# bezirganyan/m2-mixer

Measured on AMD Instinct MI355X. Metric: training samples/sec AV-MNIST M2-Mixer-B bf16, higher is better.
Workload: dtype bf16

## Files before the change

include/m2mixer.h:

```cpp
#ifndef M2MIXER_H
#define M2MIXER_H

#include <stdint.h>

#ifdef __cplusplus
extern "C" {
#endif

#define M2M_ABI_VERSION 18
#define M2M_MAX_BLOCKS 8
#define M2M_ROWS_PER_WG 16

#define M2M_SPLIT_GPART 1472

#define M2M_PREC_BF16 0
#define M2M_PREC_F32 1

typedef struct m2m_block {
    const float* ln1_w;
    const float* ln1_b;
    const float* tok_w1;
    const float* tok_b1;
    const float* tok_w2;
    const float* tok_b2;
    const float* ln2_w;
    const float* ln2_b;
    const float* ch_w1;
    const float* ch_b1;
    const float* ch_w2;
    const float* ch_b2;
    void* w1n;
    void* w2c;
    void* w2tn;
    void* w1tc;
    float* ch_b1p;
    float* g_ln1_w; float* g_ln1_b; float* g_tok_w1; float* g_tok_b1; float* g_tok_w2; float* g_tok_b2;
    float* g_ln2_w; float* g_ln2_b; float* g_ch_w1; float* g_ch_b1; float* g_ch_w2; float* g_ch_b2;
    float* x_in;
    float* x_mid;
    void* at_chn;
    void* dyt_chn;
    void* h_chn;
    void* dh_chn;
} m2m_block;

typedef struct m2m_tower {
    int32_t prec;
    int32_t D, N, T, C;
    int32_t Cp;
    int32_t nblocks;
    int32_t has_final_ln;
    float p_drop;
    uint32_t site_base;
    const float* lnf_w;
    const float* lnf_b;
    float* g_lnf_w;
    float* g_lnf_b;
    float* x_final;
    float* ws_a;
    float* ws_b;
    m2m_block blk[M2M_MAX_BLOCKS];
    float* slabs;
    int32_t nsplit;
    int32_t wgrad_flags;
    float* xres;
    float* gpart;
    void* a_nat[M2M_MAX_BLOCKS];
    void* dy_nat[M2M_MAX_BLOCKS];
    float* wslot[M2M_MAX_BLOCKS];
    void* dx0_chn;
} m2m_tower;
#define M2M_WGRAD_OVERWRITE 1
#define M2M_WGRAD_GROUP_SLOTS 4
#define M2M_WGRAD_REDUCES_SMALL 2

typedef struct m2m_embed {
    int32_t prec;
    int32_t Cin, H, W, ph, pw;
    int32_t D;
    int32_t K;
    int32_t Kp;
    const float* w;
    const float* b;
    void* wn;
    float* g_w;
    float* g_b;
    int32_t wgrad_flags;
    int32_t reserved;
} m2m_embed;

int m2m_abi_version(void);
const char* m2m_last_error(void);
int64_t m2m_packed_bytes(int prec, int64_t I, int64_t K);

int m2m_pack(int prec, int mode, int order_k_major, const float* src, int64_t stride_i, int64_t stride_k,
             int64_t I, int64_t K, void* dst, void* stream);
int m2m_pack_tower(const m2m_tower* t, void* stream);
int m2m_pack_embed(const m2m_embed* e, void* stream);
int m2m_pack_all(const m2m_tower* const* towers, int ntowers, const m2m_embed* const* embeds, int nembeds, void* stream);
int m2m_pack_skips_w1tc(const m2m_tower* t);

int m2m_embed_forward(const m2m_embed* e, const float* input, int B, float* x0, void* stream);
typedef struct m2m_step_head {
    float* adam_state; uint32_t* drop_counter; float* losses; int32_t nlosses;
} m2m_step_head;
int m2m_embeds_forward(const m2m_embed* const* embeds, const float* const* inputs, float* const* x0s, const int* nsplits,
                       const int64_t* part_strides, int nembeds, int B, const m2m_step_head* head, void* stream);
int m2m_embed_fwd_splits(const m2m_embed* e);
int m2m_embed_forward_head(const m2m_embed* e, const float* input, int B, float* x0, const m2m_step_head* head, void* stream);

int m2m_tower_forward(const m2m_tower* t, const float* x0, int64_t x0_sample_stride, int B,
                      float* out, int64_t out_sample_stride, float* pooled,
                      int training, uint32_t seed, uint32_t step, const uint32_t* step_dev, void* stream);

int m2m_towers_can_group(const m2m_tower* a, const m2m_tower* b, int B);
typedef struct m2m_tower_io {
    const float* x0; int64_t x0_sample_stride;
    float* out; int64_t out_sample_stride;
    float* pooled;
    int32_t x0_parts;
    int64_t x0_part_stride;
} m2m_tower_io;
int m2m_towers_forward(const m2m_tower* const* towers, const m2m_tower_io* io, int ntowers, int B, int training,
                       uint32_t seed, uint32_t step, const uint32_t* step_dev, void* stream);
int m2m_towers_forward_embeds_ok(const m2m_tower* const* towers, int ntowers, const m2m_embed* const* embeds, int B);
int m2m_towers_forward_embeds(const m2m_tower* const* towers, const m2m_tower_io* io, int ntowers,
                              const m2m_embed* const* embeds, const float* const* inputs, const m2m_step_head* head,
                              int B, int training, uint32_t seed, uint32_t step, const uint32_t* step_dev, void* stream);

int m2m_tower_backward(const m2m_tower* t, int B, const float* d_out, int64_t d_out_sample_stride,
                       const float* d_pooled, float* d_x0, int64_t d_x0_sample_stride,
                       uint32_t seed, uint32_t step, const uint32_t* step_dev, void* stream);
typedef struct m2m_tower_gio {
    const float* d_out; int64_t d_out_sample_stride;
    const float* d_pooled;
    float* d_x0; int64_t d_x0_sample_stride;
} m2m_tower_gio;
int m2m_towers_backward(const m2m_tower* const* towers, const m2m_tower_gio* io, int ntowers, int B,
                        uint32_t seed, uint32_t step, const uint32_t* step_dev, void* stream);
int m2m_tower_wgrad(const m2m_tower* t, int B, uint32_t seed, uint32_t step, const uint32_t* step_dev, void* stream);
int m2m_wgrad_form(const m2m_tower* t, int B);
int m2m_towers_wgrad(const m2m_tower* const* towers, const m2m_tower* const* dev_towers, int ntowers,
                     const m2m_embed* const* embeds, const float* const* inputs, const float* const* d_x0s,
                     const m2m_tower* const* embed_towers, int nembeds,
                     int B, uint32_t seed, uint32_t step, const uint32_t* step_dev, void* stream);
int m2m_wgrad_groups(const m2m_tower* t, int B);
int m2m_embeds_wgrad_form(const m2m_embed* const* embeds, const m2m_tower* const* embed_towers, int nembeds, int B);
int m2m_wgrad_slot_groups(const m2m_tower* const* towers, int ntowers, int B);
int m2m_wgrad_fold(const m2m_tower* t, void* stream);
int m2m_embed_wgrad(const m2m_embed* e, const float* input, const float* d_x0, int B, void* stream);
int m2m_embeds_wgrad(const m2m_embed* const* embeds, const float* const* inputs, const float* const* d_x0s, int nembeds, int B,
                     void* stream);

typedef struct m2m_head {
    const float* pooled;
    const float* w;
    const float* b;
    float* g_w;
    float* g_b;
    float* d_pooled;
    float weight;
    float* g_part;
    const float* tokens;
    int64_t tok_sample_stride;
    int32_t ntok;
} m2m_head;
int m2m_heads_part_tiles(int B);
int m2m_heads_ce(const m2m_head* heads, int nheads, const int64_t* labels, int B, int D, int K,
                 float* logits, float* losses, int32_t* preds, int zero_losses, void* stream);

int m2m_heads_bce(const m2m_head* heads, int nheads, const float* targets, const float* pos_weight, int B, int D, int K,
                  float* logits, float* losses, int32_t* preds, int zero_losses, void* stream);

int m2m_heads_ce_w(const m2m_head* heads, int nheads, const int64_t* labels, int B, int D, int K,
                   float* logits, float* losses, int32_t* preds, int zero_losses, const float* weights, void* stream);
int m2m_heads_bce_w(const m2m_head* heads, int nheads, const float* targets, const float* pos_weight, int B, int D, int K,
                    float* logits, float* losses, int32_t* preds, int zero_losses, const float* weights, void* stream);

int m2m_towers_wgrad_heads(const m2m_tower* const* towers, const m2m_tower* const* dev_towers, int ntowers,
                           const m2m_embed* const* embeds, const float* const* inputs, const float* const* d_x0s,
                           const m2m_tower* const* embed_towers, int nembeds,
                           int B, uint32_t seed, uint32_t step, const uint32_t* step_dev,
                           const m2m_head* heads, int nheads, int K, void* stream);

int m2m_towers_wgrad_tail(const m2m_tower* const* towers, const m2m_tower* const* dev_towers, int ntowers,
                          const m2m_embed* const* embeds, const float* const* inputs, const float* const* d_x0s,
                          const m2m_tower* const* embed_towers, int nembeds,
                          int B, uint32_t seed, uint32_t step, const uint32_t* step_dev,
                          const m2m_head* heads, int nheads, int K, uint32_t* bump_counter, void* stream);

int m2m_tower_backward_heads_ok(const m2m_tower* t, int B, int nheads, int K);
int m2m_tower_backward_heads(const m2m_tower* t, int B, const m2m_head* heads, int nheads, int own, const int64_t* labels,
                             int K, float* logits, float* losses, int32_t* preds, float* d_x0, int64_t d_x0_sample_stride,
                             uint32_t seed, uint32_t step, const uint32_t* step_dev, void* stream);

#define M2M_MLP_MAX_LAYERS 4
typedef struct m2m_mlp {
    int32_t nlayers;
    int32_t has_out;
    int32_t dims[M2M_MLP_MAX_LAYERS + 1];
    float p_drop;
    uint32_t site_base;
    const float* w[M2M_MLP_MAX_LAYERS];
    const float* b[M2M_MLP_MAX_LAYERS];
    float* g_w[M2M_MLP_MAX_LAYERS];
    float* g_b[M2M_MLP_MAX_LAYERS];
    float* act[M2M_MLP_MAX_LAYERS];
} m2m_mlp;
int m2m_mlp_forward(const m2m_mlp* m, const float* x, int B, float* out, int64_t out_sample_stride, float* out_dense,
                    int training, uint32_t seed, uint32_t step, const uint32_t* step_dev, void* stream);
int m2m_mlp_backward(const m2m_mlp* m, const float* x, int B, const float* d_out, int64_t d_out_sample_stride,
                     const float* d_out_dense, void* stream);
int m2m_mlp_forward_ride(const m2m_mlp* m, const float* x, int B, float* out, int64_t out_sample_stride, float* out_dense,
                         int training, uint32_t seed, uint32_t step, const uint32_t* step_dev);
int m2m_mlp_backward_ride(const m2m_mlp* m, const float* x, int B, const float* d_out, int64_t d_out_sample_stride,
                          const float* d_out_dense);
int m2m_mlp_ride_flush(void* stream);

int m2m_adam_step(float* param, float* grad, float* exp_avg, float* exp_avg_sq, int64_t n,
                  float* state, float beta1, float beta2, float eps, float weight_decay,
                  float grad_scale, int bump_step, void* stream);
int m2m_adam_step_bf16(float* param, float* grad, const void* grad_bf16, float* exp_avg, float* exp_avg_sq, int64_t n,
                       float* state, float beta1, float beta2, float eps, float weight_decay,
                       float grad_scale, int bump_step, void* stream);

#define M2M_MAX_GRAD_RANGES 16
typedef struct m2m_grad_range { int64_t lo, n; const float* add; int32_t keep; int32_t reserved; } m2m_grad_range;
int m2m_adam_step_ranges(float* param, float* grad, const void* grad_bf16, float* exp_avg, float* exp_avg_sq, int64_t n,
                         float* state, float beta1, float beta2, float eps, float weight_decay, float grad_scale, int bump_step,
                         const m2m_grad_range* ranges, int nranges, void* stream);

int64_t m2m_adam_pack_plan_bytes(void);
int m2m_adam_pack_plan(const m2m_tower* const* towers, int ntowers, const m2m_embed* const* embeds, int nembeds,
                       float* param, float* grad, const void* grad_bf16, float* exp_avg, float* exp_avg_sq, int64_t n,
                       const float* state, float beta1, float beta2, float eps, float weight_decay, float grad_scale,
                       void* plan_host);
int m2m_adam_pack_plan_ranges(const m2m_tower* const* towers, int ntowers, const m2m_embed* const* embeds, int nembeds,
                              float* param, float* grad, const void* grad_bf16, float* exp_avg, float* exp_avg_sq, int64_t n,
                              const float* state, float beta1, float beta2, float eps, float weight_decay, float grad_scale,
                              const m2m_grad_range* ranges, int nranges, void* plan_host);
int m2m_adam_pack_all(const m2m_tower* const* towers, int ntowers, const m2m_embed* const* embeds, int nembeds,
                      const void* plan_dev, const void* plan_host, void* stream);

int m2m_step_prologue(float* adam_state, uint32_t* drop_counter, float* losses, int nlosses, void* stream);

int m2m_counter_add(uint32_t* counter, uint32_t delta, void* stream);

#define M2M_FUSION_SUM 1
#define M2M_FUSION_MEAN 2
#define M2M_FUSION_MAX 3
int m2m_fusion_forward(int mode, const float* a, const float* b, float* y, int64_t n, void* stream);
int m2m_fusion_backward(int mode, const float* a, const float* b, const float* dy, float* da, float* db, int64_t n, void* stream);

typedef struct m2m_gate {
    int32_t D;
    int32_t reserved;
    const float *w1, *b1, *w2, *b2, *wz, *bz;
    float *g_w1, *g_b1, *g_w2, *g_b2, *g_wz, *g_bz;
    float *t1, *t2, *z, *dh, *part;
} m2m_gate;
int64_t m2m_gate_part_floats(int64_t rows, int D);
int m2m_gate_forward(const m2m_gate* g, const float* a, const float* b, float* y, int64_t rows, int save, void* stream);
int m2m_gate_backward(const m2m_gate* g, const float* dy, float* da, float* db, int64_t rows, void* stream);
int m2m_gate_wgrad(const m2m_gate* g, const float* a, const float* b, int64_t rows, void* stream);

#define M2M_SCORES_MAX_CLASSES 64
#define M2M_SCORES_MAX_LABELS 128
int m2m_scores_multiclass(const int32_t* preds, const int64_t* labels, int nheads, int B, int K, uint64_t* table, void* stream);
int m2m_scores_multilabel(const int32_t* preds, const float* targets, int nheads, int B, int K, uint64_t* table, void* stream);

int m2m_dropout_mask(const m2m_tower* t, int blk, int site, int B, uint32_t seed, uint32_t step,
                     uint8_t* mask, void* stream);
int m2m_gelu_probe(const float* x, float* y, float* dy, int64_t n, void* stream);
int m2m_gemm_probe(int prec, const float* A, const float* Bm, int I, int J, int K,
                   const float* Bc, int J2, float* C, float* C2, void* workspace, void* stream);

int m2m_clock_probe(uint64_t* out, int nwg, int spin_ticks, void* stream);

#ifdef __cplusplus
}
#endif
#endif
```

m2_mixer_amd/_lib.py:

```python
from __future__ import annotations

import ctypes as C
import os
import subprocess

_HERE = os.path.dirname(os.path.abspath(__file__))
LIB_PATH = os.environ.get("M2M_LIB_PATH", os.path.join(_HERE, "libm2mixer.so"))
CSRC = os.path.join(_HERE, "csrc")

ABI_VERSION = 18
MAX_BLOCKS = 8
ROWS_PER_WG = 16
HCHN_PAD = 4096
SPLIT_ROWS = 128
SPLIT_MAX = 8
SPLIT_GPART = 1472
PREC_BF16, PREC_F32 = 0, 1
PREC_BY_NAME = {"bf16": PREC_BF16, "fp32": PREC_F32, "f32": PREC_F32}

_fp = C.c_void_p


class Block(C.Structure):
    PARAMS = ["ln1_w", "ln1_b", "tok_w1", "tok_b1", "tok_w2", "tok_b2", "ln2_w", "ln2_b",
              "ch_w1", "ch_b1", "ch_w2", "ch_b2"]
    PACKED = ["w1n", "w2c", "w2tn", "w1tc", "ch_b1p"]
    GRADS = ["g_" + p for p in PARAMS]
    SAVED = ["x_in", "x_mid", "at_chn", "dyt_chn", "h_chn", "dh_chn"]
    _fields_ = [(n, _fp) for n in PARAMS + PACKED + GRADS + SAVED]


class Tower(C.Structure):
    _fields_ = [("prec", C.c_int32), ("D", C.c_int32), ("N", C.c_int32), ("T", C.c_int32), ("C", C.c_int32),
                ("Cp", C.c_int32), ("nblocks", C.c_int32), ("has_final_ln", C.c_int32),
                ("p_drop", C.c_float), ("site_base", C.c_uint32),
                ("lnf_w", _fp), ("lnf_b", _fp), ("g_lnf_w", _fp), ("g_lnf_b", _fp), ("x_final", _fp),
                ("ws_a", _fp), ("ws_b", _fp), ("blk", Block * MAX_BLOCKS),
                ("slabs", _fp), ("nsplit", C.c_int32), ("wgrad_flags", C.c_int32), ("xres", _fp), ("gpart", _fp),
                ("a_nat", _fp * MAX_BLOCKS), ("dy_nat", _fp * MAX_BLOCKS),
                ("wslot", _fp * MAX_BLOCKS),
                ("dx0_chn", _fp)]


WGRAD_OVERWRITE = 1
WGRAD_REDUCES_SMALL = 2
WGRAD_GROUP_SLOTS = 4
MAX_GRAD_RANGES = 16


class GradRange(C.Structure):
    _fields_ = [("lo", C.c_int64), ("n", C.c_int64), ("add", _fp), ("keep", C.c_int32), ("reserved", C.c_int32)]


class TowerIO(C.Structure):
    _fields_ = [("x0", _fp), ("x0_ss", C.c_int64), ("out", _fp), ("out_ss", C.c_int64), ("pooled", _fp),
                ("x0_parts", C.c_int32), ("x0_part_stride", C.c_int64)]


class StepHead(C.Structure):
    _fields_ = [("adam_state", _fp), ("drop_counter", _fp), ("losses", _fp), ("nlosses", C.c_int32)]


class TowerGIO(C.Structure):
    _fields_ = [("d_out", _fp), ("d_out_ss", C.c_int64), ("d_pooled", _fp), ("d_x0", _fp), ("d_x0_ss", C.c_int64)]


class Embed(C.Structure):
    _fields_ = [("prec", C.c_int32), ("Cin", C.c_int32), ("H", C.c_int32), ("W", C.c_int32), ("ph", C.c_int32),
                ("pw", C.c_int32), ("D", C.c_int32), ("K", C.c_int32), ("Kp", C.c_int32),
                ("w", _fp), ("b", _fp), ("wn", _fp), ("g_w", _fp), ("g_b", _fp), ("wgrad_flags", C.c_int32), ("reserved", C.c_int32)]


class Head(C.Structure):
    _fields_ = [("pooled", _fp), ("w", _fp), ("b", _fp), ("g_w", _fp), ("g_b", _fp), ("d_pooled", _fp),
                ("weight", C.c_float), ("g_part", _fp), ("tokens", _fp), ("tok_sample_stride", C.c_int64), ("ntok", C.c_int32)]


SCORES_MAX_CLASSES, SCORES_MAX_LABELS = 64, 128
FUSION_SUM, FUSION_MEAN, FUSION_MAX = 1, 2, 3


class Gate(C.Structure):
    _fields_ = [("D", C.c_int32), ("reserved", C.c_int32)] + [(n, _fp) for n in (
        "w1", "b1", "w2", "b2", "wz", "bz", "g_w1", "g_b1", "g_w2", "g_b2", "g_wz", "g_bz", "t1", "t2", "z", "dh", "part")]


MLP_MAX_LAYERS = 4


class Mlp(C.Structure):
    _fields_ = [("nlayers", C.c_int32), ("has_out", C.c_int32), ("dims", C.c_int32 * (MLP_MAX_LAYERS + 1)),
                ("p_drop", C.c_float), ("site_base", C.c_uint32),
                ("w", _fp * MLP_MAX_LAYERS), ("b", _fp * MLP_MAX_LAYERS), ("g_w", _fp * MLP_MAX_LAYERS),
                ("g_b", _fp * MLP_MAX_LAYERS), ("act", _fp * MLP_MAX_LAYERS)]


SIGNATURES = {
    "m2m_abi_version": (C.c_int, []),
    "m2m_last_error": (C.c_char_p, []),
    "m2m_packed_bytes": (C.c_int64, [C.c_int, C.c_int64, C.c_int64]),
    "m2m_pack": (C.c_int, [C.c_int, C.c_int, C.c_int, _fp, C.c_int64, C.c_int64, C.c_int64, C.c_int64, _fp, _fp]),
    "m2m_pack_tower": (C.c_int, [C.POINTER(Tower), _fp]),
    "m2m_pack_embed": (C.c_int, [C.POINTER(Embed), _fp]),
    "m2m_pack_skips_w1tc": (C.c_int, [C.POINTER(Tower)]),
    "m2m_pack_all": (C.c_int, [C.POINTER(C.POINTER(Tower)), C.c_int, C.POINTER(C.POINTER(Embed)), C.c_int, _fp]),
    "m2m_embed_forward": (C.c_int, [C.POINTER(Embed), _fp, C.c_int, _fp, _fp]),
    "m2m_embed_forward_head": (C.c_int, [C.POINTER(Embed), _fp, C.c_int, _fp, C.POINTER(StepHead), _fp]),
    "m2m_tower_forward": (C.c_int, [C.POINTER(Tower), _fp, C.c_int64, C.c_int, _fp, C.c_int64, _fp, C.c_int,
                                    C.c_uint32, C.c_uint32, _fp, _fp]),
    "m2m_tower_backward": (C.c_int, [C.POINTER(Tower), C.c_int, _fp, C.c_int64, _fp, _fp, C.c_int64,
                                     C.c_uint32, C.c_uint32, _fp, _fp]),
    "m2m_tower_backward_heads_ok": (C.c_int, [C.POINTER(Tower), C.c_int, C.c_int, C.c_int]),
    "m2m_tower_backward_heads": (C.c_int, [C.POINTER(Tower), C.c_int, C.POINTER(Head), C.c_int, C.c_int, _fp, C.c_int, _fp, _fp, _fp, _fp,
                                           C.c_int64, C.c_uint32, C.c_uint32, _fp, _fp]),
    "m2m_tower_wgrad": (C.c_int, [C.POINTER(Tower), C.c_int, C.c_uint32, C.c_uint32, _fp, _fp]),
    "m2m_towers_can_group": (C.c_int, [C.POINTER(Tower), C.POINTER(Tower), C.c_int]),
    "m2m_towers_forward": (C.c_int, [C.POINTER(C.POINTER(Tower)), C.POINTER(TowerIO), C.c_int, C.c_int, C.c_int, C.c_uint32,
                                     C.c_uint32, _fp, _fp]),
    "m2m_towers_forward_embeds_ok": (C.c_int, [C.POINTER(C.POINTER(Tower)), C.c_int, C.POINTER(C.POINTER(Embed)), C.c_int]),
    "m2m_towers_forward_embeds": (C.c_int, [C.POINTER(C.POINTER(Tower)), C.POINTER(TowerIO), C.c_int, C.POINTER(C.POINTER(Embed)),
                                            C.POINTER(_fp), C.POINTER(StepHead), C.c_int, C.c_int, C.c_uint32, C.c_uint32, _fp, _fp]),
    "m2m_towers_backward": (C.c_int, [C.POINTER(C.POINTER(Tower)), C.POINTER(TowerGIO), C.c_int, C.c_int, C.c_uint32, C.c_uint32,
                                      _fp, _fp]),
    "m2m_towers_wgrad": (C.c_int, [C.POINTER(C.POINTER(Tower)), C.POINTER(_fp), C.c_int, C.POINTER(C.POINTER(Embed)), C.POINTER(_fp),
                                   C.POINTER(_fp), C.POINTER(C.POINTER(Tower)), C.c_int, C.c_int, C.c_uint32, C.c_uint32, _fp, _fp]),
    "m2m_towers_wgrad_heads": (C.c_int, [C.POINTER(C.POINTER(Tower)), C.POINTER(_fp), C.c_int, C.POINTER(C.POINTER(Embed)), C.POINTER(_fp),
                                         C.POINTER(_fp), C.POINTER(C.POINTER(Tower)), C.c_int, C.c_int, C.c_uint32, C.c_uint32, _fp,
                                         C.POINTER(Head), C.c_int, C.c_int, _fp]),
    "m2m_towers_wgrad_tail": (C.c_int, [C.POINTER(C.POINTER(Tower)), C.POINTER(_fp), C.c_int, C.POINTER(C.POINTER(Embed)), C.POINTER(_fp),
                                        C.POINTER(_fp), C.POINTER(C.POINTER(Tower)), C.c_int, C.c_int, C.c_uint32, C.c_uint32, _fp,
                                        C.POINTER(Head), C.c_int, C.c_int, _fp, _fp]),
    "m2m_heads_part_tiles": (C.c_int, [C.c_int]),
    "m2m_wgrad_form": (C.c_int, [C.POINTER(Tower), C.c_int]),
    "m2m_embeds_wgrad_form": (C.c_int, [C.POINTER(C.POINTER(Embed)), C.POINTER(C.POINTER(Tower)), C.c_int, C.c_int]),
    "m2m_wgrad_groups": (C.c_int, [C.POINTER(Tower), C.c_int]),
    "m2m_wgrad_slot_groups": (C.c_int, [C.POINTER(C.POINTER(Tower)), C.c_int, C.c_int]),
    "m2m_wgrad_fold": (C.c_int, [C.POINTER(Tower), _fp]),
    "m2m_adam_step_ranges": (C.c_int, [_fp, _fp, _fp, _fp, _fp, C.c_int64, _fp, C.c_float, C.c_float, C.c_float, C.c_float,
                                       C.c_float, C.c_int, C.POINTER(GradRange), C.c_int, _fp]),
    "m2m_counter_add": (C.c_int, [_fp, C.c_uint32, _fp]),
    "m2m_embed_wgrad": (C.c_int, [C.POINTER(Embed), _fp, _fp, C.c_int, _fp]),
    "m2m_embeds_wgrad": (C.c_int, [C.POINTER(C.POINTER(Embed)), C.POINTER(_fp), C.POINTER(_fp), C.c_int, C.c_int, _fp]),
    "m2m_embeds_forward": (C.c_int, [C.POINTER(C.POINTER(Embed)), C.POINTER(_fp), C.POINTER(_fp), C.POINTER(C.c_int), C.POINTER(C.c_int64),
                                     C.c_int, C.c_int, C.POINTER(StepHead), _fp]),
    "m2m_embed_fwd_splits": (C.c_int, [C.POINTER(Embed)]),
    "m2m_heads_ce": (C.c_int, [C.POINTER(Head), C.c_int, _fp, C.c_int, C.c_int, C.c_int, _fp, _fp, _fp, C.c_int, _fp]),
    "m2m_step_prologue": (C.c_int, [_fp, _fp, _fp, C.c_int, _fp]),
    "m2m_heads_bce": (C.c_int, [C.POINTER(Head), C.c_int, _fp, _fp, C.c_int, C.c_int, C.c_int, _fp, _fp, _fp, C.c_int, _fp]),
    "m2m_heads_ce_w": (C.c_int, [C.POINTER(Head), C.c_int, _fp, C.c_int, C.c_int, C.c_int, _fp, _fp, _fp, C.c_int, _fp, _fp]),
    "m2m_heads_bce_w": (C.c_int, [C.POINTER(Head), C.c_int, _fp, _fp, C.c_int, C.c_int, C.c_int, _fp, _fp, _fp, C.c_int, _fp, _fp]),
    "m2m_fusion_forward": (C.c_int, [C.c_int, _fp, _fp, _fp, C.c_int64, _fp]),
    "m2m_fusion_backward": (C.c_int, [C.c_int, _fp, _fp, _fp, _fp, _fp, C.c_int64, _fp]),
    "m2m_gate_part_floats": (C.c_int64, [C.c_int64, C.c_int]),
    "m2m_gate_forward": (C.c_int, [C.POINTER(Gate), _fp, _fp, _fp, C.c_int64, C.c_int, _fp]),
    "m2m_gate_backward": (C.c_int, [C.POINTER(Gate), _fp, _fp, _fp, C.c_int64, _fp]),
    "m2m_gate_wgrad": (C.c_int, [C.POINTER(Gate), _fp, _fp, C.c_int64, _fp]),
    "m2m_scores_multiclass": (C.c_int, [_fp, _fp, C.c_int, C.c_int, C.c_int, _fp, _fp]),
    "m2m_scores_multilabel": (C.c_int, [_fp, _fp, C.c_int, C.c_int, C.c_int, _fp, _fp]),
    "m2m_mlp_forward": (C.c_int, [C.POINTER(Mlp), _fp, C.c_int, _fp, C.c_int64, _fp, C.c_int, C.c_uint32, C.c_uint32,
                                  _fp, _fp]),
    "m2m_mlp_backward": (C.c_int, [C.POINTER(Mlp), _fp, C.c_int, _fp, C.c_int64, _fp, _fp]),
    "m2m_mlp_forward_ride": (C.c_int, [C.POINTER(Mlp), _fp, C.c_int, _fp, C.c_int64, _fp, C.c_int, C.c_uint32, C.c_uint32, _fp]),
    "m2m_mlp_backward_ride": (C.c_int, [C.POINTER(Mlp), _fp, C.c_int, _fp, C.c_int64, _fp]),
    "m2m_mlp_ride_flush": (C.c_int, [_fp]),
    "m2m_adam_step": (C.c_int, [_fp, _fp, _fp, _fp, C.c_int64, _fp, C.c_float, C.c_float, C.c_float, C.c_float,
                                C.c_float, C.c_int, _fp]),
    "m2m_adam_step_bf16": (C.c_int, [_fp, _fp, _fp, _fp, _fp, C.c_int64, _fp, C.c_float, C.c_float, C.c_float, C.c_float,
                                     C.c_float, C.c_int, _fp]),
    "m2m_adam_pack_plan_bytes": (C.c_int64, []),
    "m2m_adam_pack_plan": (C.c_int, [C.POINTER(C.POINTER(Tower)), C.c_int, C.POINTER(C.POINTER(Embed)), C.c_int, _fp, _fp, _fp, _fp, _fp,
                                    C.c_int64, _fp, C.c_float, C.c_float, C.c_float, C.c_float, C.c_float, _fp]),
    "m2m_adam_pack_plan_ranges": (C.c_int, [C.POINTER(C.POINTER(Tower)), C.c_int, C.POINTER(C.POINTER(Embed)), C.c_int, _fp, _fp, _fp, _fp, _fp,
                                           C.c_int64, _fp, C.c_float, C.c_float, C.c_float, C.c_float, C.c_float,
                                           C.POINTER(GradRange), C.c_int, _fp]),
    "m2m_adam_pack_all": (C.c_int, [C.POINTER(C.POINTER(Tower)), C.c_int, C.POINTER(C.POINTER(Embed)), C.c_int, _fp, _fp, _fp]),
    "m2m_dropout_mask": (C.c_int, [C.POINTER(Tower), C.c_int, C.c_int, C.c_int, C.c_uint32, C.c_uint32, _fp, _fp]),
    "m2m_gelu_probe": (C.c_int, [_fp, _fp, _fp, C.c_int64, _fp]),
    "m2m_gemm_probe": (C.c_int, [C.c_int, _fp, _fp, C.c_int, C.c_int, C.c_int, _fp, C.c_int, _fp, _fp, _fp, _fp]),
    "m2m_clock_probe": (C.c_int, [_fp, C.c_int, C.c_int, _fp]),
}

_lib = None


def csrc_hash() -> str:
    import glob
    import hashlib
    h = hashlib.sha256()
    for f in sorted(glob.glob(os.path.join(CSRC, "*.hip")) + glob.glob(os.path.join(CSRC, "*.h")) +
                    [os.path.join(os.path.dirname(_HERE), "include", "m2mixer.h")]):
        h.update(os.path.basename(f).encode())
        h.update(open(f, "rb").read())
    return h.hexdigest()


def build(force: bool = False, verbose: bool = False) -> str:
    if force:
        subprocess.run(["make", "-C", CSRC, "clean"], check=True, capture_output=not verbose)
    r = subprocess.run(["make", "-C", CSRC, "-j", str(min(6, os.cpu_count() or 2))], capture_output=True, text=True)
    if r.returncode != 0:
        raise RuntimeError("building libm2mixer.so failed:\n" + r.stdout[-4000:] + r.stderr[-4000:])
    if verbose:
        print(r.stdout)
    return LIB_PATH


def lib() -> C.CDLL:
    global _lib
    if _lib is None:
        if not os.path.exists(LIB_PATH):
            raise RuntimeError(
                f"{LIB_PATH} is missing: the M2-Mixer hot path exists only as the HIP library "
                "(python -c 'import __graft_entry__ as g; g.build()' builds it); there is no CPU fallback")
        L = C.CDLL(LIB_PATH)
        for name, (res, args) in SIGNATURES.items():
            fn = getattr(L, name)
            fn.restype = res
            fn.argtypes = args
        got = L.m2m_abi_version()
        if got != ABI_VERSION:
            raise RuntimeError(f"libm2mixer ABI {got} != binding ABI {ABI_VERSION}; rebuild")
        _lib = L
    return _lib


def check(rc: int, what: str = "") -> None:
    if rc != 0:
        msg = lib().m2m_last_error().decode("utf-8", "replace")
        kind = "unsupported shape/argument" if rc == -1 else "HIP runtime error"
        raise RuntimeError(f"libm2mixer {what}: {kind}: {msg}")


def ptr(t) -> int:
    return 0 if t is None else t.data_ptr()


def stream_ptr() -> int:
    import torch
    return torch.cuda.current_stream().cuda_stream


def packed_bytes(prec: int, I: int, K: int) -> int:
    kb = 32 if prec == PREC_BF16 else 16
    return ((I + 15) // 16) * ((K + kb - 1) // kb) * 1024
```

m2_mixer_amd/csrc/embed.hip:

```cpp
#include "tile.h"
#include "embed_wgrad.h"

#include "embed_fwd.h"

template <int P, int D, int RB>
__global__ __launch_bounds__(NTHREADS) void embed_fwd_kernel(const m2m_embed em, const float* __restrict__ in, long M, int N,
                                                             float* __restrict__ x0, int fast, const m2m_step_head head) {
    extern __shared__ __attribute__((aligned(16))) char smem[];
    if (blockIdx.x == 0) {
        const int t = threadIdx.x;
        if (t == 0 && head.adam_state) head.adam_state[0] += 1.0f;
        if (t == 1 && head.drop_counter) *head.drop_counter += 1u;
        if (head.losses && t < head.nlosses) head.losses[t] = 0.f;
    }
    if (P == PREC_BF16 && fast) embed_fwd_fast_body<D>(em, in, M, N, x0, blockIdx.x, 0, 1, smem);
    else embed_fwd_body<P, D, RB>(em, in, M, N, x0, blockIdx.x, smem);
}

struct EmbedFwdGroupArgs {
    m2m_embed em[2];
    const float* in[2];
    float* x0[2];
    long M[2];
    int N[2], nwg0, fast[2], nsplit[2];
    long part_stride[2];
    float* adam_state;
    unsigned int* drop_counter;
    float* losses;
    int nlosses, prologue;
};
template <int P, int D, int RB>
__global__ __launch_bounds__(NTHREADS, (P == PREC_BF16 && D <= 128) ? 4 : 1) void embed_fwd_group_kernel(const EmbedFwdGroupArgs a) {
    extern __shared__ __attribute__((aligned(16))) char smem[];
    if (a.prologue && blockIdx.x == 0) {
        const int t = threadIdx.x;
        if (t == 0 && a.adam_state) a.adam_state[0] += 1.0f;
        if (t == 1 && a.drop_counter) *a.drop_counter += 1u;
        if (a.losses && t < a.nlosses) a.losses[t] = 0.f;
    }
    const int e = (int)blockIdx.x < a.nwg0 ? 0 : 1;
    const int wg = e ? blockIdx.x - a.nwg0 : blockIdx.x;
    if (P == PREC_BF16 && a.fast[e]) {
        const int ns = a.nsplit[e], split = wg % ns;
        embed_fwd_fast_body<D>(a.em[e], a.in[e], a.M[e], a.N[e], a.x0[e] + split * a.part_stride[e], wg / ns, split, ns, smem);
    }
    else {
        const int ns = a.nsplit[e], split = wg % ns, tile = wg / ns;
        if (split == 0) embed_fwd_body<P, D, RB>(a.em[e], a.in[e], a.M[e], a.N[e], a.x0[e], tile, smem);
        else {
            float* part = a.x0[e] + split * a.part_stride[e];
            const long m0 = (long)tile * RB;
            for (int idx = threadIdx.x; idx < RB * D; idx += NTHREADS) {
                const long m = m0 + idx / D;
                if (m < a.M[e]) part[m * D + idx % D] = 0.f;
            }
        }
    }
}

template <int P, int D>
__global__ __launch_bounds__(NTHREADS) void embed_wgrad_kernel(const m2m_embed em, const float* __restrict__ in,
                                                               const float* __restrict__ dx0, long M, int N, int tiles_per_group) {
    extern __shared__ __attribute__((aligned(16))) char smem[];
    embed_wgrad_body<P, D, NTHREADS>(em, in, dx0, M, N, tiles_per_group, blockIdx.x, blockIdx.y, gridDim.y == 1, smem);
}

template <int P, int D>
__global__ __launch_bounds__(NTHREADS) void embed_wgrad_group_kernel(const EmbedWgradGroupArgs a) {
    extern __shared__ __attribute__((aligned(16))) char smem[];
    embed_wgrad_group_body<P, D, NTHREADS>(a, blockIdx.x, smem);
}

int m2m_check_embed(const m2m_embed* e, int B) {
    if (!e || B < 1) { m2m_set_error("embed: bad argument", __FILE__, __LINE__); return -1; }
    if (e->H % e->ph || e->W % e->pw) { m2m_set_error("embed: image not divisible by patch", __FILE__, __LINE__); return -1; }
    if (e->K != e->Cin * e->ph * e->pw) { m2m_set_error("embed: K != Cin*ph*pw", __FILE__, __LINE__); return -1; }
    const int KB = e->prec == PREC_BF16 ? 32 : 16;
    if (e->Kp % KB || e->Kp < e->K) { m2m_set_error("embed: Kp must be K rounded up to the k-block", __FILE__, __LINE__); return -1; }
    if (e->Kp > EMB_KMAX - EMB_KS) { m2m_set_error("embed: patch too large (Cin*ph*pw must be <= 3968)", __FILE__, __LINE__); return -1; }
    return 0;
}

template <int P, int D>
static int launch_embed_fwd(const m2m_embed* e, const float* in, int B, float* x0, hipStream_t st, const m2m_step_head* head = nullptr) {
    m2m_step_head hd;
    memset(&hd, 0, sizeof(hd));
    if (head) {
        if (head->nlosses < 0 || head->nlosses > 64) { m2m_set_error("embed_forward: step head nlosses must be in [0, 64]", __FILE__, __LINE__); return -1; }
        hd = *head;
    }
    const int N = (e->H / e->ph) * (e->W / e->pw);
    const long M = (long)B * N;
    constexpr int RB = 16;
    const size_t lds = (size_t)RB * EMB_LD * 4 + (size_t)RB * EMB_KS * Prec<P>::ESZ + EMB_KMAX * 4 + RB * 8;
    auto kern = embed_fwd_kernel<P, D, RB>;
    static bool done = false;
    if (!done) { M2M_CHECK_HIP(hipFuncSetAttribute(reinterpret_cast<const void*>(kern), hipFuncAttributeMaxDynamicSharedMemorySize, (int)lds)); done = true; }
    hipLaunchKernelGGL(kern, dim3((unsigned)((M + RB - 1) / RB)), dim3(NTHREADS), lds, st, *e, in, M, N, x0, (int)embed_fwd_fast_ok(e, in), hd);
    M2M_CHECK_HIP(hipGetLastError());
    return 0;
}
template <int P, int D>
static int launch_embed_fwd_group(const m2m_embed* const* es, const float* const* ins, float* const* x0s, const int* nsplits,
                                  const int64_t* part_strides, const m2m_step_head* head, int B, hipStream_t st) {
    constexpr int RB = 16;
    EmbedFwdGroupArgs a;
    memset(&a, 0, sizeof(a));
    if (head) {
        if (head->nlosses < 0 || head->nlosses > 64) { m2m_set_error("embeds_forward: step head nlosses must be in [0, 64]", __FILE__, __LINE__); return -1; }
        a.prologue = 1; a.adam_state = head->adam_state; a.drop_counter = head->drop_counter; a.losses = head->losses; a.nlosses = head->nlosses;
    }
    const int first = es[1]->Kp > es[0]->Kp ? 1 : 0;
    int total = 0;
    for (int k = 0; k < 2; ++k) {
        const int i = k == 0 ? first : 1 - first;
        const int N = (es[i]->H / es[i]->ph) * (es[i]->W / es[i]->pw);
        a.em[k] = *es[i]; a.in[k] = ins[i]; a.x0[k] = x0s[i]; a.N[k] = N; a.M[k] = (long)B * N;
        a.fast[k] = embed_fwd_fast_ok(es[i], ins[i]);
        a.nsplit[k] = nsplits ? nsplits[i] : 1;
        a.part_stride[k] = part_strides ? (long)part_strides[i] : 0;
        if (a.nsplit[k] < 1 || a.nsplit[k] > 4 || (a.nsplit[k] > 1 && a.part_stride[k] < a.M[k] * (long)D)) {
            m2m_set_error("embeds_forward: 1..4 k-splits, part stride >= B*N*D", __FILE__, __LINE__);
            return -1;
        }
        const int nwg = (int)((a.M[k] + RB - 1) / RB) * a.nsplit[k];
        if (k == 0) a.nwg0 = nwg;
        total += nwg;
    }
    const size_t lds = (size_t)RB * EMB_LD * 4 + (size_t)RB * EMB_KS * Prec<P>::ESZ + EMB_KMAX * 4 + RB * 8;
    auto kern = embed_fwd_group_kernel<P, D, RB>;
    static bool done = false;
    if (!done) { M2M_CHECK_HIP(hipFuncSetAttribute(reinterpret_cast<const void*>(kern), hipFuncAttributeMaxDynamicSharedMemorySize, (int)lds)); done = true; }
    hipLaunchKernelGGL(kern, dim3((unsigned)total), dim3(NTHREADS), lds, st, a);
    M2M_CHECK_HIP(hipGetLastError());
    return 0;
}

template <int P, int D>
static int launch_embed_wgrad(const m2m_embed* e, const float* in, const float* dx0, int B, hipStream_t st) {
    const EmbedWgradPlan pl = embed_wgrad_plan(e, B, 256);
    const size_t lds = embed_wgrad_lds<D, P>();
    auto kern = embed_wgrad_kernel<P, D>;
    static bool done = false;
    if (!done) { M2M_CHECK_HIP(hipFuncSetAttribute(reinterpret_cast<const void*>(kern), hipFuncAttributeMaxDynamicSharedMemorySize, (int)lds)); done = true; }
    hipLaunchKernelGGL(kern, dim3((unsigned)pl.nchunks, (unsigned)pl.groups), dim3(NTHREADS), lds, st, *e, in, dx0, pl.M, pl.N, pl.tpg);
    M2M_CHECK_HIP(hipGetLastError());
    return 0;
}
template <int P, int D>
static int launch_embed_wgrad_group(const m2m_embed* const* es, const float* const* ins, const float* const* dx0s, int B, hipStream_t st) {
    EmbedWgradGroupArgs a;
    const int total = embed_wgrad_group_args(a, es, ins, dx0s, B, 256);
    const size_t lds = embed_wgrad_lds<D, P>();
    auto kern = embed_wgrad_group_kernel<P, D>;
    static bool done = false;
    if (!done) { M2M_CHECK_HIP(hipFuncSetAttribute(reinterpret_cast<const void*>(kern), hipFuncAttributeMaxDynamicSharedMemorySize, (int)lds)); done = true; }
    hipLaunchKernelGGL(kern, dim3((unsigned)total), dim3(NTHREADS), lds, st, a);
    M2M_CHECK_HIP(hipGetLastError());
    return 0;
}

extern "C" int m2m_embed_forward(const m2m_embed* e, const float* input, int B, float* x0, void* stream) {
    return m2m_embed_forward_head(e, input, B, x0, nullptr, stream);
}
extern "C" int m2m_embed_forward_head(const m2m_embed* e, const float* input, int B, float* x0, const m2m_step_head* head, void* stream) {
    if (int rc = m2m_check_embed(e, B)) return rc;
    hipStream_t st = reinterpret_cast<hipStream_t>(stream);
#define M2M_EF_CASE(PP, DD) if (e->prec == PP && e->D == DD) return launch_embed_fwd<PP, DD>(e, input, B, x0, st, head);
    M2M_EF_CASE(PREC_BF16, 32) M2M_EF_CASE(PREC_BF16, 64) M2M_EF_CASE(PREC_BF16, 128) M2M_EF_CASE(PREC_BF16, 256)
    M2M_EF_CASE(PREC_F32, 32) M2M_EF_CASE(PREC_F32, 64) M2M_EF_CASE(PREC_F32, 128) M2M_EF_CASE(PREC_F32, 256)
#undef M2M_EF_CASE
    m2m_set_error("embed_forward: unsupported (prec, D)", __FILE__, __LINE__);
    return -1;
}

extern "C" int m2m_embed_wgrad(const m2m_embed* e, const float* input, const float* d_x0, int B, void* stream) {
    if (int rc = m2m_check_embed(e, B)) return rc;
    hipStream_t st = reinterpret_cast<hipStream_t>(stream);
#define M2M_EW_CASE(PP, DD) if (e->prec == PP && e->D == DD) return launch_embed_wgrad<PP, DD>(e, input, d_x0, B, st);
    M2M_EW_CASE(PREC_BF16, 32) M2M_EW_CASE(PREC_BF16, 64) M2M_EW_CASE(PREC_BF16, 128) M2M_EW_CASE(PREC_BF16, 256)
    M2M_EW_CASE(PREC_F32, 32) M2M_EW_CASE(PREC_F32, 64) M2M_EW_CASE(PREC_F32, 128) M2M_EW_CASE(PREC_F32, 256)
#undef M2M_EW_CASE
    m2m_set_error("embed_wgrad: unsupported (prec, D)", __FILE__, __LINE__);
    return -1;
}

extern "C" int m2m_embeds_wgrad(const m2m_embed* const* embeds, const float* const* inputs, const float* const* d_x0s, int nembeds,
                                int B, void* stream) {
    if (!embeds || !inputs || !d_x0s || nembeds != EMB_GROUP) { m2m_set_error("embeds_wgrad: exactly two embeddings", __FILE__, __LINE__); return -1; }
    for (int i = 0; i < nembeds; ++i) {
        if (int rc = m2m_check_embed(embeds[i], B)) return rc;
        if (embeds[i]->prec != embeds[0]->prec || embeds[i]->D != embeds[0]->D) {
            m2m_set_error("embeds_wgrad: the embeddings of one launch must share precision and hidden_dim", __FILE__, __LINE__);
            return -1;
        }
    }
    hipStream_t st = reinterpret_cast<hipStream_t>(stream);
    const m2m_embed* e = embeds[0];
#define M2M_EWG_CASE(PP, DD) if (e->prec == PP && e->D == DD) return launch_embed_wgrad_group<PP, DD>(embeds, inputs, d_x0s, B, st);
    M2M_EWG_CASE(PREC_BF16, 32) M2M_EWG_CASE(PREC_BF16, 64) M2M_EWG_CASE(PREC_BF16, 128) M2M_EWG_CASE(PREC_BF16, 256)
    M2M_EWG_CASE(PREC_F32, 32) M2M_EWG_CASE(PREC_F32, 64) M2M_EWG_CASE(PREC_F32, 128) M2M_EWG_CASE(PREC_F32, 256)
#undef M2M_EWG_CASE
    m2m_set_error("embeds_wgrad: unsupported (prec, D)", __FILE__, __LINE__);
    return -1;
}

extern "C" int m2m_embed_fwd_splits(const m2m_embed* e) {
    if (!e) return 1;
    static const int forced = [] { const char* v = getenv("M2M_EMBED_SPLITS"); return v ? atoi(v) : 0; }();
    const bool pays = embed_fwd_fast_ok(e, nullptr) && e->Kp >= 4 * EMB_FKS;
    if (pays && forced >= 1 && forced <= 4) return forced;
    return pays ? 2 : 1;
}

extern "C" int m2m_embeds_forward(const m2m_embed* const* embeds, const float* const* inputs, float* const* x0s, const int* nsplits,
                                  const int64_t* part_strides, int nembeds, int B, const m2m_step_head* head, void* stream) {
    if (!embeds || !inputs || !x0s || nembeds != 2) { m2m_set_error("embeds_forward: exactly two embeddings", __FILE__, __LINE__); return -1; }
    for (int i = 0; i < nembeds; ++i) {
        if (int rc = m2m_check_embed(embeds[i], B)) return rc;
        if (embeds[i]->prec != embeds[0]->prec || embeds[i]->D != embeds[0]->D) {
            m2m_set_error("embeds_forward: the embeddings of one launch must share precision and hidden_dim", __FILE__, __LINE__);
            return -1;
        }
    }
    hipStream_t st = reinterpret_cast<hipStream_t>(stream);
    const m2m_embed* e = embeds[0];
#define M2M_EFG_CASE(PP, DD) if (e->prec == PP && e->D == DD) return launch_embed_fwd_group<PP, DD>(embeds, inputs, x0s, nsplits, part_strides, head, B, st);
    M2M_EFG_CASE(PREC_BF16, 32) M2M_EFG_CASE(PREC_BF16, 64) M2M_EFG_CASE(PREC_BF16, 128) M2M_EFG_CASE(PREC_BF16, 256)
    M2M_EFG_CASE(PREC_F32, 32) M2M_EFG_CASE(PREC_F32, 64) M2M_EFG_CASE(PREC_F32, 128) M2M_EFG_CASE(PREC_F32, 256)
#undef M2M_EFG_CASE
    m2m_set_error("embeds_forward: unsupported (prec, D)", __FILE__, __LINE__);
    return -1;
}
```

m2_mixer_amd/csrc/embed_fwd.h:

```cpp
#pragma once
#include "tile.h"
#include "embed_wgrad.h"

#ifndef EMB_KS
#define EMB_KS 128
#endif
#define EMB_LD (EMB_KS + 4)
#define EMB_KMAX 4096

template <int P, int D, int RB>
static __device__ __forceinline__ void embed_fwd_body(const m2m_embed& em, const float* __restrict__ in, long M, int N,
                                                      float* __restrict__ x0, int wg, char* smem) {
    typedef Prec<P> Pr;
    constexpr int DT = D / 16, KSB = EMB_KS / Pr::KB;
    constexpr int DPW = (DT + NWAVES - 1) / NWAVES;
    float* tile = reinterpret_cast<float*>(smem);
    char* img = smem + RB * EMB_LD * 4;
    int* koff = reinterpret_cast<int*>(img + RB * EMB_KS * Pr::ESZ);
    long* rbase = reinterpret_cast<long*>(koff + EMB_KMAX);

    const int tid = threadIdx.x, lane = tid & 63, wave = tid >> 6, g = lane >> 4, il = lane & 15;
    PatchGeom pg{em.Cin, em.H, em.W, em.ph, em.pw, em.W / em.pw, N, em.K};
    const long m0 = (long)wg * RB;
    const int nKB = em.Kp / Pr::KB;
    const int kext = (em.Kp + EMB_KS - 1) / EMB_KS * EMB_KS;
    for (int k = tid; k < kext; k += NTHREADS) koff[k] = patch_koff(pg, k);
    if (tid < RB) rbase[tid] = patch_rowbase(pg, m0 + tid, M);

    f32x4_t acc[(RB / 16)][DPW];
#pragma unroll
    for (int mt = 0; mt < (RB / 16); ++mt)
#pragma unroll
        for (int j = 0; j < DPW; ++j) acc[mt][j] = f32x4_t{0.f, 0.f, 0.f, 0.f};

    constexpr int EPT = RB * EMB_KS / NTHREADS;
    float pre[EPT];
    Frag wpre[DPW][KSB];
    auto load_stage = [&](int k0) {
#pragma unroll
        for (int i = 0; i < EPT; ++i) {
            const int idx = i * NTHREADS + tid;
            const int r = idx / EMB_KS, kk = idx % EMB_KS;
            const long rb = rbase[r];
            const int ko = koff[k0 + kk];
            pre[i] = (rb >= 0 && ko >= 0) ? in[rb + ko] : 0.f;
        }
        const int kb0 = k0 / Pr::KB;
#pragma unroll
        for (int j = 0; j < DPW; ++j) {
            const int dt = wave + NWAVES * j;
#pragma unroll
            for (int kb = 0; kb < KSB; ++kb) {
                wpre[j][kb].u = u32x4_t{0u, 0u, 0u, 0u};
                if (dt < DT && kb0 + kb < nKB) wpre[j][kb] = ld_frag_global(em.wn, (long)dt * nKB + kb0 + kb, lane);
            }
        }
    };
    __syncthreads();
    load_stage(0);
    for (int k0 = 0; k0 < em.Kp; k0 += EMB_KS) {
#pragma unroll
        for (int i = 0; i < EPT; ++i) {
            const int idx = i * NTHREADS + tid;
            tile[(idx / EMB_KS) * EMB_LD + idx % EMB_KS] = pre[i];
        }
        Frag wcur[DPW][KSB];
#pragma unroll
        for (int j = 0; j < DPW; ++j)
#pragma unroll
            for (int kb = 0; kb < KSB; ++kb) wcur[j][kb] = wpre[j][kb];
        __syncthreads();
        if (k0 + EMB_KS < em.Kp) load_stage(k0 + EMB_KS);
        for (int slot = tid; slot < (RB / 16) * KSB * 64; slot += NTHREADS) {
            const int blk = slot >> 6;
            *reinterpret_cast<u32x4_t*>(img + slot * 16) =
                gather_slot<P>(tile, EMB_LD, PACK_NAT, false, blk / KSB, blk % KSB, slot & 63);
        }
        __syncthreads();
#pragma unroll
        for (int j = 0; j < DPW; ++j) {
            const int dt = wave + NWAVES * j;
            if (dt < DT) {
#pragma unroll
                for (int kb = 0; kb < KSB; ++kb) {
#pragma unroll
                    for (int mt = 0; mt < (RB / 16); ++mt) {
                        const Frag a = ld_frag_lds(img, mt * KSB + kb, lane);
                        Pr::mma(acc[mt][j], a, wcur[j][kb]);
                    }
                }
            }
        }
    }
#pragma unroll
    for (int j = 0; j < DPW; ++j) {
        const int dt = wave + NWAVES * j;
        if (dt < DT) {
            const int d = 16 * dt + il;
            const float bv = em.b[d];
#pragma unroll
            for (int mt = 0; mt < (RB / 16); ++mt)
#pragma unroll
                for (int r = 0; r < 4; ++r) {
                    const long m = m0 + 16 * mt + 4 * g + r;
                    if (m < M) x0[m * D + d] = acc[mt][j][r] + bv;
                }
        }
    }
}

#define EMB_FKS 256
#ifndef EMB_FDEPTH
#define EMB_FDEPTH 2
#endif
template <int D>
static __device__ __forceinline__ void embed_fwd_fast_body(const m2m_embed& em, const float* __restrict__ in, long M, int N,
                                                           float* __restrict__ x0, int wg, int split, int nsplit, char* smem) {
    typedef Prec<PREC_BF16> Pr;
    constexpr int KSB = EMB_FKS / 32, DT = D / 16, DPW = (DT + NWAVES - 1) / NWAVES, IMG_B = 16 * EMB_FKS * 2;
    static_assert(KSB == NWAVES, "one k-block of the stage per wave");
    char* img = smem;
    const int tid = threadIdx.x, lane = tid & 63, wave = tid >> 6, g = lane >> 4, il = lane & 15;
    PatchGeom pg{em.Cin, em.H, em.W, em.ph, em.pw, em.W / em.pw, N, em.K};
    const long m0 = (long)wg * 16;
    const long rb = patch_rowbase(pg, m0 + il, M);
    const int nKB = em.Kp / 32;
    const int nst_all = (em.Kp + EMB_FKS - 1) / EMB_FKS;
    const int per = (nst_all + nsplit - 1) / nsplit;
    const int st_begin = split * per, nst = min(nst_all, st_begin + per);

    f32x4_t acc[DPW];
#pragma unroll
    for (int j = 0; j < DPW; ++j) acc[j] = f32x4_t{0.f, 0.f, 0.f, 0.f};
    struct Pre {
        f32x4_t p0, p1;
        Frag w[DPW][KSB];
    };
    auto load = [&](Pre& p, int st) {
        const int k = min(st * EMB_FKS + wave * 32 + 8 * g, em.K - 8);
        const float* src = in + (rb >= 0 ? rb : 0) + patch_koff(pg, k);
        p.p0 = *reinterpret_cast<const f32x4_t*>(src);
        p.p1 = *reinterpret_cast<const f32x4_t*>(src + 4);
#pragma unroll
        for (int j = 0; j < DPW; ++j) {
            const int dt = min(wave + NWAVES * j, DT - 1);
#pragma unroll
            for (int kb = 0; kb < KSB; ++kb) p.w[j][kb] = ld_frag_global(em.wn, (long)dt * nKB + min(st * KSB + kb, nKB - 1), lane);
        }
    };
    auto step = [&](Pre& p, int st) {
        const bool valid = rb >= 0 && st < nst && st * EMB_FKS + wave * 32 + 8 * g < em.K;
        Frag f;
        f.u[0] = pack_bf2(p.p0[0], p.p0[1]); f.u[1] = pack_bf2(p.p0[2], p.p0[3]);
        f.u[2] = pack_bf2(p.p1[0], p.p1[1]); f.u[3] = pack_bf2(p.p1[2], p.p1[3]);
        if (!valid) f.u = u32x4_t{0u, 0u, 0u, 0u};
        char* cur = img + ((st - st_begin) & 1) * IMG_B;
        *reinterpret_cast<u32x4_t*>(cur + tid * 16) = f.u;
        __syncthreads();
#pragma unroll
        for (int kb = 0; kb < KSB; ++kb) {
            const Frag a = ld_frag_lds(cur, kb, lane);
#pragma unroll
            for (int j = 0; j < DPW; ++j)
                if (wave + NWAVES * j < DT) Pr::mma(acc[j], a, p.w[j][kb]);
        }
        load(p, st + EMB_FDEPTH);
    };
    Pre ring[EMB_FDEPTH];
#pragma unroll
    for (int d = 0; d < EMB_FDEPTH; ++d) load(ring[d], st_begin + d);
    for (int st = st_begin; st < nst; st += EMB_FDEPTH) {
#pragma unroll
        for (int d = 0; d < EMB_FDEPTH; ++d) step(ring[d], st + d);
    }
#pragma unroll
    for (int j = 0; j < DPW; ++j) {
        const int dt = wave + NWAVES * j;
        if (dt < DT) {
            const int d = 16 * dt + il;
            const float bv = split == 0 ? em.b[d] : 0.f;
#pragma unroll
            for (int r = 0; r < 4; ++r) {
                const long m = m0 + 4 * g + r;
                if (m < M) x0[m * D + d] = acc[j][r] + bv;
            }
        }
    }
}
static inline bool embed_fwd_fast_ok(const m2m_embed* e, const float* in) {
    return e->prec == PREC_BF16 && e->pw % 8 == 0 && e->W % 4 == 0 && e->K >= 8 && (reinterpret_cast<uintptr_t>(in) & 15) == 0;
}
```

m2_mixer_amd/csrc/embed_wgrad.h:

```cpp
#pragma once
#include "tile.h"
#include <stdlib.h>

#define EBM 32

int m2m_check_embed(const m2m_embed* e, int B);

struct PatchGeom {
    int Cin, H, W, ph, pw, GW, N, K;
};
static __device__ __forceinline__ int patch_koff(const PatchGeom& pg, int k) {
    if (k >= pg.K) return -1;
    const int c = k / (pg.ph * pg.pw), rem = k % (pg.ph * pg.pw);
    const int py = rem / pg.pw, px = rem % pg.pw;
    return (c * pg.H + py) * pg.W + px;
}
static __device__ __forceinline__ long patch_rowbase(const PatchGeom& pg, long m, long M) {
    if (m >= M) return -1;
    const long b = m / pg.N;
    const int n = (int)(m % pg.N);
    const int gy = n / pg.GW, gx = n % pg.GW;
    return (b * pg.Cin * pg.H + gy * pg.ph) * (long)pg.W + gx * pg.pw;
}

template <int P, int D, int NT>
static __device__ __forceinline__ void embed_wgrad_body(const m2m_embed& em, const float* __restrict__ in,
                                                        const float* __restrict__ dx0, long M, int N, int tiles_per_group,
                                                        int chunk, int group, bool single, char* smem) {
    typedef Prec<P> Pr;
    constexpr int DT = D / 16, NKM = EBM / Pr::KB, XLD = TileGeom<D>::XLD;
    constexpr int KC = 64, KCT = KC / 16, PLD = KC + 4;
    constexpr int DPW = (DT + (NT / 64) - 1) / (NT / 64);
    constexpr int NDX = (EBM * (D / 4) + NT - 1) / NT;
    constexpr int NPT = EBM * KC / NT;
    static_assert(NT % KC == 0 && EBM % (NT / KC) == 0, "patch tile mapping");
    float* dxt = reinterpret_cast<float*>(smem);
    float* pt = dxt + EBM * XLD;
    char* aimg = reinterpret_cast<char*>(pt + EBM * PLD);
    char* bimg = aimg + EBM * D * Pr::ESZ;

    const int tid = threadIdx.x, lane = tid & 63, wave = tid >> 6, g = lane >> 4, il = lane & 15;
    PatchGeom pg{em.Cin, em.H, em.W, em.ph, em.pw, em.W / em.pw, N, em.K};
    const int k0 = chunk * KC;
    const int ko = patch_koff(pg, k0 + (tid % KC));

    f32x4_t acc[DPW][KCT];
#pragma unroll
    for (int j = 0; j < DPW; ++j)
#pragma unroll
        for (int kt = 0; kt < KCT; ++kt) acc[j][kt] = f32x4_t{0.f, 0.f, 0.f, 0.f};
    float bsum = 0.f;

    const long ntiles = (M + EBM - 1) / EBM;
    const long t_begin = (long)group * tiles_per_group;
    const long t_end = min(ntiles, t_begin + tiles_per_group);
    float4 dxr[NDX];
    float ptr_[NPT];
    auto load_tile = [&](long tl) {
        const long m0 = tl * EBM;
#pragma unroll
        for (int i = 0; i < NDX; ++i) {
            const int idx = i * NT + tid;
            const int r = idx / (D / 4), c = (idx % (D / 4)) * 4;
            dxr[i] = make_float4(0.f, 0.f, 0.f, 0.f);
            if (idx < EBM * (D / 4) && m0 + r < M) dxr[i] = *reinterpret_cast<const float4*>(dx0 + (m0 + r) * D + c);
        }
#pragma unroll
        for (int i = 0; i < NPT; ++i) {
            const long rb = patch_rowbase(pg, m0 + tid / KC + (NT / KC) * i, M);
            ptr_[i] = (rb >= 0 && ko >= 0) ? in[rb + ko] : 0.f;
        }
    };
    if (t_begin < t_end) load_tile(t_begin);
    for (long tl = t_begin; tl < t_end; ++tl) {
        __syncthreads();
#pragma unroll
        for (int i = 0; i < NDX; ++i) {
            const int idx = i * NT + tid;
            if (idx < EBM * (D / 4)) *reinterpret_cast<float4*>(dxt + (idx / (D / 4)) * XLD + (idx % (D / 4)) * 4) = dxr[i];
        }
#pragma unroll
        for (int i = 0; i < NPT; ++i) pt[(tid / KC + (NT / KC) * i) * PLD + tid % KC] = ptr_[i];
        if (tl + 1 < t_end) load_tile(tl + 1);
        __syncthreads();
        if (chunk == 0 && tid < D) {
            float s = 0.f;
            for (int r = 0; r < EBM; ++r) s += dxt[r * XLD + tid];
            bsum += s;
        }
        for (int slot = tid; slot < DT * NKM * 64; slot += NT) {
            const int blk = slot >> 6;
            *reinterpret_cast<u32x4_t*>(aimg + slot * 16) =
                gather_slot<P>(dxt, XLD, PACK_NAT, true, blk / NKM, blk % NKM, slot & 63);
        }
        for (int slot = tid; slot < KCT * NKM * 64; slot += NT) {
            const int blk = slot >> 6;
            *reinterpret_cast<u32x4_t*>(bimg + slot * 16) =
                gather_slot<P>(pt, PLD, PACK_NAT, true, blk / NKM, blk % NKM, slot & 63);
        }
        __syncthreads();
#pragma unroll
        for (int j = 0; j < DPW; ++j) {
            const int dt = wave + (NT / 64) * j;
            if (dt < DT) {
#pragma unroll
                for (int kbm = 0; kbm < NKM; ++kbm) {
                    const Frag a = ld_frag_lds(aimg, dt * NKM + kbm, lane);
#pragma unroll
                    for (int kt = 0; kt < KCT; ++kt) {
                        const Frag b = ld_frag_lds(bimg, kt * NKM + kbm, lane);
                        Pr::mma(acc[j][kt], a, b);
                    }
                }
            }
        }
    }
#pragma unroll
    for (int j = 0; j < DPW; ++j) {
        const int dt = wave + (NT / 64) * j;
        if (dt < DT) {
#pragma unroll
            for (int kt = 0; kt < KCT; ++kt)
#pragma unroll
                for (int r = 0; r < 4; ++r) {
                    const int d = 16 * dt + 4 * g + r, k = k0 + 16 * kt + il;
                    if (k < em.K) {
                        float* p = em.g_w + (long)d * em.K + k;
                        if (single) *p += acc[j][kt][r]; else atomicAdd(p, acc[j][kt][r]);
                    }
                }
        }
    }
    if (chunk == 0 && tid < D) { if (single) em.g_b[tid] += bsum; else atomicAdd(em.g_b + tid, bsum); }
}

#define EFK 32
template <int D, int NT> static constexpr size_t embed_wgrad_fast_red_bytes() { return (size_t)(NT / 64) * (EFK / 16) * (D / 16) * 64 * 16; }
bool m2m_split_eligible(const m2m_tower* t, int B, int training);
template <int D, int NT>
static __device__ __forceinline__ void embed_wgrad_fast_body(const m2m_embed& em, const float* __restrict__ in,
                                                             const char* __restrict__ dx0_chn, long M, int N, int npairs, int rpt,
                                                             int chunk, bool vec2, char* smem) {
    typedef Prec<PREC_BF16> Pr;
    constexpr int DT = D / 16, NW = NT / 64, NB = EFK / 16;
    static_assert(NB == 2, "two 16-column fragments per workgroup (the 8-byte gather pairs them)");
    const int tid = threadIdx.x, lane = tid & 63, g = lane >> 4, il = lane & 15;
    const int wave = __builtin_amdgcn_readfirstlane(tid >> 6);
    PatchGeom pg{em.Cin, em.H, em.W, em.ph, em.pw, em.W / em.pw, N, em.K};
    const int k0 = chunk * EFK;
    int ko[NB];
#pragma unroll
    for (int jb = 0; jb < NB; ++jb) ko[jb] = patch_koff(pg, vec2 ? k0 + 2 * il + jb : k0 + 16 * jb + il);
    int* tokoff = reinterpret_cast<int*>(smem + embed_wgrad_fast_red_bytes<D, NT>());
    for (int n = tid; n < N; n += NT) tokoff[n] = (n / pg.GW) * pg.ph * pg.W + (n % pg.GW) * pg.pw;
    __syncthreads();
    const unsigned int sstride = (unsigned int)(em.Cin * em.H * em.W), uN = (unsigned int)N, uM = (unsigned int)M;
    const unsigned int magic = 0xFFFFFFFFu / uN;

    f32x4_t acc[NB][DT];
#pragma unroll
    for (int jb = 0; jb < NB; ++jb)
#pragma unroll
        for (int dt = 0; dt < DT; ++dt) acc[jb][dt] = f32x4_t{0.f, 0.f, 0.f, 0.f};

    struct Tile { Frag a[DT]; float v[NB][8]; unsigned int okbits; };
    auto load = [&](Tile& t, int p) {
#pragma unroll
        for (int dt = 0; dt < DT; ++dt) t.a[dt] = ld_frag_global(dx0_chn, (long)p * DT + dt, lane);
        unsigned int rb[8];
        bool okr[8];
#pragma unroll
        for (int e = 0; e < 8; ++e) {
            const int r = 4 * g + (e & 3);
            const unsigned int row = (unsigned int)((2 * p + (e >> 2)) * rpt + r);
            okr[e] = r < rpt && row < uM;
            const unsigned int rowc = okr[e] ? row : 0u;
            unsigned int q = __umulhi(rowc, magic);
            unsigned int n = rowc - q * uN;
            if (n >= uN) { n -= uN; q += 1u; }
            rb[e] = q * sstride + (unsigned int)tokoff[n];
        }
        if (vec2) {
            const unsigned int k2 = (unsigned int)max(ko[0], 0);
#pragma unroll
            for (int e = 0; e < 8; ++e) {
                const float2 x = *reinterpret_cast<const float2*>(in + rb[e] + k2);
                t.v[0][e] = x.x; t.v[1][e] = x.y;
            }
        } else {
#pragma unroll
            for (int e = 0; e < 8; ++e)
#pragma unroll
                for (int jb = 0; jb < NB; ++jb) t.v[jb][e] = in[rb[e] + (unsigned int)max(ko[jb], 0)];
        }
        t.okbits = 0u;
#pragma unroll
        for (int e = 0; e < 8; ++e) t.okbits |= (okr[e] ? 1u : 0u) << e;
    };
    auto mac = [&](const Tile& t) {
#pragma unroll
        for (int jb = 0; jb < NB; ++jb) {
            Frag b;
            float z[8];
#pragma unroll
            for (int e = 0; e < 8; ++e) z[e] = ((t.okbits >> e) & 1u) && ko[jb] >= 0 ? t.v[jb][e] : 0.f;
#pragma unroll
            for (int e = 0; e < 4; ++e) b.u[e] = pack_bf2(z[2 * e], z[2 * e + 1]);
#pragma unroll
            for (int dt = 0; dt < DT; ++dt) Pr::mma(acc[jb][dt], t.a[dt], b);
        }
    };
    Tile t0, t1;
    const int p0 = wave;
    if (p0 < npairs) load(t0, p0);
    for (int p = p0; p < npairs; p += 2 * NW) {
        if (p + NW < npairs) load(t1, p + NW);
        mac(t0);
        if (p + NW < npairs) {
            if (p + 2 * NW < npairs) load(t0, p + 2 * NW);
            mac(t1);
        }
    }
    f32x4_t* red = reinterpret_cast<f32x4_t*>(smem);
#pragma unroll
    for (int jb = 0; jb < NB; ++jb)
#pragma unroll
        for (int dt = 0; dt < DT; ++dt) red[((wave * NB + jb) * DT + dt) * 64 + lane] = acc[jb][dt];
    __syncthreads();
    for (int q = wave; q < NB * DT; q += NW) {
        const int jb = q / DT, dt = q % DT;
        f32x4_t s = red[q * 64 + lane];
#pragma unroll
        for (int w = 1; w < NW; ++w) s = s + red[(w * NB * DT + q) * 64 + lane];
        const int k = vec2 ? k0 + 2 * il + jb : k0 + 16 * jb + il;
        if (k < em.K) {
            const bool store = (em.wgrad_flags & M2M_WGRAD_OVERWRITE) != 0;
#pragma unroll
            for (int r = 0; r < 4; ++r) {
                float* qd = em.g_w + (long)(16 * dt + 4 * g + r) * em.K + k;
                *qd = store ? s[r] : *qd + s[r];
            }
        }
    }
    if (chunk == 0) {
        Frag ones;
        ones.u = u32x4_t{0x3F803F80u, 0x3F803F80u, 0x3F803F80u, 0x3F803F80u};
        f32x4_t accb[DT];
#pragma unroll
        for (int dt = 0; dt < DT; ++dt) accb[dt] = f32x4_t{0.f, 0.f, 0.f, 0.f};
        for (int p = wave; p < npairs; p += NW) {
            Frag a[DT];
#pragma unroll
            for (int dt = 0; dt < DT; ++dt) a[dt] = ld_frag_global(dx0_chn, (long)p * DT + dt, lane);
#pragma unroll
            for (int dt = 0; dt < DT; ++dt) Pr::mma(accb[dt], a[dt], ones);
        }
        __syncthreads();
#pragma unroll
        for (int dt = 0; dt < DT; ++dt) red[(wave * DT + dt) * 64 + lane] = accb[dt];
        __syncthreads();
        for (int dt = wave; dt < DT; dt += NW) {
            f32x4_t sb = red[dt * 64 + lane];
#pragma unroll
            for (int w = 1; w < NW; ++w) sb = sb + red[(w * DT + dt) * 64 + lane];
            if (il == 0) {
#pragma unroll
                for (int r = 0; r < 4; ++r) em.g_b[16 * dt + 4 * g + r] += sb[r];
            }
        }
    }
}
template <int D, int NT> static constexpr size_t embed_wgrad_fast_lds() { return embed_wgrad_fast_red_bytes<D, NT>() + 128 * sizeof(int); }

#define EMB_GROUP 2
struct EmbedWgradGroupArgs {
    m2m_embed em[EMB_GROUP];
    const float* in[EMB_GROUP];
    const float* dx0[EMB_GROUP];
    long M[EMB_GROUP];
    int N[EMB_GROUP], tpg[EMB_GROUP], nchunks[EMB_GROUP], groups[EMB_GROUP];
    const char* dx0_chn[EMB_GROUP];
    int npairs[EMB_GROUP], rpt[EMB_GROUP], vec2[EMB_GROUP], fast;
};
template <int P, int D, int NT>
static __device__ __forceinline__ void embed_wgrad_group_body(const EmbedWgradGroupArgs& a, int id, char* smem) {
    const int n0 = a.nchunks[0] * a.groups[0];
    const int e = id < n0 ? 0 : 1;
    if (e) id -= n0;
    if constexpr (P == PREC_BF16) {
        if (a.fast) {
            embed_wgrad_fast_body<D, NT>(a.em[e], a.in[e], a.dx0_chn[e], a.M[e], a.N[e], a.npairs[e], a.rpt[e], id, a.vec2[e] != 0, smem);
            return;
        }
    }
    if constexpr (NT % 64 == 0 && EBM % (NT / 64) == 0)
        embed_wgrad_body<P, D, NT>(a.em[e], a.in[e], a.dx0[e], a.M[e], a.N[e], a.tpg[e], id % a.nchunks[e], id / a.nchunks[e],
                                   a.groups[e] == 1, smem);
}

struct EmbedWgradPlan { long M; int N, nchunks, groups, tpg; };
static EmbedWgradPlan embed_wgrad_plan(const m2m_embed* e, int B, int target_wgs) {
    EmbedWgradPlan pl;
    pl.N = (e->H / e->ph) * (e->W / e->pw);
    pl.M = (long)B * pl.N;
    pl.nchunks = (e->K + 63) / 64;
    const long ntiles = (pl.M + EBM - 1) / EBM;
    long groups = (target_wgs + pl.nchunks - 1) / pl.nchunks;
    if (groups > ntiles / 4) groups = ntiles / 4;
    if (groups < 1) groups = 1;
    pl.tpg = (int)((ntiles + groups - 1) / groups);
    pl.groups = (int)((ntiles + pl.tpg - 1) / pl.tpg);
    return pl;
}
template <int D, int P> static constexpr size_t embed_wgrad_lds() {
    return (size_t)EBM * TileGeom<D>::XLD * 4 + (size_t)EBM * 68 * 4 + (size_t)EBM * D * Prec<P>::ESZ + (size_t)EBM * 64 * Prec<P>::ESZ;
}


static inline int embed_wgrad_group_args_fast(EmbedWgradGroupArgs& a, const m2m_embed* const* es, const float* const* ins,
                                              const m2m_tower* const* tw, int B) {
    memset(&a, 0, sizeof(a));
    int total = 0;
    for (int i = 0; i < EMB_GROUP; ++i) {
        const m2m_embed* e = es[i];
        const m2m_tower* t = tw ? tw[i] : nullptr;
        const int N = (e->H / e->ph) * (e->W / e->pw);
        if (!t || !t->dx0_chn || e->prec != PREC_BF16 || t->prec != PREC_BF16 || m2m_is_wide(t) || t->N != N || t->D != e->D) return 0;
        if (m2m_split_eligible(t, B, 1)) return 0;
        if (N > 128 || e->D > 128 || (long)B * e->Cin * e->H * e->W >= (1L << 31)) return 0;
        const int SPW = BM / t->N, nchain = (B + SPW - 1) / SPW;
        a.em[i] = *e; a.in[i] = ins[i]; a.dx0_chn[i] = (const char*)t->dx0_chn;
        a.M[i] = (long)B * N; a.N[i] = N; a.npairs[i] = (nchain * BM + WPAIR - 1) / WPAIR; a.rpt[i] = SPW * t->N;
        a.nchunks[i] = (e->K + EFK - 1) / EFK; a.groups[i] = 1; a.tpg[i] = 0;
        static const int vec2_on = [] { const char* v = getenv("M2M_EMBED_VEC2"); return v ? atoi(v) : 1; }();
        a.vec2[i] = (vec2_on && e->pw % 2 == 0 && e->W % 2 == 0 && ((long)e->H * e->W) % 2 == 0 && e->K % 2 == 0 && ((uintptr_t)ins[i] & 7) == 0) ? 1 : 0;
        total += a.nchunks[i];
    }
    a.fast = 1;
    return total;
}

static inline int embed_wgrad_group_args(EmbedWgradGroupArgs& a, const m2m_embed* const* es, const float* const* ins,
                                         const float* const* dx0s, int B, int target_wgs, int n = EMB_GROUP) {
    memset(&a, 0, sizeof(a));
    if (n == 1) {
        const EmbedWgradPlan p0 = embed_wgrad_plan(es[0], B, target_wgs);
        a.em[0] = *es[0]; a.in[0] = ins[0]; a.dx0[0] = dx0s[0];
        a.M[0] = p0.M; a.N[0] = p0.N; a.tpg[0] = p0.tpg; a.nchunks[0] = p0.nchunks; a.groups[0] = p0.groups;
        a.em[1] = *es[0];
        return p0.nchunks * p0.groups;
    }
    EmbedWgradPlan pl[EMB_GROUP];
    for (int i = 0; i < EMB_GROUP; ++i) pl[i] = embed_wgrad_plan(es[i], B, target_wgs);
    const int first = pl[1].tpg > pl[0].tpg ? 1 : 0;
    int total = 0;
    for (int k = 0; k < EMB_GROUP; ++k) {
        const int i = k == 0 ? first : 1 - first;
        a.em[k] = *es[i]; a.in[k] = ins[i]; a.dx0[k] = dx0s[i];
        a.M[k] = pl[i].M; a.N[k] = pl[i].N; a.tpg[k] = pl[i].tpg; a.nchunks[k] = pl[i].nchunks; a.groups[k] = pl[i].groups;
        total += pl[i].nchunks * pl[i].groups;
    }
    return total;
}
```

m2_mixer_amd/csrc/tower_wgrad.hip:

```cpp
#include "tile.h"
#include "embed_wgrad.h"
#include "split.h"
#include <stdlib.h>
#include <string.h>
bool m2m_split_eligible(const m2m_tower* t, int B, int training);

#if defined(__HIP_DEVICE_COMPILE__)
#define M2M_GLOBAL_AS __attribute__((address_space(1)))
#else
#define M2M_GLOBAL_AS
#endif

#define WBM 32
#ifndef WG_RING_MAX
#define WG_RING_MAX 24
#endif
#define WG_WAVES 4
#ifndef WG_WAVES_WIDE
#define WG_WAVES_WIDE 5
#endif
#ifndef WG_LA
#define WG_LA 4
#endif
#ifndef WG_MINWAVES
// ... 225 lines not shown
        };
        auto step2 = [&](HD& x, int tile, int i) {
            char* cur = smem + (i & 1) * STAGE_B;
#pragma unroll
            for (int k = 0; k < NLD; ++k) {
                const int o = (k * G::THREADS + tid) * 16;
                if (o < STAGE_B) *reinterpret_cast<u32x4_t*>(cur + o) = st[k];
            }
            Frag hf[CPW], df[CPW];
#pragma unroll
            for (int j = 0; j < CPW; ++j) {
                hf[j].u = u32x4_t{x.h0[2 * j], x.h0[2 * j + 1], x.h1[2 * j], x.h1[2 * j + 1]};
                df[j].u = u32x4_t{x.d0[2 * j], x.d0[2 * j + 1], x.d1[2 * j], x.d1[2 * j + 1]};
            }
            load_st(min(tile + 1, t_end - 1));
            load_hd(x, min(tile + 2, t_end - 1));
            __syncthreads();
            constexpr int NQ = DT;
            constexpr int LA = WG_LA < NQ ? WG_LA : NQ;
            Frag aq[LA], dq[LA];
#pragma unroll
            for (int q = 0; q < LA; ++q) { aq[q] = ld_frag_lds(cur, q, lane); dq[q] = ld_frag_lds(cur + IMG_B, q, lane); }
#pragma unroll
            for (int q = 0; q < NQ; ++q) {
                const Frag at = aq[q % LA], dyt = dq[q % LA];
                if (q + LA < NQ) { aq[q % LA] = ld_frag_lds(cur, q + LA, lane); dq[q % LA] = ld_frag_lds(cur + IMG_B, q + LA, lane); }
#pragma unroll
                for (int j = 0; j < CPW; ++j) {
                    Pr::mma(dw1[j][q], df[j], at);
                    Pr::mma(dw2[j][q], hf[j], dyt);
                }
                if (q == NQ - 1) {
#pragma unroll
                    for (int j = 0; j < CPW; ++j) Pr::mma(db1[j], df[j], ones);
                }
            }
        };
        HD ring[2];
        load_hd(ring[0], t_begin);
        load_st(t_begin);
        load_hd(ring[1], min(t_begin + 1, t_end - 1));
        int tile = t_begin, it = 0;
        for (; tile + 2 <= t_end; tile += 2) {
            step2(ring[0], tile, it++);
            step2(ring[1], tile + 1, it++);
        }
        if (tile < t_end) step2(ring[0], tile, it++);
    } else {
    Pre p[DEPTH];
#pragma unroll
    for (int k = 0; k < DEPTH; ++k) tile_load(p[k], min(t_begin + k * TPS, t_end - 1), t_end);
    int tile = t_begin, it = 0;
    if (DEPTH == 1) {
        for (; tile < t_end; tile += TPS) step(p[0], tile, t_end, it++);
    } else {
        for (; tile + DEPTH <= t_end; tile += DEPTH) {
#pragma unroll
            for (int k = 0; k < DEPTH; ++k) step(p[k], tile + k, t_end, it++);
        }
#pragma unroll
        for (int k = 0; k + 1 < DEPTH; ++k)
            if (tile + k < t_end) step(p[k], tile + k, t_end, it++);
    }
    }

    __syncthreads();
    wgrad_write_w<D, CPW>(dw1, dw2, out, ct0, nct, C, smem, wave, lane);
#pragma unroll
    for (int j = 0; j < CPW; ++j) {
        if (ct0 + j >= nct || il != 0) continue;
#pragma unroll
        for (int r = 0; r < 4; ++r) {
            const int c = 16 * (ct0 + j) + 4 * g + r;
            if (c >= C) continue;
            if (out.mode == WG_OUT_ATOMIC) atomicAdd(out.b1 + c, db1[j][r]);
            else if (out.mode == WG_OUT_ADD) out.b1[c] += db1[j][r];
            else out.b1[c] = db1[j][r];
        }
    }
    TIMER_MARK(g_tm_wg, 4);
}

template <class TW>
static __device__ __forceinline__ WgOut wgrad_out(const TW& tw, int b, int group, int ngroups, int slot_mode) {
    const m2m_block& bk = tw.blk[b];
    WgOut o;
    o.w1 = bk.g_ch_w1; o.w2 = bk.g_ch_w2; o.b1 = bk.g_ch_b1;
    const bool overwrite = (tw.wgrad_flags & M2M_WGRAD_OVERWRITE) != 0;
    if (ngroups == 1) o.mode = overwrite ? WG_OUT_STORE : WG_OUT_ADD;
    else if (slot_mode) {
        if (group == 0) o.mode = overwrite ? WG_OUT_STORE : WG_OUT_ADD;
        else {
            const long cd = (long)tw.C * tw.D;
            float* s = tw.wslot[b];
            o.w1 = s; o.b1 = s + cd; o.w2 = s + cd + tw.C;
            o.mode = WG_OUT_STORE;
        }
    } else o.mode = WG_OUT_ATOMIC;
    return o;
}

#ifndef M2M_WGRAD_DMA
#define M2M_WGRAD_DMA 0
#endif
template <int P, int D, int RCDM> struct WgradHasDma { static constexpr bool value = M2M_WGRAD_DMA && RCDM < 0 && P == PREC_BF16 && D == 128; };

template <int P, int D, int RCDM> struct WgradKernelGeom {
    static constexpr bool RC = RCDM >= 0;
    static constexpr int LDS_PLAIN = RC ? RcGeom<D>::LDS_B : WgradGeom<P, D>::LDS_B;
    static constexpr int LDS_DMA = DrGeom<D, WgradGeom<P, D>::WAVES>::LDS_B;
    static constexpr int LDS_B = WgradHasDma<P, D, RCDM>::value ? LDS_DMA : LDS_PLAIN;
    static constexpr int COLS = RC ? RcGeom<D>::COLS : WgradGeom<P, D>::COLS;
    static constexpr int MINWAVES = RC ? 2 : WgradGeom<P, D>::MINWAVES;
    static constexpr int THREADS = RC ? RC_THREADS : WgradGeom<P, D>::THREADS;
};

template <int P, int D, int RCDM, class TW>
static __device__ __forceinline__ void wgrad_dispatch(const TW& tw, int b, int slice, int group, int ngroups, int slot_mode, int ntiles,
                                                      int tpg, int rows_per_t16, unsigned int seed, unsigned int step, int dma, char* smem) {
    const WgOut out = wgrad_out(tw, b, group, ngroups, slot_mode);
    if constexpr (RCDM >= 0) {
        const Drop dr = make_drop(true, tw.p_drop, seed, step, tw.site_base + 4u * (unsigned int)b + 2u);
        wgrad_rc_body<D, RCDM>(tw.blk[b], out, tw.Cp, tw.C, slice, group, ntiles, tpg, rows_per_t16, dr.key, dr.scale, smem);
    } else {
        if constexpr (WgradHasDma<P, D, RCDM>::value)
            wgrad_dma_body<D, WgradGeom<P, D>::WAVES>(tw.blk[b], out, tw.Cp, tw.C, slice, group, ntiles, tpg, smem);
        else
            wgrad_body<P, D>(tw.blk[b], out, tw.Cp, tw.C, slice, group, ntiles, tpg, smem);
    }
}

template <int P, int D, int RCDM>
__global__ __launch_bounds__((WgradKernelGeom<P, D, RCDM>::THREADS), (WgradKernelGeom<P, D, RCDM>::MINWAVES)) void tower_wgrad_kernel(
    const m2m_tower tw, int ntiles, int tiles_per_group, int slot_mode, int rows_per_t16, unsigned int seed, unsigned int step_host,
    const unsigned int* __restrict__ step_dev, int dma) {
    extern __shared__ __attribute__((aligned(16))) char smem[];
    const unsigned int step = step_host + (step_dev ? *step_dev : 0u);
    wgrad_dispatch<P, D, RCDM>(tw, (int)blockIdx.y, (int)blockIdx.x, (int)blockIdx.z, (int)gridDim.z, slot_mode, ntiles, tiles_per_group,
                               rows_per_t16, seed, step, dma, smem);
}

#define WG_MAX_TOWERS 4
#define WG_MAX_JOBS 32
struct WgradGroupArgs {
    const m2m_tower* tw[WG_MAX_TOWERS];
    int ntiles[WG_MAX_TOWERS], tpg[WG_MAX_TOWERS], groups[WG_MAX_TOWERS], nsl[WG_MAX_TOWERS], slot[WG_MAX_TOWERS], rpt[WG_MAX_TOWERS];
    unsigned char job_tower[WG_MAX_JOBS], job_block[WG_MAX_JOBS];
    short job_start[WG_MAX_JOBS + 1];
    short xcd_start[8], xcd_len[8];
    int njobs, n_tower_wgs;
    int dma;
    int n_embed_first, n_embed_pad;
    int n_reduce, reduce_sets;
    unsigned int seed, step_host;
    const unsigned int* step_dev;
    unsigned int* bump_counter;
};
#ifndef M2M_WG_KATTR
#define M2M_WG_KATTR
#endif
template <int P, int D, int RCDM>
__global__ __launch_bounds__((WgradKernelGeom<P, D, RCDM>::THREADS), (WgradKernelGeom<P, D, RCDM>::MINWAVES)) M2M_WG_KATTR void tower_wgrad_group_kernel(const WgradGroupArgs a,
                                                                                                          const EmbedWgradGroupArgs ea,
                                                                                                          const SplitReduceArgs ra) {
    extern __shared__ __attribute__((aligned(16))) char smem[];
    int id = blockIdx.x;
    if (a.bump_counter && blockIdx.x == 0 && threadIdx.x == 0) *a.bump_counter += 1u;
#ifndef M2M_WG_PROBE_TOWERS_ONLY
    if (a.n_reduce && id >= (int)gridDim.x - a.n_reduce) {
        const int rid = id - ((int)gridDim.x - a.n_reduce);
        const int bx = rid % SPR_NBX, L = (rid / SPR_NBX) % a.reduce_sets, z = rid / (SPR_NBX * a.reduce_sets);
        split_small_grads_body<WgradKernelGeom<P, D, RCDM>::THREADS>(ra.t[z], bx, L, reinterpret_cast<float*>(smem));
        return;
    }
    if (id < a.n_embed_pad) {
        if (id < a.n_embed_first) embed_wgrad_group_body<P, D, WgradKernelGeom<P, D, RCDM>::THREADS>(ea, id, smem);
        return;
    }
    id -= a.n_embed_pad;
    if (id >= a.n_tower_wgs) {
        embed_wgrad_group_body<P, D, WgradKernelGeom<P, D, RCDM>::THREADS>(ea, id - a.n_tower_wgs, smem);
        return;
    }
#endif
    const int xcd = id & 7, idx = id >> 3;
    if (idx >= a.xcd_len[xcd]) return;
    const int lin = a.xcd_start[xcd] + idx;
    int job = 0;
    while (job + 1 < a.njobs && lin >= a.job_start[job + 1]) ++job;
    const int t = a.job_tower[job], rel = lin - a.job_start[job];
    const int slice = rel % a.nsl[t], group = rel / a.nsl[t];
    const m2m_tower& tw = *a.tw[t];
    const unsigned int step = a.step_host + (a.step_dev ? *a.step_dev : 0u);
    wgrad_dispatch<P, D, RCDM>(tw, (int)a.job_block[job], slice, group, a.groups[t], a.slot[t], a.ntiles[t], a.tpg[t], a.rpt[t], a.seed,
                               step, a.dma, smem);
}

static_assert(sizeof(WgradGroupArgs) + sizeof(EmbedWgradGroupArgs) + sizeof(SplitReduceArgs) <= 3840, "kernel arguments are limited to 4 KiB");

#ifdef M2M_ISA_PROBE
template __global__ void tower_wgrad_group_kernel<PREC_BF16, 128, -1>(const WgradGroupArgs, const EmbedWgradGroupArgs, const SplitReduceArgs);
template __global__ void tower_wgrad_group_kernel<PREC_BF16, 128, DM_HALF>(const WgradGroupArgs, const EmbedWgradGroupArgs, const SplitReduceArgs);
#else
template <int D>
__global__ __launch_bounds__(256, 2) void embed_wgrad_fast_group_kernel(const EmbedWgradGroupArgs ea) {
    extern __shared__ __attribute__((aligned(16))) char smem[];
    embed_wgrad_group_body<PREC_BF16, D, 256>(ea, blockIdx.x, smem);
}

static int wgrad_env(const char* name, int dflt) {
    const char* e = getenv(name);
    return e ? atoi(e) : dflt;
}
bool m2m_wgrad_recompute(const m2m_tower* t, int B) {
    static const int on = wgrad_env("M2M_WGRAD_RECOMP", 0);
    if (!on || t->prec != PREC_BF16 || t->D != 128 || t->nblocks < 1 || t->Cp < 64) return false;
    if (m2m_drop_mode(1, t->p_drop) == DM_GEN) return false;
    if (m2m_split_eligible(t, B, 1)) return false;
    return true;
}
extern "C" int m2m_wgrad_form(const m2m_tower* t, int B) { return t && m2m_wgrad_recompute(t, B) ? 1 : 0; }

static bool wgrad_slot_usable(const m2m_tower* t) {
    static const int on = wgrad_env("M2M_WGRAD_SLOT", 1);
    if (!on || t->nblocks < 1) return false;
    for (int b = 0; b < t->nblocks; ++b) {
        const m2m_block& k = t->blk[b];
        if (!t->wslot[b]) return false;
        if (k.g_ch_b1 != k.g_ch_w1 + (long)t->C * t->D || k.g_ch_w2 != k.g_ch_b1 + t->C) return false;
    }
    return true;
}

static int wgrad_use_dma() { static const int on = wgrad_env("M2M_WGRAD_DMA", 1); return on; }

struct WgradPlan { int ntiles, nsl, groups, tpg, rpt, slot; };
static WgradPlan wgrad_plan(const m2m_tower* t, int B, int cols, bool honour_overwrite = true) {
    const bool wide = m2m_is_wide(t);
    const int SPW = wide ? 1 : BM / t->N;
    const int nchain = wide ? (int)(((long)B * t->N + BM - 1) / BM) : (B + SPW - 1) / SPW;
    const int ntiles = (nchain * BM + WBM - 1) / WBM;
    const int nsl = (t->Cp + cols - 1) / cols;
    int groups = 1;
    const int wgs = nsl * t->nblocks;
    while (wgs * groups < 128 && (ntiles + groups - 1) / groups > 64) ++groups;
    if (groups < (32 + wgs - 1) / wgs) groups = (32 + wgs - 1) / wgs;
    if (const char* e = getenv("M2M_WGRAD_GROUPS")) groups = atoi(e);
    if (const char* e = getenv("M2M_WGRAD_LONG_GROUPS")) { if (ntiles > 64) groups = atoi(e); }
    if (honour_overwrite && (t->wgrad_flags & M2M_WGRAD_OVERWRITE)) groups = 1;
    if (groups < 1) groups = 1;
    int tpg = (ntiles + groups - 1) / groups;
    if (tpg < 4) tpg = 4;
    if (tpg > ntiles) tpg = ntiles;
    groups = (ntiles + tpg - 1) / tpg;
    WgradPlan pl;
    pl.ntiles = ntiles; pl.nsl = nsl; pl.groups = groups; pl.tpg = tpg; pl.slot = 0;
    pl.rpt = wide ? BM : SPW * t->N;
    return pl;
}
static int wgrad_cols(const m2m_tower* t, int B) {
    if (m2m_wgrad_recompute(t, B)) return RcGeom<128>::COLS;
    if (t->prec == PREC_BF16 && t->D == 128) return WgradGeom<PREC_BF16, 128>::COLS;
    return t->prec == PREC_BF16 && t->D < 128 ? WG_WAVES * 32 : WG_WAVES * 16;
}
extern "C" int m2m_wgrad_groups(const m2m_tower* t, int B) {
    if (!t || t->nblocks < 1) return 1;
    return wgrad_plan(t, B, wgrad_cols(t, B), false).groups;
}

template <int P, int D, int RCDM>
static int launch_wgrad(const m2m_tower* t, int B, unsigned int seed, unsigned int step, const unsigned int* step_dev, hipStream_t st) {
    typedef WgradKernelGeom<P, D, RCDM> KG;
    const WgradPlan pl = wgrad_plan(t, B, KG::COLS);
    const size_t lds = (size_t)KG::LDS_B;
    auto kern = tower_wgrad_kernel<P, D, RCDM>;
    static bool attr_done = false;
    if (!attr_done) {
        M2M_CHECK_HIP(hipFuncSetAttribute(reinterpret_cast<const void*>(kern), hipFuncAttributeMaxDynamicSharedMemorySize, (int)lds));
        attr_done = true;
    }
    hipLaunchKernelGGL(kern, dim3(pl.nsl, t->nblocks, pl.groups), dim3(KG::THREADS), lds, st, *t, pl.ntiles, pl.tpg, 0, pl.rpt, seed, step,
                       step_dev, wgrad_use_dma());
    M2M_CHECK_HIP(hipGetLastError());
    return 0;
}

static void wgrad_group_plans(const m2m_tower* const* host, int n, int B, int cols, WgradPlan* pl) {
    int min_tpg = 1 << 30;
    WgradPlan nat[WG_MAX_TOWERS];
    for (int i = 0; i < n; ++i) {
        pl[i] = wgrad_plan(host[i], B, cols);
        nat[i] = wgrad_plan(host[i], B, cols, false);
        if (nat[i].tpg < min_tpg) min_tpg = nat[i].tpg;
    }
    for (int i = 0; i < n; ++i) {
        if (n < 2 || !wgrad_slot_usable(host[i])) continue;
        if (nat[i].groups == 2) { pl[i] = nat[i]; pl[i].slot = 1; }
        else if (nat[i].groups == 1 && nat[i].tpg >= 2 * min_tpg && nat[i].tpg >= 32) { pl[i] = nat[i]; pl[i].groups = 2; pl[i].tpg = (pl[i].ntiles + 1) / 2; pl[i].slot = 1; }
    }
}

template <int P, int D, int RCDM>
static int launch_wgrad_group(const m2m_tower* const* host, const m2m_tower* const* dev, int n, const m2m_embed* const* embeds,
                              const float* const* inputs, const float* const* d_x0s, const m2m_tower* const* embed_towers,
                              int nembeds, int B, unsigned int seed, unsigned int step, const unsigned int* step_dev, hipStream_t st,
                              const SplitReduceTower* heads_reduce = nullptr, unsigned int* bump_counter = nullptr) {
    typedef WgradKernelGeom<P, D, RCDM> KG;
    WgradGroupArgs a;
    memset(&a, 0, sizeof(a));
    int njobs = 0, total = 0;
    int order[WG_MAX_TOWERS];
    WgradPlan pl[WG_MAX_TOWERS];
    wgrad_group_plans(host, n, B, KG::COLS, pl);
    for (int i = 0; i < n; ++i) order[i] = i;
    for (int i = 0; i < n; ++i)
        for (int j = i + 1; j < n; ++j)
            if (pl[order[j]].tpg > pl[order[i]].tpg) { const int t = order[i]; order[i] = order[j]; order[j] = t; }
    for (int k = 0; k < n; ++k) {
        const int i = order[k];
        a.tw[i] = dev[i];
        a.ntiles[i] = pl[i].ntiles; a.tpg[i] = pl[i].tpg; a.groups[i] = pl[i].groups; a.nsl[i] = pl[i].nsl; a.slot[i] = pl[i].slot;
        a.rpt[i] = pl[i].rpt;
        for (int b = 0; b < host[i]->nblocks; ++b) {
            if (njobs >= WG_MAX_JOBS) { m2m_set_error("towers_wgrad: more than 32 (tower, block) jobs", __FILE__, __LINE__); return -1; }
            a.job_tower[njobs] = (unsigned char)i;
            a.job_block[njobs] = (unsigned char)b;
            a.job_start[njobs] = (short)total;
            total += pl[i].nsl * pl[i].groups;
            ++njobs;
        }
    }
    if (njobs == 0 && nembeds == 0) return 0;
    if (total > 32000) { m2m_set_error("towers_wgrad: too many workgroups for one launch", __FILE__, __LINE__); return -1; }
    a.job_start[njobs] = (short)total;
    int max_len = 0;
    for (int x = 0, at = 0; x < 8; ++x) {
        const int len = total / 8 + (x < total % 8 ? 1 : 0);
        a.xcd_start[x] = (short)at; a.xcd_len[x] = (short)len;
        at += len;
        if (len > max_len) max_len = len;
    }
    a.njobs = njobs; a.n_tower_wgs = 8 * max_len;
    a.seed = seed; a.step_host = step; a.step_dev = step_dev;
    a.bump_counter = bump_counter;
    a.dma = wgrad_use_dma();
    EmbedWgradGroupArgs ea;
    memset(&ea, 0, sizeof(ea));
    int n_embed_wgs = 0;
    size_t lds_e = 0;
    bool embeds_separately = false;
    if (nembeds) {
        n_embed_wgs = (P == PREC_BF16 && nembeds == EMB_GROUP) ? embed_wgrad_group_args_fast(ea, embeds, inputs, embed_towers, B) : 0;
        if (n_embed_wgs) lds_e = embed_wgrad_fast_lds<D, KG::THREADS>();
        else if (KG::THREADS == 256) { static const int ewgs = wgrad_env("M2M_EMBED_WGS", D >= 256 ? 128 : 512);    n_embed_wgs = embed_wgrad_group_args(ea, embeds, inputs, d_x0s, B, ewgs, nembeds); lds_e = embed_wgrad_lds<D, P>(); }
        else embeds_separately = true;
    }
    if (embeds_separately) {
        if (nembeds == 1) { if (int rc = m2m_embed_wgrad(embeds[0], inputs[0], d_x0s[0], B, (void*)st)) return rc; }
        else if (int rc = m2m_embeds_wgrad(embeds, inputs, d_x0s, nembeds, B, (void*)st)) return rc;
    }
    if constexpr (P == PREC_BF16) {
        static const int merged = wgrad_env("M2M_EMBED_MERGED", 1);
        if (n_embed_wgs && ea.fast && !merged && KG::THREADS != 256) {
            const size_t le = embed_wgrad_fast_lds<D, 256>();
            auto ek = embed_wgrad_fast_group_kernel<D>;
            static bool eattr = false;
            if (!eattr) { M2M_CHECK_HIP(hipFuncSetAttribute(reinterpret_cast<const void*>(ek), hipFuncAttributeMaxDynamicSharedMemorySize, (int)le)); eattr = true; }
            hipLaunchKernelGGL(ek, dim3((unsigned)n_embed_wgs), dim3(256), le, st, ea);
            M2M_CHECK_HIP(hipGetLastError());
            n_embed_wgs = 0; lds_e = 0;
        }
    }
    const size_t lds_t = (size_t)KG::LDS_B;
    const size_t lds = lds_t > lds_e ? lds_t : lds_e;
    auto kern = tower_wgrad_group_kernel<P, D, RCDM>;
    static size_t attr_lds = 0;
    if (lds > attr_lds) {
        M2M_CHECK_HIP(hipFuncSetAttribute(reinterpret_cast<const void*>(kern), hipFuncAttributeMaxDynamicSharedMemorySize, (int)lds));
        attr_lds = lds;
    }
    static const int embed_first = wgrad_env("M2M_EMBED_FIRST", 1);
    if (ea.fast && n_embed_wgs && embed_first) { a.n_embed_first = n_embed_wgs; a.n_embed_pad = (n_embed_wgs + 7) & ~7; n_embed_wgs = 0; }
    SplitReduceArgs ra;
    memset(&ra, 0, sizeof(ra));
    for (int i = 0; i < n; ++i) {
        if (!(host[i]->wgrad_flags & M2M_WGRAD_REDUCES_SMALL)) continue;
        SplitReduceTower x;
        if (!m2m_small_part_deferred(x, host[i], B)) continue;
        if (ra.ntow < SPR_MAX_TOWERS && KG::THREADS % SPR_COLS == 0) { ra.t[ra.ntow++] = x; continue; }
        SplitReduceArgs one;
        memset(&one, 0, sizeof(one));
        one.t[0] = x; one.ntow = 1;
        if (int rc = m2m_split_small_grads(one, st)) return rc;
    }
    if (heads_reduce) {
        if (ra.ntow < SPR_MAX_TOWERS && KG::THREADS % SPR_COLS == 0) ra.t[ra.ntow++] = *heads_reduce;
        else {
            SplitReduceArgs one;
            memset(&one, 0, sizeof(one));
            one.t[0] = *heads_reduce; one.ntow = 1;
            if (int rc = m2m_split_small_grads(one, st)) return rc;
        }
    }
    for (int i = 0; i < ra.ntow; ++i) a.reduce_sets = ra.t[i].nlaunch > a.reduce_sets ? ra.t[i].nlaunch : a.reduce_sets;
    a.n_reduce = SPR_NBX * a.reduce_sets * ra.ntow;
    hipLaunchKernelGGL(kern, dim3((unsigned)(a.n_embed_pad + a.n_tower_wgs + n_embed_wgs + a.n_reduce)), dim3(KG::THREADS), lds, st, a, ea, ra);
    M2M_CHECK_HIP(hipGetLastError());
    return 0;
}

int m2m_check_tower(const m2m_tower* t, int B);

extern "C" int m2m_wgrad_slot_groups(const m2m_tower* const* towers, int ntowers, int B) {
    if (!towers || ntowers < 1 || ntowers > WG_MAX_TOWERS) return 0;
    WgradPlan pl[WG_MAX_TOWERS];
    wgrad_group_plans(towers, ntowers, B, wgrad_cols(towers[0], B), pl);
    int bits = 0;
    for (int i = 0; i < ntowers; ++i) bits |= pl[i].slot << i;
    return bits;
}

extern "C" int m2m_tower_wgrad(const m2m_tower* t, int B, uint32_t seed, uint32_t step, const uint32_t* step_dev, void* stream) {
    if (int rc = m2m_check_tower(t, B)) return rc;
    if (t->nblocks == 0) return 0;
    hipStream_t st = reinterpret_cast<hipStream_t>(stream);
    if (t->wgrad_flags & M2M_WGRAD_REDUCES_SMALL) {
        SplitReduceArgs one;
        memset(&one, 0, sizeof(one));
        if (m2m_small_part_deferred(one.t[0], t, B)) {
            one.ntow = 1;
            if (int rc = m2m_split_small_grads(one, st)) return rc;
        }
    }
    if (m2m_wgrad_recompute(t, B)) {
        if (m2m_drop_mode(1, t->p_drop) == DM_HALF) return launch_wgrad<PREC_BF16, 128, DM_HALF>(t, B, seed, step, step_dev, st);
        return launch_wgrad<PREC_BF16, 128, DM_NONE>(t, B, seed, step, step_dev, st);
    }
#define M2M_WG_CASE(PP, DD) if (t->prec == PP && t->D == DD) return launch_wgrad<PP, DD, -1>(t, B, seed, step, step_dev, st);
    M2M_WG_CASE(PREC_BF16, 32) M2M_WG_CASE(PREC_BF16, 64) M2M_WG_CASE(PREC_BF16, 128) M2M_WG_CASE(PREC_BF16, 256)
    M2M_WG_CASE(PREC_F32, 32) M2M_WG_CASE(PREC_F32, 64) M2M_WG_CASE(PREC_F32, 128) M2M_WG_CASE(PREC_F32, 256)
#undef M2M_WG_CASE
    m2m_set_error("tower_wgrad: unsupported (prec, D)", __FILE__, __LINE__);
    return -1;
}

extern "C" int m2m_heads_part_tiles(int B);
static int towers_wgrad_impl(const m2m_tower* const* towers, const m2m_tower* const* dev_towers, int ntowers,
                             const m2m_embed* const* embeds, const float* const* inputs, const float* const* d_x0s,
                             const m2m_tower* const* embed_towers, int nembeds,
                             int B, uint32_t seed, uint32_t step, const uint32_t* step_dev,
                             const m2m_head* heads, int nheads, int K, void* stream, uint32_t* bump_counter = nullptr) {
    SplitReduceTower hr;
    const SplitReduceTower* heads_reduce = nullptr;
    if (heads && nheads > 0) {
        if (nheads > 3 || K < 2 || !towers || ntowers < 1 || !towers[0]) { m2m_set_error("towers_wgrad_heads: 1..3 heads, K >= 2", __FILE__, __LINE__); return -1; }
        const int D = towers[0]->D, tiles = m2m_heads_part_tiles(B);
        if ((long)K * D + K + 2 > SPP_STRIDE) { m2m_set_error("towers_wgrad_heads: K*D + K + 2 exceeds the slot", __FILE__, __LINE__); return -1; }
        memset(&hr, 0, sizeof(hr));
        for (int h = 0; h < nheads; ++h) {
            if (!heads[h].g_part || !heads[h].g_w || !heads[h].g_b || heads[h].g_part != heads[0].g_part + (long)h * tiles * SPP_STRIDE) {
                m2m_set_error("towers_wgrad_heads: every head needs g_w, g_b and consecutive g_part buffers", __FILE__, __LINE__);
                return -1;
            }
            hr.g_hw[h] = heads[h].g_w; hr.g_hb[h] = heads[h].g_b;
        }
        hr.part = heads[0].g_part; hr.ntiles = tiles; hr.nlaunch = nheads; hr.D = D; hr.head_set0 = 0; hr.nheads = nheads; hr.K = K;
        hr.losses = nullptr;
        heads_reduce = &hr;
    }
    if (!towers || !dev_towers || ntowers < 1 || ntowers > WG_MAX_TOWERS) { m2m_set_error("towers_wgrad: 1..4 towers", __FILE__, __LINE__); return -1; }
    if (nembeds != 0 && (nembeds < 1 || nembeds > EMB_GROUP || !embeds || !inputs || !d_x0s)) {
        m2m_set_error("towers_wgrad: at most two patch embeddings", __FILE__, __LINE__);
        return -1;
    }
    for (int i = 0; i < ntowers; ++i) {
        if (int rc = m2m_check_tower(towers[i], B)) return rc;
        if (!dev_towers[i]) { m2m_set_error("towers_wgrad: missing device-resident descriptor", __FILE__, __LINE__); return -1; }
        if (towers[i]->prec != towers[0]->prec || towers[i]->D != towers[0]->D) {
            m2m_set_error("towers_wgrad: the towers of one launch must share precision and hidden_dim", __FILE__, __LINE__);
            return -1;
        }
        if (m2m_wgrad_recompute(towers[i], B) != m2m_wgrad_recompute(towers[0], B) ||
            (m2m_wgrad_recompute(towers[0], B) && m2m_drop_mode(1, towers[i]->p_drop) != m2m_drop_mode(1, towers[0]->p_drop))) {
            m2m_set_error("towers_wgrad: the towers of one launch must share the weight-gradient form and the dropout mode", __FILE__, __LINE__);
            return -1;
        }
    }
    for (int i = 0; i < nembeds; ++i) {
        if (int rc = m2m_check_embed(embeds[i], B)) return rc;
        if (!inputs[i] || !d_x0s[i]) { m2m_set_error("towers_wgrad: null embedding input", __FILE__, __LINE__); return -1; }
        if (embeds[i]->prec != towers[0]->prec || embeds[i]->D != towers[0]->D) {
            m2m_set_error("towers_wgrad: embeddings must share the towers' precision and hidden_dim", __FILE__, __LINE__);
            return -1;
        }
    }
    hipStream_t st = reinterpret_cast<hipStream_t>(stream);
    const m2m_tower* t = towers[0];
    if (bump_counter && m2m_wgrad_recompute(t, B)) {
        m2m_set_error("towers_wgrad_tail: the recompute form READS the dropout counter in this launch; advance it with m2m_counter_add", __FILE__, __LINE__);
        return -1;
    }
    if (m2m_wgrad_recompute(t, B)) {
        if (m2m_drop_mode(1, t->p_drop) == DM_HALF)
            return launch_wgrad_group<PREC_BF16, 128, DM_HALF>(towers, dev_towers, ntowers, embeds, inputs, d_x0s, embed_towers, nembeds, B, seed, step, step_dev, st, heads_reduce);
        return launch_wgrad_group<PREC_BF16, 128, DM_NONE>(towers, dev_towers, ntowers, embeds, inputs, d_x0s, embed_towers, nembeds, B, seed, step, step_dev, st, heads_reduce);
    }
#define M2M_WGG_CASE(PP, DD) if (t->prec == PP && t->D == DD) return launch_wgrad_group<PP, DD, -1>(towers, dev_towers, ntowers, embeds, inputs, d_x0s, embed_towers, nembeds, B, seed, step, step_dev, st, heads_reduce, bump_counter);
    M2M_WGG_CASE(PREC_BF16, 32) M2M_WGG_CASE(PREC_BF16, 64) M2M_WGG_CASE(PREC_BF16, 128) M2M_WGG_CASE(PREC_BF16, 256)
    M2M_WGG_CASE(PREC_F32, 32) M2M_WGG_CASE(PREC_F32, 64) M2M_WGG_CASE(PREC_F32, 128) M2M_WGG_CASE(PREC_F32, 256)
#undef M2M_WGG_CASE
    m2m_set_error("towers_wgrad: unsupported (prec, D)", __FILE__, __LINE__);
    return -1;
}

extern "C" int m2m_towers_wgrad(const m2m_tower* const* towers, const m2m_tower* const* dev_towers, int ntowers,
                                const m2m_embed* const* embeds, const float* const* inputs, const float* const* d_x0s,
                                const m2m_tower* const* embed_towers, int nembeds,
                                int B, uint32_t seed, uint32_t step, const uint32_t* step_dev, void* stream) {
    return towers_wgrad_impl(towers, dev_towers, ntowers, embeds, inputs, d_x0s, embed_towers, nembeds, B, seed, step, step_dev, nullptr, 0, 0, stream);
}
extern "C" int m2m_towers_wgrad_heads(const m2m_tower* const* towers, const m2m_tower* const* dev_towers, int ntowers,
                                      const m2m_embed* const* embeds, const float* const* inputs, const float* const* d_x0s,
                                      const m2m_tower* const* embed_towers, int nembeds,
                                      int B, uint32_t seed, uint32_t step, const uint32_t* step_dev,
                                      const m2m_head* heads, int nheads, int K, void* stream) {
    return towers_wgrad_impl(towers, dev_towers, ntowers, embeds, inputs, d_x0s, embed_towers, nembeds, B, seed, step, step_dev, heads, nheads, K, stream);
}

extern "C" int m2m_towers_wgrad_tail(const m2m_tower* const* towers, const m2m_tower* const* dev_towers, int ntowers,
                                     const m2m_embed* const* embeds, const float* const* inputs, const float* const* d_x0s,
                                     const m2m_tower* const* embed_towers, int nembeds,
                                     int B, uint32_t seed, uint32_t step, const uint32_t* step_dev,
                                     const m2m_head* heads, int nheads, int K, uint32_t* bump_counter, void* stream) {
    return towers_wgrad_impl(towers, dev_towers, ntowers, embeds, inputs, d_x0s, embed_towers, nembeds, B, seed, step, step_dev, heads, nheads, K, stream, bump_counter);
}

extern "C" int m2m_embeds_wgrad_form(const m2m_embed* const* embeds, const m2m_tower* const* embed_towers, int nembeds, int B) {
    if (!embeds || !embed_towers || nembeds != EMB_GROUP) return 0;
    EmbedWgradGroupArgs ea;
    const float* ins[EMB_GROUP] = {nullptr, nullptr};
    return embed_wgrad_group_args_fast(ea, embeds, ins, embed_towers, B) > 0 ? 1 : 0;
}

__global__ void wgrad_fold_kernel(float* __restrict__ g, const float* __restrict__ s, long n) {
    const long stride = (long)gridDim.x * blockDim.x;
    for (long i = (long)blockIdx.x * blockDim.x + threadIdx.x; i < n; i += stride) g[i] += s[i];
}
extern "C" int m2m_wgrad_fold(const m2m_tower* t, void* stream) {
    if (!t) { m2m_set_error("wgrad_fold: null tower", __FILE__, __LINE__); return -1; }
    if (!wgrad_slot_usable(t)) { m2m_set_error("wgrad_fold: channel gradients are not contiguous", __FILE__, __LINE__); return -1; }
    hipStream_t st = reinterpret_cast<hipStream_t>(stream);
    const long n = 2L * t->C * t->D + t->C;
    for (int b = 0; b < t->nblocks; ++b) {
        hipLaunchKernelGGL(wgrad_fold_kernel, dim3(512), dim3(256), 0, st, t->blk[b].g_ch_w1, t->wslot[b], n);
        M2M_CHECK_HIP(hipGetLastError());
    }
    return 0;
}
#endif
```

m2_mixer_amd/engine.py:

```python
from __future__ import annotations

from collections import OrderedDict
from typing import Dict, List, Optional, Sequence, Tuple

import ctypes as C
import os

import torch

from . import _lib as L
from . import config
from .runtime import (AdamPackPlan, BLOCK_FIELDS, BLOCK_KEYS, EmbedRuntime, MlpRuntime, TowerRuntime, block_param_shapes, heads_bce,
                      heads_ce, can_group, can_group_embeds, can_pack_all, embeds_forward, pack_all,
                      towers_backward, towers_forward, towers_forward_embeds_ok, towers_wgrad, wgrad_slot_groups)


def config_fused_update(n_params: int = 0) -> bool:
    env = os.environ.get("M2M_FUSED_UPDATE")
    if env is not None:
        return env == "1"
    return n_params > 0


def _num_patch(c: dict) -> int:
# ... 561 lines not shown
                    self.optimizer_step(scale, getattr(grad_sync, "reduced_bf16", None))
        torch.cuda.current_stream().wait_stream(s)
        torch.cuda.synchronize()
        for dst, src in zip(state, snap):
            dst.copy_(src)
        self.pack()
        torch.cuda.synchronize()
        g1 = torch.cuda.CUDAGraph()
        out_losses = self.losses
        if grad_sync is None:
            if steps > 1:
                home = (self.losses, self.logits, self.preds)
                self.losses_steps = torch.zeros(steps, *self.losses.shape, device=self.device)
                self.logits_steps = torch.zeros(steps, *self.logits.shape, device=self.device)
                self.preds_steps = torch.zeros(steps, *self.preds.shape, dtype=self.preds.dtype, device=self.device)
                out_losses = self.losses_steps
            with torch.cuda.graph(g1, capture_error_mode="thread_local"):
                for i in range(steps):
                    if steps > 1:
                        self.losses, self.logits, self.preds = self.losses_steps[i], self.logits_steps[i], self.preds_steps[i]
                    self.fused_step(*slots[i])
            if steps > 1:
                self.losses, self.logits, self.preds = home
            graphs = (g1,)
        elif getattr(grad_sync, "pipelined", False):
            with torch.cuda.graph(g1, capture_error_mode="thread_local"):
                self.forward_backward(*st)
            chunk_graphs = []
            for k in range(len(self._update_chunks())):
                gk = torch.cuda.CUDAGraph()
                with torch.cuda.graph(gk, capture_error_mode="thread_local"):
                    self._update_one_chunk(k, scale)
                chunk_graphs.append(gk)
            self._slots_folded = False
            graphs = (g1, *chunk_graphs)
        else:
            g2 = torch.cuda.CUDAGraph()
            with torch.cuda.graph(g1, capture_error_mode="thread_local"):
                self.forward_backward(*st)
            with torch.cuda.graph(g2, capture_error_mode="thread_local"):
                self.optimizer_step(scale, getattr(grad_sync, "reduced_bf16", None))
            graphs = (g1, g2)
        self._graph = graphs
        pipelined = grad_sync is not None and getattr(grad_sync, "pipelined", False)

        def replay(*new_batch):
            if new_batch and new_batch[0] is not None:
                if len(new_batch) != nb * steps:
                    raise ValueError(f"replay expects {nb * steps} tensors ({steps} step(s) x {nb}), got {len(new_batch)}")
                for i in range(steps):
                    for dst, src in zip(slots[i], new_batch[i * nb:(i + 1) * nb]):
                        dst.copy_(src, non_blocking=True)
            graphs[0].replay()
            if pipelined:
                grad_sync.start(self.flat_g, [(lo, hi) for lo, hi, _ in self._update_chunks()])
                for k in range(len(graphs) - 1):
                    grad_sync.wait(k)
                    graphs[1 + k].replay()
            elif grad_sync is not None:
                grad_sync(self.flat_g)
                graphs[1].replay()
            return out_losses

        replay.losses = out_losses
        return replay


class _TwoTowerEngine(_FlatEngine):

    MODS: Tuple[str, str] = ("image", "audio")

    def _param_shapes(self, cfg):
        return two_tower_param_shapes(cfg, self.MODS)

    def _segment_of(self, k: str) -> str:
        a, b = self.MODS
        return a if k.startswith(f"{a}_mixer.") else (b if k.startswith(f"{b}_mixer.") else "fusion")

    def _build(self):
        a, b = self.MODS
        cfg = self.cfg
        ca, cb, cm = cfg[a], cfg[b], cfg["multimodal"]
        self.D = ca["hidden_dim"]
        self.fusion_name = fusion_function_name(cm)
        self.concat = self.fusion_name == "ConcatFusion"
        if not (cb["hidden_dim"] == self.D == cm["hidden_dim"]):
            raise RuntimeError(f"both towers and the fusion mixer must share hidden_dim ({self.fusion_name} on dim 1)")
        if self.fusion_name == "BiModalGatedUnit" and not (cm["mod1_in"] == cm["mod2_in"] == cm["out_size"] == self.D):
            raise RuntimeError(f"multimodal.mod1_in / mod2_in / out_size = {cm['mod1_in']} / {cm['mod2_in']} / {cm['out_size']}: "
                               f"the engine's BiModalGatedUnit takes and gives the towers' hidden_dim {self.D} (one D for the heads)")
        self.Na, self.Nb = _num_patch(ca), _num_patch(cb)
        self.Nf = fusion_tokens(cm, self.Na, self.Nb)
        self.t_a = self._make_tower(f"{a}_mixer.", ca, self.Na, 0)
        self.t_b = self._make_tower(f"{b}_mixer.", cb, self.Nb, 1024)
        self.t_fus = self._make_tower("fusion_mixer.", cm, self.Nf, 2048)

        def make_embed(prefix, c):
            e = EmbedRuntime(c["in_channels"], c["image_size"][0], c["image_size"][1], c["patch_size"], c["patch_size"],
                             self.D, self.prec)
            e.bind_params(self.params[prefix + "to_patch_embedding.0.weight"], self.params[prefix + "to_patch_embedding.0.bias"])
            e.bind_grads(self.grads[prefix + "to_patch_embedding.0.weight"], self.grads[prefix + "to_patch_embedding.0.bias"])
            return e

        self.e_a = make_embed(f"{a}_mixer.", ca)
        self.e_b = make_embed(f"{b}_mixer.", cb)
        B, D, dev = self.B, self.D, self.device
        f = lambda *s: torch.zeros(*s, device=dev)
        grouped = can_group_embeds(self.e_a, self.e_b) and can_group(self.t_a, self.t_b, self.B)
        self.x0_splits = (self.e_a.fwd_splits(), self.e_b.fwd_splits()) if grouped and not self.t_a.wide else (1, 1)
        self._x0_a, self._x0_b = f(self.x0_splits[0], B * self.Na, D), f(self.x0_splits[1], B * self.Nb, D)
        self.x0_a, self.x0_b = self._x0_a[0], self._x0_b[0]
        self.fused, self.fus_out = f(B, self.Nf, D), f(B, self.Nf, D)
        self.pool_a, self.pool_b, self.pool_fus = f(B, D), f(B, D), f(B, D)
        self.dpool_a, self.dpool_b, self.dpool_fus = f(B, D), f(B, D), f(B, D)
        self.d_fused = f(B, self.Nf, D)
        self.dx0_a, self.dx0_b = f(B * self.Na, D), f(B * self.Nb, D)
        self._build_fusion()
        self.preds = torch.zeros(self._preds_shape(), dtype=torch.int32, device=dev)
        self._early_fus_wgrad = (self.concurrent and self.t_fus.wide and B * self.Nf <= 8192 and
                                 os.environ.get("M2M_EARLY_FUSION_WGRAD", "0") == "1")
        self._setup_wgrad([[self.t_fus], [self.t_a, self.t_b]] if self._early_fus_wgrad else [[self.t_fus, self.t_a, self.t_b]])
        self._fused_heads = self._heads_are_ce() and self.t_fus.backward_heads_ok(B, 3, self.K)
        self._heads_pool = (self.t_a.wide and self.t_b.wide and self.t_fus.wide and os.environ.get("M2M_HEADS_POOL", "1") != "0")
        self.t_fus.set_wgrad_reduces_small(not self._fused_heads and os.environ.get("M2M_DEFER_SMALL", "1") != "0")
        self._head_part, self._wgrad_heads = None, None
        if (self._heads_are_ce() and not self._fused_heads and os.environ.get("M2M_HEAD_SLOTS", "1") != "0"
                and self.K * D + self.K + 2 <= L.SPLIT_GPART):
            self._head_part = torch.zeros(3, int(L.lib().m2m_heads_part_tiles(B)), L.SPLIT_GPART, device=dev)
        if (os.environ.get("M2M_GROUP_SLOTS", "1") != "0" and self.t_a.has_small_slots() and self.t_b.has_small_slots()
                and can_group(self.t_a, self.t_b, self.B)):
            for t in (self.t_a, self.t_b):
                t.set_wgrad_group_slots(True)
                t.set_wgrad_reduces_small(True)
        self._embed_towers = []
        if os.environ.get("M2M_EMBED_FAST", "1") != "0" and self.t_a.enable_dx0_image(B) and self.t_b.enable_dx0_image(B):
            self._embed_towers = [self.t_a, self.t_b]
            import ctypes as C
            ep = (C.POINTER(L.Embed) * 2)(C.pointer(self.e_a.desc), C.pointer(self.e_b.desc))
            tp = (C.POINTER(L.Tower) * 2)(C.pointer(self.t_a.desc), C.pointer(self.t_b.desc))
            fast = bool(L.lib().m2m_embeds_wgrad_form(ep, tp, 2, B))
            if fast and os.environ.get("M2M_WGRAD_OVERWRITE", "1") != "0" and len(self._ranges_add) + 2 <= L.MAX_GRAD_RANGES:
                for e, pre in ((self.e_a, f"{a}_mixer."), (self.e_b, f"{b}_mixer.")):
                    gw = self.grads[pre + "to_patch_embedding.0.weight"]
                    e.set_wgrad_overwrite(True)
                    self._ranges_add.append(((gw.data_ptr() - self.flat_g.data_ptr()) // 4, gw.numel(), None, 1))
                self._ranges_add.sort(key=lambda r: r[0])
                self._ranges_keep = [(lo, n, None, k) for lo, n, _, k in self._ranges_add]

        self._embed_fold = (os.environ.get("M2M_EMBED_FOLD", "0") == "1" and grouped and self.concurrent and not self._early_fus_wgrad
                            and self.x0_splits is not None and self.e_a.prec == self.t_a.prec and self.e_a.D == self.t_a.D
                            and towers_forward_embeds_ok([self.t_a, self.t_b], [self.e_a, self.e_b], B)
                            and self.t_a.wgrad_form(B) == 0 and self.t_fus.wgrad_form(B) == 0)
        self._pending_bump = False

    def _build_fusion(self):
        B, D, dev = self.B, self.D, self.device
        self.out_a = self.out_b = self.d_out_a = self.d_out_b = None
        self.gate = None
        if self.concat:
            return
        f = lambda *s: torch.zeros(*s, device=dev)
        self.out_a, self.out_b = f(B, self.Na, D), f(B, self.Nb, D)
        if self.fusion_name == "SumFusion":
            self.d_out_a = self.d_out_b = self.d_fused
        else:
            self.d_out_a, self.d_out_b = f(B, self.Na, D), f(B, self.Nb, D)
        if self.fusion_name != "BiModalGatedUnit":
            return
        rows = B * self.Nf
        self._gate_bufs = dict(t1=f(rows, D), t2=f(rows, D), z=f(rows, D), dh=f(rows, 3 * D),
                               part=f(int(L.lib().m2m_gate_part_floats(rows, D))))
        g = L.Gate()
        g.D = D
        P, G = self.params, self.grads
        for fld, key in (("w1", "mod1_hidden.weight"), ("b1", "mod1_hidden.bias"), ("w2", "mod2_hidden.weight"),
                         ("b2", "mod2_hidden.bias"), ("wz", "z_hidden.weight"), ("bz", "z_hidden.bias")):
            setattr(g, fld, P["fusion_function." + key].data_ptr())
            setattr(g, "g_" + fld, G["fusion_function." + key].data_ptr())
        for fld, t in self._gate_bufs.items():
            setattr(g, fld, t.data_ptr())
        self.gate = g

    def _tower_outputs(self):
        D = self.D
        if self.concat:
            return self.fused, self.fused.view(-1)[self.Na * D:], self.Nf * D
        return self.out_a, self.out_b, None

    def _fusion_forward(self, training: bool):
        rows = self.B * self.Nf
        if self.concat:
            return
        if self.gate is not None:
            L.check(L.lib().m2m_gate_forward(C.byref(self.gate), self.out_a.data_ptr(), self.out_b.data_ptr(), self.fused.data_ptr(),
                                             rows, int(training), L.stream_ptr()), "gate_forward")
        else:
            L.check(L.lib().m2m_fusion_forward(_ELEM_FUSION_MODE[self.fusion_name], self.out_a.data_ptr(), self.out_b.data_ptr(),
                                               self.fused.data_ptr(), rows * self.D, L.stream_ptr()), "fusion_forward")

    def _fusion_backward(self):
        rows = self.B * self.Nf
        if self.concat or self.fusion_name == "SumFusion":
            return
        if self.gate is not None:
            L.check(L.lib().m2m_gate_backward(C.byref(self.gate), self.d_fused.data_ptr(), self.d_out_a.data_ptr(),
                                              self.d_out_b.data_ptr(), rows, L.stream_ptr()), "gate_backward")
            L.check(L.lib().m2m_gate_wgrad(C.byref(self.gate), self.out_a.data_ptr(), self.out_b.data_ptr(), rows, L.stream_ptr()),
                    "gate_wgrad")
        else:
            L.check(L.lib().m2m_fusion_backward(_ELEM_FUSION_MODE[self.fusion_name], self.out_a.data_ptr(), self.out_b.data_ptr(),
                                                self.d_fused.data_ptr(), self.d_out_a.data_ptr(), self.d_out_b.data_ptr(),
                                                rows * self.D, L.stream_ptr()), "fusion_backward")

    def _preds_shape(self):
        return (3, self.B)

    def pack(self):
        towers, embeds = [self.t_a, self.t_b, self.t_fus], [self.e_a, self.e_b]
        if can_pack_all(towers, embeds):
            pack_all(towers, embeds)
            return
        for m in towers + embeds:
            m.pack(force=True)

    def _loss_heads(self, heads, labels, zero_losses):
        raise NotImplementedError

    def _heads_are_ce(self) -> bool:
        return False

    def _forward(self, xa, xb, labels, training: bool, with_grad: bool, prologue: bool = False):
        B, D = self.B, self.D
        sd = self.drop_step if training else None
        fs = self.Nf * D
        out_a, b_part, ts = self._tower_outputs()
        sa_, sb_ = (ts, ts) if self.concat else (self.Na * D, self.Nb * D)
        main, side, _ = self._streams()
        so = 0
        pa, pb, pf = (None, None, None) if self._heads_pool else (self.pool_a, self.pool_b, self.pool_fus)
        self._pending_bump = False
        if self._embed_fold and training and prologue:
            so, self._pending_bump = 1, True
            towers_forward([self.t_a, self.t_b],
                           [(self.x0_a, self.Na * D, out_a, sa_, pa), (self.x0_b, self.Nb * D, b_part, sb_, pb)],
                           B, training, self.seed, so, sd, embeds=[self.e_a, self.e_b], inputs=[xa, xb],
                           head=(self.adam_state, self.losses))
        elif self.concurrent and can_group(self.t_a, self.t_b, self.B):
            sa, sb = self.x0_splits
            if can_group_embeds(self.e_a, self.e_b):
                head = (self.adam_state, self.drop_step, self.losses) if prologue else None
                embeds_forward([self.e_a, self.e_b], [xa, xb], [self._x0_a, self._x0_b], B, [sa, sb], head)
            else:
                if prologue:
                    self._prologue()
                sa = sb = 1
                self.e_a.forward(xa, B, self.x0_a)
                self.e_b.forward(xb, B, self.x0_b)
            towers_forward([self.t_a, self.t_b],
                           [(self.x0_a, self.Na * D, out_a, sa_, pa, sa, B * self.Na * D),
                            (self.x0_b, self.Nb * D, b_part, sb_, pb, sb, B * self.Nb * D)],
                           B, training, self.seed, 0, sd)
        else:
            if prologue:
                self._prologue()
            side.wait_stream(main)
            with torch.cuda.stream(side):
                self.e_b.forward(xb, B, self.x0_b)
                self.t_b.forward(self.x0_b, self.Nb * D, B, b_part, sb_, pb, training, self.seed, 0, sd)
            self.e_a.forward(xa, B, self.x0_a)
            self.t_a.forward(self.x0_a, self.Na * D, B, out_a, sa_, pa, training, self.seed, 0, sd)
            main.wait_stream(side)
        self._fusion_forward(training and with_grad)
        self.t_fus.forward(self.fused, fs, B, self.fus_out, fs, pf, training, self.seed, so, sd)
        a, b = self.MODS
        hw = self.head_weights
        heads = [self._head(a, self.pool_a, self.dpool_a, hw[a], with_grad),
                 self._head(b, self.pool_b, self.dpool_b, hw[b], with_grad),
                 self._head("fusion", self.pool_fus, self.dpool_fus, hw["fusion"], with_grad)]
        if self._heads_pool:
            heads[0]["tokens"] = (out_a, self.Na, sa_)
            heads[1]["tokens"] = (b_part.data_ptr(), self.Nb, sb_)
            heads[2]["tokens"] = (self.fus_out, self.Nf, fs)
        self._wgrad_heads = None
        if training and with_grad and self._head_part is not None:
            for i, h in enumerate(heads):
                h["g_part"] = self._head_part[i]
            self._wgrad_heads = heads
        self._heads = heads
        self._labels = labels
        if training and with_grad and self._fused_heads:
            return
        self._loss_heads(heads, labels, not training)

    def _backward(self, xa, xb, fused_update: bool = False):
        B, D = self.B, self.D
        fs = self.Nf * D
        sd = self.drop_step
        a, b = self.MODS
        so = 1 if self._pending_bump else 0
        if self._fused_heads:
            self.t_fus.backward_heads(B, self._heads, 2, self._labels, self.K, (self.logits, self.losses, self.preds),
                                      self.d_fused, fs, self.seed, so, sd)
        else:
            self.t_fus.backward(B, None, 0, self.dpool_fus, self.d_fused, fs, self.seed, so, sd)
        if self.concat:
            d_a_part, d_b_part, sa_, sb_ = self.d_fused, self.d_fused.view(-1)[self.Na * D:], fs, fs
        else:
            self._fusion_backward()
            d_a_part, d_b_part, sa_, sb_ = self.d_out_a, self.d_out_b, self.Na * D, self.Nb * D
        main, s_a, s_f = self._streams()
        wg_towers = [self.t_fus, self.t_a, self.t_b]
        if self._early_fus_wgrad:
            s_f.wait_stream(main)
            with torch.cuda.stream(s_f):
                self.t_fus.wgrad(B, self.seed, so, sd)
            wg_towers = [self.t_a, self.t_b]
        s_e = self.s_emb if self.concurrent else main
        if self.concurrent and can_group(self.t_a, self.t_b, self.B):
            towers_backward([self.t_a, self.t_b],
                            [(d_a_part, sa_, self.dpool_a, self.dx0_a, self.Na * D), (d_b_part, sb_, self.dpool_b, self.dx0_b, self.Nb * D)],
                            B, self.seed, so, sd)
        else:
            s_a.wait_stream(main)
            with torch.cuda.stream(s_a):
                self.t_a.backward(B, d_a_part, sa_, self.dpool_a, self.dx0_a, self.Na * D, self.seed, so, sd)
            self.t_b.backward(B, d_b_part, sb_, self.dpool_b, self.dx0_b, self.Nb * D, self.seed, so, sd)
            main.wait_stream(s_a)
        bump = self.drop_step if self._pending_bump else None
        if can_group_embeds(self.e_a, self.e_b) and self.e_a.prec == self.t_a.prec and self.e_a.D == self.t_a.D:
            towers_wgrad(wg_towers, B, [self.e_a, self.e_b], [xa, xb], [self.dx0_a, self.dx0_b],
                         seed=self.seed, step=so, step_dev=sd, embed_towers=self._embed_towers, heads=self._wgrad_heads, K=self.K,
                         bump=bump)
        else:
            if bump is not None:
                raise RuntimeError("the embedding fold needs the merged weight-gradient launch (it advances the dropout counter)")
            s_e.wait_stream(main)
            with torch.cuda.stream(s_e):
                self.e_b.wgrad(xb, self.dx0_b, B)
                self.e_a.wgrad(xa, self.dx0_a, B)
            towers_wgrad(wg_towers, B, seed=self.seed, step=so, step_dev=sd, heads=self._wgrad_heads, K=self.K)
            main.wait_stream(s_e)
        self._pending_bump = False
        if self._early_fus_wgrad:
            main.wait_stream(s_f)
        if fused_update:
            self._update(1.0)

    def _adam_pack_modules(self):
        towers, embeds = [self.t_a, self.t_b, self.t_fus], [self.e_a, self.e_b]
        return (towers, embeds) if can_pack_all(towers, embeds) else None

    def _update_chunks(self):
        a, b = self.MODS
        mods = {a: [self.t_a, self.e_a], b: [self.t_b, self.e_b], "fusion": [self.t_fus]}
        segs = sorted(self.segments.items(), key=lambda kv: kv[1][0])
        return [(lo, hi, mods[name]) for name, (lo, hi) in segs]

    @torch.no_grad()
    def evaluate(self, xa, xb, labels, scores: Optional[ScoreTable] = None):
        self._forward(xa, xb, labels, False, False)
        if scores is not None:
            scores.add(self.preds, labels)
        a, b = self.MODS
        return {"logits": self.logits[2], f"{a}_logits": self.logits[0], f"{b}_logits": self.logits[1],
                f"loss_{a}": self.losses[0], f"loss_{b}": self.losses[1], "loss_fusion": self.losses[2],
                "loss": self.losses[3], "preds": self.preds[2], f"preds_{a}": self.preds[0], f"preds_{b}": self.preds[1]}


class AVMnistEngine(_TwoTowerEngine):

    MODS = ("image", "audio")

    def __init__(self, cfg: dict, batch_size: int, device="cuda:0", precision: Optional[str] = None,
                 lr: float = 1e-2, betas=(0.9, 0.999), eps: float = 1e-8, weight_decay: float = 0.0,
                 fusion_loss_weight: float = 1.0 / 3, seed: int = 42, init: bool = True, share=None, scores: bool = False):
        w = fusion_loss_weight
        ow = (1 - w) / 2
        self.head_weights = {"image": 3 * ow, "audio": 3 * ow, "fusion": 3 * w}
        self.fusion_loss_weight = w
        super().__init__(cfg, batch_size, device, precision, lr, betas, eps, weight_decay, seed, init, share, scores)

    HEAD_NAMES = ("image", "audio", "fusion")
    SCORES_TASK = "avmnist"

    def set_fusion_loss_weight(self, w: float):
        ow = (1 - w) / 2
        self.set_loss_weights(3 * ow, 3 * ow, 3 * w)
        self.fusion_loss_weight = w

    def _loss_heads(self, heads, labels, zero_losses):
        heads_ce(heads, labels, self.B, self.D, self.K, out=(self.logits, self.losses, self.preds), zero_losses=zero_losses,
                 weights=self.loss_weights)

    def _heads_are_ce(self) -> bool:
        return True

    t_img = property(lambda self: self.t_a)
    t_aud = property(lambda self: self.t_b)
    e_img = property(lambda self: self.e_a)
    e_aud = property(lambda self: self.e_b)
    s_aud = property(lambda self: self.s_b)
    Ni = property(lambda self: self.Na)
    x0_img = property(lambda self: self.x0_a)


class MMIMDBEngine(_TwoTowerEngine):

    MODS = ("image", "text")
    HEAD_NAMES = ("image", "text", "fusion")
    SCORES_TASK = "mmimdb"
    EXTRA_STATE_KEYS = ("image_criterion.pos_weight", "text_criterion.pos_weight", "fusion_criterion.pos_weight")

    def __init__(self, cfg: dict, batch_size: int, device="cuda:0", precision: Optional[str] = None,
                 lr: float = 1e-3, betas=(0.9, 0.999), eps: float = 1e-8, weight_decay: float = 0.0,
                 seed: int = 42, init: bool = True, share=None, scores: bool = False):
        self.head_weights = {"image": 1.0, "text": 1.0, "fusion": 1.0}
        super().__init__(cfg, batch_size, device, precision, lr, betas, eps, weight_decay, seed, init, share, scores)
        self.pos_weight = torch.tensor(cfg["pos_weight"], dtype=torch.float32, device=self.device)
        if self.pos_weight.numel() != self.K:
            raise RuntimeError("pos_weight needs one entry per class")

    def _consume_extra_state(self, key, value):
        v = value.to(self.device, torch.float32).reshape(-1)
        if v.numel() != self.K:
            raise RuntimeError(f"{key}: expected {self.K} entries")
        if key == self.EXTRA_STATE_KEYS[0]:
            self.pos_weight.copy_(v)
        elif not torch.equal(v, self.pos_weight):
            raise RuntimeError(f"{key} differs from image_criterion.pos_weight: the fused heads kernel takes one pos_weight")

    def _extra_state(self):
        return OrderedDict((k, self.pos_weight.detach().clone()) for k in self.EXTRA_STATE_KEYS)

    def _preds_shape(self):
        return (3, self.B, self.K)

    def _loss_heads(self, heads, labels, zero_losses):
        heads_bce(heads, labels, self.pos_weight, self.B, self.D, self.K, out=(self.logits, self.losses, self.preds),
                  zero_losses=zero_losses, weights=self.loss_weights)


class MimicEngine(_FlatEngine):

    def __init__(self, cfg: dict, batch_size: int, device="cuda:0", precision: Optional[str] = None,
                 lr: float = 1e-2, betas=(0.9, 0.999), eps: float = 1e-8, weight_decay: float = 0.0,
                 fusion_loss_weight: float = 1.0 / 3, seed: int = 42, init: bool = True, share=None, scores: bool = False):
        w = fusion_loss_weight
        ow = (1 - w) / 2
        self.head_weights = {"static": ow, "time": ow, "fusion": w}
        self.fusion_loss_weight = w
        super().__init__(cfg, batch_size, device, precision, lr, betas, eps, weight_decay, seed, init, share, scores)

    HEAD_NAMES = ("static", "time", "fusion")
    SCORES_TASK = "mimic"

    def set_fusion_loss_weight(self, w: float):
        ow = (1 - w) / 2
        self.set_loss_weights(ow, ow, w)
        self.fusion_loss_weight = w

    def _param_shapes(self, cfg):
        return mimic_param_shapes(cfg)

    def _segment_of(self, k: str) -> str:
        return "time" if k.startswith("time_mixer.") else ("static" if k.startswith("static_extractor.") else "fusion")

    def _build(self):
        cfg = self.cfg
        ct, cs, cm = cfg["time"], cfg["static"], cfg["multimodal"]
        self.D = ct["hidden_dim"]
        if not (ct["proj_dim"] == self.D == cm["hidden_dim"] == cs["output_dim"]):
            raise RuntimeError("time hidden_dim / proj_dim, static output_dim and fusion hidden_dim must agree")
        self.Nt = ct["num_patch"]
        self.Nf = 1 + self.Nt
        mode = os.environ.get("M2M_MIMIC_STREAMS", "none" if self.B <= 1024 else "both")
        self._merged_tail = os.environ.get("M2M_MIMIC_MERGED_TAIL", "1") != "0"
        self._conc_fwd, self._conc_bwd = mode in ("fwd", "both"), mode in ("bwd", "both")
        self._heads_pool = os.environ.get("M2M_HEADS_POOL", "1") != "0"
        self._mlp_ride = os.environ.get("M2M_MLP_RIDE", "1") != "0" and self.B <= 2048
        self.t_time = self._make_tower("time_mixer.", ct, self.Nt, 0)
        self.t_fus = self._make_tower("fusion_mixer.", cm, self.Nf, 2048)
        self.e_time = EmbedRuntime(1, self.Nt, ct["embedding_dim"], 1, ct["embedding_dim"], self.D, self.prec)
        self.e_time.bind_params(self.params["time_mixer.proj.weight"], self.params["time_mixer.proj.bias"])
        self.e_time.bind_grads(self.grads["time_mixer.proj.weight"], self.grads["time_mixer.proj.bias"])
        nb = cs["num_blocks"]
# ... 111 lines not shown
```

m2_mixer_amd/runtime.py:

```python
from __future__ import annotations

import ctypes as C
from typing import Dict, List, Optional, Sequence

import torch

from . import _lib as L

BLOCK_KEYS = {
    "ln1_w": "token_mix.0.weight", "ln1_b": "token_mix.0.bias",
    "tok_w1": "token_mix.2.net.0.weight", "tok_b1": "token_mix.2.net.0.bias",
    "tok_w2": "token_mix.2.net.3.weight", "tok_b2": "token_mix.2.net.3.bias",
    "ln2_w": "channel_mix.0.weight", "ln2_b": "channel_mix.0.bias",
    "ch_w1": "channel_mix.1.net.0.weight", "ch_b1": "channel_mix.1.net.0.bias",
    "ch_w2": "channel_mix.1.net.3.weight", "ch_b2": "channel_mix.1.net.3.bias",
}
BLOCK_FIELDS = list(BLOCK_KEYS.keys())


def block_param_shapes(D: int, N: int, T: int, Cc: int) -> Dict[str, tuple]:
    return {"ln1_w": (D,), "ln1_b": (D,), "tok_w1": (T, N), "tok_b1": (T,), "tok_w2": (N, T), "tok_b2": (N,),
            "ln2_w": (D,), "ln2_b": (D,), "ch_w1": (Cc, D), "ch_b1": (Cc,), "ch_w2": (D, Cc), "ch_b2": (D,)}


# ... 229 lines not shown
    def wgrad_form(self, B: int) -> int:
        return int(L.lib().m2m_wgrad_form(C.byref(self.desc), B))

    def wgrad_groups(self, B: int) -> int:
        return int(L.lib().m2m_wgrad_groups(C.byref(self.desc), B))

    def channel_grad_ranges(self, flat_g: torch.Tensor):
        out = []
        cd = self.C * self.D
        base, end = flat_g.data_ptr(), flat_g.data_ptr() + flat_g.numel() * 4
        for i in range(self.nblocks):
            b = self.desc.blk[i]
            w1, b1, w2 = b.g_ch_w1, b.g_ch_b1, b.g_ch_w2
            if not w1 or b1 != w1 + 4 * cd or w2 != b1 + 4 * self.C or w1 < base or w2 + 4 * cd > end:
                return None
            out.append(((w1 - base) // 4, 2 * cd + self.C))
        return out

    def alloc_wslot(self, flat_g: torch.Tensor) -> bool:
        rng = self.channel_grad_ranges(flat_g)
        if rng is None or self.nblocks == 0:
            return False
        n = rng[0][1]
        buf = torch.zeros(self.nblocks * (n + 8), device=self.device)
        views = []
        off = 0
        for i, (lo, _) in enumerate(rng):
            while (off - lo) % 4:
                off += 1
            v = buf[off:off + n]
            self.desc.wslot[i] = v.data_ptr()
            views.append(v)
            off += n
        self._keep["wslot"] = (buf, views)
        return True

    def clear_wslot(self):
        for i in range(L.MAX_BLOCKS):
            self.desc.wslot[i] = None
        self._keep.pop("wslot", None)

    def wslot_views(self):
        return self._keep["wslot"][1] if "wslot" in self._keep else None

    def set_wgrad_overwrite(self, on: bool):
        self.desc.wgrad_flags = (self.desc.wgrad_flags | L.WGRAD_OVERWRITE) if on else (self.desc.wgrad_flags & ~L.WGRAD_OVERWRITE)

    def set_wgrad_reduces_small(self, on: bool):
        self.desc.wgrad_flags = (self.desc.wgrad_flags | L.WGRAD_REDUCES_SMALL) if on else (self.desc.wgrad_flags & ~L.WGRAD_REDUCES_SMALL)

    def has_small_slots(self) -> bool:
        return (not self.wide and self.prec == L.PREC_BF16 and self.D == 128 and self.nblocks > 0
                and 2 * self.T * self.N + self.T + self.N <= 576)

    def set_wgrad_group_slots(self, on: bool):
        self.desc.wgrad_flags = (self.desc.wgrad_flags | L.WGRAD_GROUP_SLOTS) if on else (self.desc.wgrad_flags & ~L.WGRAD_GROUP_SLOTS)

    def wgrad_fold(self):
        L.check(L.lib().m2m_wgrad_fold(C.byref(self.desc), L.stream_ptr()), "wgrad_fold")

    def backward_heads_ok(self, B: int, nheads: int, K: int) -> bool:
        return bool(L.lib().m2m_tower_backward_heads_ok(C.byref(self.desc), B, nheads, K))

    def backward_heads(self, B: int, heads: Sequence[dict], own: int, labels: torch.Tensor, K: int, out, d_x0: torch.Tensor,
                       d_x0_ss: int, seed: int, step: int, step_dev: Optional[torch.Tensor] = None):
        arr = _head_array(heads)
        logits, losses, preds = out
        L.check(L.lib().m2m_tower_backward_heads(C.byref(self.desc), B, arr, len(heads), own, labels.data_ptr(), K, logits.data_ptr(),
                                                 losses.data_ptr(), preds.data_ptr(), d_x0.data_ptr(), d_x0_ss, seed & 0xFFFFFFFF,
                                                 step & 0xFFFFFFFF, L.ptr(step_dev), L.stream_ptr()), "tower_backward_heads")

    def wgrad(self, B: int, seed: int, step: int, step_dev: Optional[torch.Tensor] = None):
        L.check(L.lib().m2m_tower_wgrad(C.byref(self.desc), B, seed & 0xFFFFFFFF, step & 0xFFFFFFFF, L.ptr(step_dev),
                                        L.stream_ptr()), "tower_wgrad")

    def device_desc(self) -> int:
        raw = bytes(self.desc)
        if self._keep.get("desc_bytes") != raw:
            self._keep["desc_dev"] = torch.frombuffer(bytearray(raw), dtype=torch.uint8).to(self.device)
            self._keep["desc_bytes"] = raw
        return self._keep["desc_dev"].data_ptr()

    def dropout_mask(self, blk: int, site: int, B: int, seed: int, step: int) -> torch.Tensor:
        n = {0: B * self.D * self.T, 1: B * self.D * self.N, 2: B * self.N * self.Cp, 3: B * self.N * self.D}[site]
        m = torch.empty(n, dtype=torch.uint8, device=self.device)
        L.check(L.lib().m2m_dropout_mask(C.byref(self.desc), blk, site, B, seed & 0xFFFFFFFF, step & 0xFFFFFFFF,
                                         m.data_ptr(), L.stream_ptr()), "dropout_mask")
        return m


def can_group(a: TowerRuntime, b: TowerRuntime, B: Optional[int] = None) -> bool:
    if B is not None:
        return bool(L.lib().m2m_towers_can_group(C.byref(a.desc), C.byref(b.desc), B))
    return (not a.wide and not b.wide and a.prec == b.prec and a.D == b.D and a.desc.p_drop == b.desc.p_drop
            and (a.N <= 4) == (b.N <= 4) and (a.T % 16 == 0) == (b.T % 16 == 0) and a.nblocks <= 4 and b.nblocks <= 4)


def towers_forward_embeds_ok(towers: Sequence[TowerRuntime], embeds: Sequence["EmbedRuntime"], B: int) -> bool:
    n = len(towers)
    host = (C.POINTER(L.Tower) * n)(*[C.pointer(t.desc) for t in towers])
    ep = (C.POINTER(L.Embed) * n)(*[C.pointer(e.desc) for e in embeds])
    return bool(L.lib().m2m_towers_forward_embeds_ok(host, n, ep, B))


def towers_forward(towers: Sequence[TowerRuntime], ios: Sequence[tuple], B: int, training: bool, seed: int, step: int,
                   step_dev: Optional[torch.Tensor] = None, embeds: Sequence["EmbedRuntime"] = (), inputs: Sequence[torch.Tensor] = (),
                   head: Optional[tuple] = None):
    n = len(towers)
    for t in towers:
        if training:
            t.ensure_buffers(B)
        t.ensure_workspace(B)
    host = (C.POINTER(L.Tower) * n)(*[C.pointer(t.desc) for t in towers])
    io = (L.TowerIO * n)()
    for i, (x0, x0_ss, out, out_ss, pooled, *parts) in enumerate(ios):
        io[i].x0, io[i].x0_ss, io[i].out, io[i].out_ss, io[i].pooled = x0.data_ptr(), x0_ss, out.data_ptr(), out_ss, L.ptr(pooled)
        io[i].x0_parts, io[i].x0_part_stride = parts if parts else (1, 0)
    if len(embeds):
        ep = (C.POINTER(L.Embed) * n)(*[C.pointer(e.desc) for e in embeds])
        ip = (C.c_void_p * n)(*[t.data_ptr() for t in inputs])
        hd = None
        if head is not None:
            hd = L.StepHead()
            hd.adam_state, hd.drop_counter, hd.losses, hd.nlosses = L.ptr(head[0]), None, L.ptr(head[1]), int(head[1].numel())
        L.check(L.lib().m2m_towers_forward_embeds(host, io, n, ep, ip, C.byref(hd) if hd is not None else None, B, int(training),
                                                  seed & 0xFFFFFFFF, step & 0xFFFFFFFF, L.ptr(step_dev), L.stream_ptr()),
                "towers_forward_embeds")
        return
    L.check(L.lib().m2m_towers_forward(host, io, n, B, int(training), seed & 0xFFFFFFFF, step & 0xFFFFFFFF, L.ptr(step_dev),
                                       L.stream_ptr()), "towers_forward")


def towers_backward(towers: Sequence[TowerRuntime], ios: Sequence[tuple], B: int, seed: int, step: int,
                    step_dev: Optional[torch.Tensor] = None):
    n = len(towers)
    host = (C.POINTER(L.Tower) * n)(*[C.pointer(t.desc) for t in towers])
    io = (L.TowerGIO * n)()
    for i, (d_out, d_out_ss, d_pooled, d_x0, d_x0_ss) in enumerate(ios):
        io[i].d_out, io[i].d_out_ss, io[i].d_pooled = L.ptr(d_out), d_out_ss, L.ptr(d_pooled)
        io[i].d_x0, io[i].d_x0_ss = d_x0.data_ptr(), d_x0_ss
    L.check(L.lib().m2m_towers_backward(host, io, n, B, seed & 0xFFFFFFFF, step & 0xFFFFFFFF, L.ptr(step_dev), L.stream_ptr()),
            "towers_backward")


def wgrad_slot_groups(towers: Sequence[TowerRuntime], B: int) -> int:
    n = len(towers)
    host = (C.POINTER(L.Tower) * n)(*[C.pointer(t.desc) for t in towers])
    return int(L.lib().m2m_wgrad_slot_groups(host, n, B))


def towers_wgrad(towers: Sequence[TowerRuntime], B: int, embeds: Sequence["EmbedRuntime"] = (),
                 inputs: Sequence[torch.Tensor] = (), d_x0s: Sequence[torch.Tensor] = (), seed: int = 0, step: int = 0,
                 step_dev: Optional[torch.Tensor] = None, embed_towers: Sequence[TowerRuntime] = (),
                 heads: Optional[Sequence[dict]] = None, K: int = 0, bump: Optional[torch.Tensor] = None):
    n, ne = len(towers), len(embeds)
    host = (C.POINTER(L.Tower) * n)(*[C.pointer(t.desc) for t in towers])
    dev = (C.c_void_p * n)(*[t.device_desc() for t in towers])
    ep = (C.POINTER(L.Embed) * max(ne, 1))(*[C.pointer(e.desc) for e in embeds])
    ip = (C.c_void_p * max(ne, 1))(*[t.data_ptr() for t in inputs])
    dp = (C.c_void_p * max(ne, 1))(*[t.data_ptr() for t in d_x0s])
    et = (C.POINTER(L.Tower) * max(ne, 1))(*[C.pointer(t.desc) for t in embed_towers]) if len(embed_towers) == ne and ne else None
    if bump is not None:
        L.check(L.lib().m2m_towers_wgrad_tail(host, dev, n, ep, ip, dp, et, ne, B, seed & 0xFFFFFFFF, step & 0xFFFFFFFF,
                                              L.ptr(step_dev), _head_array(heads) if heads else None, len(heads) if heads else 0, K,
                                              bump.data_ptr(), L.stream_ptr()), "towers_wgrad_tail")
        return
    if heads:
        L.check(L.lib().m2m_towers_wgrad_heads(host, dev, n, ep, ip, dp, et, ne, B, seed & 0xFFFFFFFF, step & 0xFFFFFFFF,
                                               L.ptr(step_dev), _head_array(heads), len(heads), K, L.stream_ptr()), "towers_wgrad_heads")
        return
    L.check(L.lib().m2m_towers_wgrad(host, dev, n, ep, ip, dp, et, ne, B, seed & 0xFFFFFFFF, step & 0xFFFFFFFF, L.ptr(step_dev),
                                     L.stream_ptr()), "towers_wgrad")


def can_pack_all(towers: Sequence[TowerRuntime], embeds: Sequence["EmbedRuntime"]) -> bool:
    precs = {t.prec for t in towers} | {e.prec for e in embeds}
    return len(towers) <= 3 and len(embeds) <= 2 and len(precs) == 1 and all(t.nblocks <= 4 for t in towers)


def pack_all(towers: Sequence[TowerRuntime], embeds: Sequence["EmbedRuntime"]):
    nt, ne = len(towers), len(embeds)
    tp = (C.POINTER(L.Tower) * max(nt, 1))(*[C.pointer(t.desc) for t in towers])
    ep = (C.POINTER(L.Embed) * max(ne, 1))(*[C.pointer(e.desc) for e in embeds])
    L.check(L.lib().m2m_pack_all(tp, nt, ep, ne, L.stream_ptr()), "pack_all")
    for t in towers:
        t.mark_packed()
    for e in embeds:
        e.mark_packed()


class AdamPackPlan:

    def __init__(self, towers: Sequence[TowerRuntime], embeds: Sequence["EmbedRuntime"], flat_p, flat_g, grad_bf16, flat_m, flat_v,
                 state, betas, eps: float, weight_decay: float, grad_scale: float, ranges=None):
        self.towers, self.embeds = list(towers), list(embeds)
        nt, ne = len(towers), len(embeds)
        self._tp = (C.POINTER(L.Tower) * max(nt, 1))(*[C.pointer(t.desc) for t in towers])
        self._ep = (C.POINTER(L.Embed) * max(ne, 1))(*[C.pointer(e.desc) for e in embeds])
        nbytes = int(L.lib().m2m_adam_pack_plan_bytes())
        self.host = C.create_string_buffer(nbytes)
        ranges = list(ranges or [])
        arr = (L.GradRange * max(len(ranges), 1))()
        for i, (rlo, rn, add, keep) in enumerate(ranges):
            arr[i].lo, arr[i].n, arr[i].add, arr[i].keep = rlo, rn, L.ptr(add), int(keep)
        L.check(L.lib().m2m_adam_pack_plan_ranges(self._tp, nt, self._ep, ne, flat_p.data_ptr(), flat_g.data_ptr(), L.ptr(grad_bf16),
                                                  flat_m.data_ptr(), flat_v.data_ptr(), flat_p.numel(), state.data_ptr(), betas[0], betas[1],
                                                  eps, weight_decay, abs(grad_scale), arr, len(ranges), self.host), "adam_pack_plan_ranges")
        self.dev = torch.frombuffer(bytearray(self.host.raw), dtype=torch.uint8).to(flat_p.device)
        self._keep = (flat_p, flat_g, grad_bf16, flat_m, flat_v, state, [r[2] for r in ranges])

    def run(self):
        L.check(L.lib().m2m_adam_pack_all(self._tp, len(self.towers), self._ep, len(self.embeds), self.dev.data_ptr(), self.host,
                                          L.stream_ptr()), "adam_pack_all")
        for t in self.towers:
            t.mark_packed()
        for e in self.embeds:
            e.mark_packed()


class EmbedRuntime:

    def __init__(self, Cin: int, H: int, W: int, ph: int, pw: int, D: int, prec: int):
        self.desc = L.Embed()
        d = self.desc
        kb = 32 if prec == L.PREC_BF16 else 16
        K = Cin * ph * pw
        d.prec, d.Cin, d.H, d.W, d.ph, d.pw, d.D, d.K = prec, Cin, H, W, ph, pw, D, K
        d.Kp = (K + kb - 1) // kb * kb
        self.N = (H // ph) * (W // pw)
        self.D, self.K, self.prec = D, K, prec
        self._keep = {}
        self._packed_for = None

    def bind_params(self, w: torch.Tensor, b: torch.Tensor):
        if not w.is_cuda:
            raise RuntimeError("patch embedding: m2_mixer_amd runs on the GPU only; there is no CPU path")
        if w.dtype != torch.float32 or not w.is_contiguous() or w.numel() != self.D * self.K:
            raise RuntimeError(f"embedding weight: expected contiguous float32 with {self.D * self.K} elements")
        self.desc.w, self.desc.b = w.data_ptr(), b.data_ptr()
        self._keep["w"], self._keep["b"] = w, b
        self._packed_for = None
        if "wn" not in self._keep:
            wn = torch.zeros(L.packed_bytes(self.prec, self.D, self.desc.Kp), dtype=torch.uint8, device=w.device)
            self.desc.wn = wn.data_ptr()
            self._keep["wn"] = wn

    def params_changed(self, w, b) -> bool:
        return w.data_ptr() != self.desc.w or b.data_ptr() != self.desc.b

    def mark_packed(self):
        self._packed_for = self._keep["w"]._version

    def invalidate(self):
        self._packed_for = None

    def pack(self, force: bool = False):
        if force or self._keep["w"]._version != self._packed_for:
            L.check(L.lib().m2m_pack_embed(C.byref(self.desc), L.stream_ptr()), "pack_embed")
            self.mark_packed()

    def bind_grads(self, g_w: torch.Tensor, g_b: torch.Tensor):
        self.desc.g_w, self.desc.g_b = g_w.data_ptr(), g_b.data_ptr()
        self._keep["g"] = (g_w, g_b)

    def set_wgrad_overwrite(self, on: bool):
        self.desc.wgrad_flags = L.WGRAD_OVERWRITE if on else 0

    def fwd_splits(self) -> int:
        return int(L.lib().m2m_embed_fwd_splits(C.byref(self.desc)))

    def forward(self, inp: torch.Tensor, B: int, x0: torch.Tensor, step_head: Optional[tuple] = None):
        head = None
        if step_head is not None:
            adam_state, drop_counter, losses = step_head
            head = C.byref(L.StepHead(adam_state.data_ptr(), drop_counter.data_ptr(), losses.data_ptr(), losses.numel()))
        L.check(L.lib().m2m_embed_forward_head(C.byref(self.desc), inp.data_ptr(), B, x0.data_ptr(), head, L.stream_ptr()),
                "embed_forward")

    def wgrad(self, inp: torch.Tensor, d_x0: torch.Tensor, B: int):
        L.check(L.lib().m2m_embed_wgrad(C.byref(self.desc), inp.data_ptr(), d_x0.data_ptr(), B, L.stream_ptr()),
                "embed_wgrad")


def can_group_embeds(a: EmbedRuntime, b: EmbedRuntime) -> bool:
    return a.prec == b.prec and a.D == b.D


def embeds_forward(embeds: Sequence[EmbedRuntime], inputs: Sequence[torch.Tensor], x0s: Sequence[torch.Tensor], B: int,
                   nsplits: Optional[Sequence[int]] = None, step_head: Optional[tuple] = None):
    n = len(embeds)
    ep = (C.POINTER(L.Embed) * n)(*[C.pointer(e.desc) for e in embeds])
    ip = (C.c_void_p * n)(*[t.data_ptr() for t in inputs])
    xp = (C.c_void_p * n)(*[t.data_ptr() for t in x0s])
    ns = (C.c_int * n)(*(nsplits if nsplits is not None else [1] * n))
    ps = (C.c_int64 * n)(*[B * e.N * e.D for e in embeds])
    head = None
    if step_head is not None:
        adam_state, drop_counter, losses = step_head
        head = C.byref(L.StepHead(adam_state.data_ptr(), drop_counter.data_ptr(), losses.data_ptr(), losses.numel()))
    L.check(L.lib().m2m_embeds_forward(ep, ip, xp, ns, ps, n, B, head, L.stream_ptr()), "embeds_forward")


def embeds_wgrad(embeds: Sequence[EmbedRuntime], inputs: Sequence[torch.Tensor], d_x0s: Sequence[torch.Tensor], B: int):
    n = len(embeds)
    ep = (C.POINTER(L.Embed) * n)(*[C.pointer(e.desc) for e in embeds])
    ip = (C.c_void_p * n)(*[t.data_ptr() for t in inputs])
    dp = (C.c_void_p * n)(*[t.data_ptr() for t in d_x0s])
    L.check(L.lib().m2m_embeds_wgrad(ep, ip, dp, n, B, L.stream_ptr()), "embeds_wgrad")


class MlpRuntime:

    def __init__(self, dims: Sequence[int], has_out: bool, p_drop: float, site_base: int = 0):
        nl = len(dims) - 1
        if nl < 1 or nl > L.MLP_MAX_LAYERS:
            raise RuntimeError(f"MLP: 1..{L.MLP_MAX_LAYERS} Linear layers supported, got {nl}")
        self.dims, self.nlayers, self.has_out = list(dims), nl, bool(has_out)
        self.desc = L.Mlp()
        d = self.desc
        d.nlayers, d.has_out, d.p_drop, d.site_base = nl, int(self.has_out), float(p_drop), site_base
        for i, w in enumerate(dims):
            d.dims[i] = int(w)
        self._keep: Dict[str, object] = {}
        self._B = 0

    def bind(self, params: Sequence[tuple], grads: Optional[Sequence[tuple]], B: int):
        for i, (w, b) in enumerate(params):
            _check_tensor(w, (self.dims[i + 1], self.dims[i]), f"mlp layer {i} weight")
            _check_tensor(b, (self.dims[i + 1],), f"mlp layer {i} bias")
            self.desc.w[i], self.desc.b[i] = w.data_ptr(), b.data_ptr()
        if grads is not None:
            for i, (gw, gb) in enumerate(grads):
                self.desc.g_w[i], self.desc.g_b[i] = gw.data_ptr(), gb.data_ptr()
        self._keep["params"], self._keep["grads"] = list(params), grads
        self.ensure_buffers(B, params[0][0].device)

    def ensure_buffers(self, B: int, device):
        if B == self._B:
            return
        self.use_acts([torch.zeros(B, self.dims[i + 1], device=device) for i in range(self.nlayers)])
        self._B = B

    def fresh_acts(self, B: int, device) -> list:
        acts = [torch.zeros(B, self.dims[i + 1], device=device) for i in range(self.nlayers)]
        self.use_acts(acts)
        self._B = B
        return acts

    def use_acts(self, acts: list):
        for i, a in enumerate(acts):
            self.desc.act[i] = a.data_ptr()
        self._keep["act"] = acts

    def forward(self, x: torch.Tensor, B: int, out: torch.Tensor, out_ss: int, out_dense: Optional[torch.Tensor],
                training: bool, seed: int, step: int, step_dev: Optional[torch.Tensor] = None):
        _check_tensor(x, (B, self.dims[0]), "mlp input")
        self.ensure_buffers(B, x.device)
        L.check(L.lib().m2m_mlp_forward(C.byref(self.desc), x.data_ptr(), B, out.data_ptr(), out_ss, L.ptr(out_dense),
                                        int(training), seed & 0xFFFFFFFF, step & 0xFFFFFFFF, L.ptr(step_dev),
                                        L.stream_ptr()), "mlp_forward")

    def backward(self, x: torch.Tensor, B: int, d_out: Optional[torch.Tensor], d_out_ss: int,
                 d_out_dense: Optional[torch.Tensor]):
        L.check(L.lib().m2m_mlp_backward(C.byref(self.desc), x.data_ptr(), B, L.ptr(d_out), d_out_ss, L.ptr(d_out_dense),
                                         L.stream_ptr()), "mlp_backward")

    def forward_ride(self, x: torch.Tensor, B: int, out: torch.Tensor, out_ss: int, out_dense: Optional[torch.Tensor],
                     training: bool, seed: int, step: int, step_dev: Optional[torch.Tensor] = None):
        _check_tensor(x, (B, self.dims[0]), "mlp input")
        self.ensure_buffers(B, x.device)
        L.check(L.lib().m2m_mlp_forward_ride(C.byref(self.desc), x.data_ptr(), B, out.data_ptr(), out_ss, L.ptr(out_dense),
                                             int(training), seed & 0xFFFFFFFF, step & 0xFFFFFFFF, L.ptr(step_dev)), "mlp_forward_ride")

    def backward_ride(self, x: torch.Tensor, B: int, d_out: Optional[torch.Tensor], d_out_ss: int,
                      d_out_dense: Optional[torch.Tensor]):
        L.check(L.lib().m2m_mlp_backward_ride(C.byref(self.desc), x.data_ptr(), B, L.ptr(d_out), d_out_ss, L.ptr(d_out_dense)),
                "mlp_backward_ride")

    @staticmethod
    def ride_flush():
        L.check(L.lib().m2m_mlp_ride_flush(L.stream_ptr()), "mlp_ride_flush")


def _head_array(heads: Sequence[dict]):
    nh = len(heads)
    arr = (L.Head * nh)()
    for i, h in enumerate(heads):
        arr[i].pooled, arr[i].w, arr[i].b = L.ptr(h.get("pooled")), h["w"].data_ptr(), h["b"].data_ptr()
        tok = h.get("tokens")
        if tok is not None:
            arr[i].tokens = tok[0] if isinstance(tok[0], int) else tok[0].data_ptr()
            arr[i].ntok, arr[i].tok_sample_stride = int(tok[1]), int(tok[2])
        elif h.get("pooled") is None:
            raise ValueError("a head needs `pooled` or `tokens`")
        arr[i].g_w, arr[i].g_b, arr[i].d_pooled = L.ptr(h.get("g_w")), L.ptr(h.get("g_b")), L.ptr(h.get("d_pooled"))
        arr[i].weight = float(h["weight"])
        arr[i].g_part = L.ptr(h.get("g_part"))
    return arr


def _check_weights(weights: Optional[torch.Tensor], nh: int):
    if weights is not None and (not weights.is_cuda or weights.dtype != torch.float32 or weights.numel() < nh
                                or not weights.is_contiguous()):
        raise ValueError(f"head weights: a contiguous float32 device tensor of at least {nh} entries")


def heads_bce(heads: Sequence[dict], targets: torch.Tensor, pos_weight: torch.Tensor, B: int, D: int, K: int, out=None,
              zero_losses: bool = True, weights: Optional[torch.Tensor] = None):
    nh = len(heads)
    _check_weights(weights, nh)
    arr = _head_array(heads)
    _check_tensor(targets, (B, K), "BCE targets")
    dev = targets.device
    if out is not None:
        logits, losses, preds = out
    else:
        logits = torch.empty(nh, B, K, device=dev)
        losses = torch.empty(nh + 1, device=dev)
        preds = torch.empty(nh, B, K, dtype=torch.int32, device=dev)
    if weights is not None:
        L.check(L.lib().m2m_heads_bce_w(arr, nh, targets.data_ptr(), pos_weight.data_ptr(), B, D, K, logits.data_ptr(),
                                        losses.data_ptr(), preds.data_ptr(), int(zero_losses), weights.data_ptr(), L.stream_ptr()),
                "heads_bce_w")
    else:
        L.check(L.lib().m2m_heads_bce(arr, nh, targets.data_ptr(), pos_weight.data_ptr(), B, D, K, logits.data_ptr(),
                                      losses.data_ptr(), preds.data_ptr(), int(zero_losses), L.stream_ptr()), "heads_bce")
    return logits, losses, preds


def heads_ce(heads: Sequence[dict], labels: torch.Tensor, B: int, D: int, K: int, out=None, zero_losses: bool = True,
             weights: Optional[torch.Tensor] = None):
    nh = len(heads)
    _check_weights(weights, nh)
    arr = _head_array(heads)
    dev = labels.device
    if out is not None:
        logits, losses, preds = out
    else:
        logits = torch.empty(nh, B, K, device=dev)
        losses = torch.empty(nh + 1, device=dev)
        preds = torch.empty(nh, B, dtype=torch.int32, device=dev)
    if weights is not None:
        L.check(L.lib().m2m_heads_ce_w(arr, nh, labels.data_ptr(), B, D, K, logits.data_ptr(), losses.data_ptr(),
                                       preds.data_ptr(), int(zero_losses), weights.data_ptr(), L.stream_ptr()), "heads_ce_w")
    else:
        L.check(L.lib().m2m_heads_ce(arr, nh, labels.data_ptr(), B, D, K, logits.data_ptr(), losses.data_ptr(),
                                     preds.data_ptr(), int(zero_losses), L.stream_ptr()), "heads_ce")
    return logits, losses, preds
```

Before: 1.058 million.

## Stash bf16 patch matrix in forward and reuse it in embedding weight-gradient

During the fused embedding forward, the bf16-packed patch fragments are also written with nontemporal stores into a per-embedding workspace. The embedding weight-gradient then reads this contiguous bf16 patch matrix through a new p16 kernel body (LDS staging with swizzle and transposed reads) instead of re-gathering and converting the fp32 image patches. The aim is to cut redundant fp32 gathers and conversions in backward, at the cost of extra forward write traffic, workspace memory and added API plumbing. It is on by default and controlled by the M2M_EMBED_P16 environment variable.

```diff
diff --git a/include/m2mixer.h b/include/m2mixer.h
--- a/include/m2mixer.h
+++ b/include/m2mixer.h
@@ -107,6 +107,10 @@
 int m2m_embeds_forward(const m2m_embed* const* embeds, const float* const* inputs, float* const* x0s, const int* nsplits,
                        const int64_t* part_strides, int nembeds, int B, const m2m_step_head* head, void* stream);
 int m2m_embed_fwd_splits(const m2m_embed* e);
+int64_t m2m_embed_p16_bytes(const m2m_embed* e, const float* input, int B);
+int m2m_embeds_forward_p16(const m2m_embed* const* embeds, const float* const* inputs, float* const* x0s, const int* nsplits,
+                           const int64_t* part_strides, int nembeds, int B, const m2m_step_head* head,
+                           void* const* p16s, const int64_t* p16_bytes, void* stream);
 int m2m_embed_forward_head(const m2m_embed* e, const float* input, int B, float* x0, const m2m_step_head* head, void* stream);
 
 int m2m_tower_forward(const m2m_tower* t, const float* x0, int64_t x0_sample_stride, int B,
@@ -188,6 +192,12 @@
                           const m2m_tower* const* embed_towers, int nembeds,
                           int B, uint32_t seed, uint32_t step, const uint32_t* step_dev,
                           const m2m_head* heads, int nheads, int K, uint32_t* bump_counter, void* stream);
+int m2m_towers_wgrad_p16(const m2m_tower* const* towers, const m2m_tower* const* dev_towers, int ntowers,
+                         const m2m_embed* const* embeds, const float* const* inputs, const float* const* d_x0s,
+                         const m2m_tower* const* embed_towers, int nembeds,
+                         int B, uint32_t seed, uint32_t step, const uint32_t* step_dev,
+                         const m2m_head* heads, int nheads, int K, uint32_t* bump_counter,
+                         const void* const* p16s, void* stream);
 
 int m2m_tower_backward_heads_ok(const m2m_tower* t, int B, int nheads, int K);
 int m2m_tower_backward_heads(const m2m_tower* t, int B, const m2m_head* heads, int nheads, int own, const int64_t* labels,
diff --git a/m2_mixer_amd/_lib.py b/m2_mixer_amd/_lib.py
--- a/m2_mixer_amd/_lib.py
+++ b/m2_mixer_amd/_lib.py
@@ -144,6 +144,12 @@
     "m2m_embeds_forward": (C.c_int, [C.POINTER(C.POINTER(Embed)), C.POINTER(_fp), C.POINTER(_fp), C.POINTER(C.c_int), C.POINTER(C.c_int64),
                                      C.c_int, C.c_int, C.POINTER(StepHead), _fp]),
     "m2m_embed_fwd_splits": (C.c_int, [C.POINTER(Embed)]),
+    "m2m_embed_p16_bytes": (C.c_int64, [C.POINTER(Embed), _fp, C.c_int]),
+    "m2m_embeds_forward_p16": (C.c_int, [C.POINTER(C.POINTER(Embed)), C.POINTER(_fp), C.POINTER(_fp), C.POINTER(C.c_int), C.POINTER(C.c_int64),
+                                         C.c_int, C.c_int, C.POINTER(StepHead), C.POINTER(_fp), C.POINTER(C.c_int64), _fp]),
+    "m2m_towers_wgrad_p16": (C.c_int, [C.POINTER(C.POINTER(Tower)), C.POINTER(_fp), C.c_int, C.POINTER(C.POINTER(Embed)), C.POINTER(_fp),
+                                       C.POINTER(_fp), C.POINTER(C.POINTER(Tower)), C.c_int, C.c_int, C.c_uint32, C.c_uint32, _fp,
+                                       C.POINTER(Head), C.c_int, C.c_int, _fp, C.POINTER(_fp), _fp]),
     "m2m_heads_ce": (C.c_int, [C.POINTER(Head), C.c_int, _fp, C.c_int, C.c_int, C.c_int, _fp, _fp, _fp, C.c_int, _fp]),
     "m2m_step_prologue": (C.c_int, [_fp, _fp, _fp, C.c_int, _fp]),
     "m2m_heads_bce": (C.c_int, [C.POINTER(Head), C.c_int, _fp, _fp, C.c_int, C.c_int, C.c_int, _fp, _fp, _fp, C.c_int, _fp]),
diff --git a/m2_mixer_amd/csrc/embed.hip b/m2_mixer_amd/csrc/embed.hip
--- a/m2_mixer_amd/csrc/embed.hip
+++ b/m2_mixer_amd/csrc/embed.hip
@@ -24,6 +24,7 @@
     long M[2];
     int N[2], nwg0, fast[2], nsplit[2];
     long part_stride[2];
+    char* p16[2];
     float* adam_state;
     unsigned int* drop_counter;
     float* losses;
@@ -42,7 +43,7 @@
     const int wg = e ? blockIdx.x - a.nwg0 : blockIdx.x;
     if (P == PREC_BF16 && a.fast[e]) {
         const int ns = a.nsplit[e], split = wg % ns;
-        embed_fwd_fast_body<D>(a.em[e], a.in[e], a.M[e], a.N[e], a.x0[e] + split * a.part_stride[e], wg / ns, split, ns, smem);
+        embed_fwd_fast_body<D>(a.em[e], a.in[e], a.M[e], a.N[e], a.x0[e] + split * a.part_stride[e], wg / ns, split, ns, smem, a.p16[e]);
     }
     else {
         const int ns = a.nsplit[e], split = wg % ns, tile = wg / ns;
@@ -102,7 +103,8 @@
 }
 template <int P, int D>
 static int launch_embed_fwd_group(const m2m_embed* const* es, const float* const* ins, float* const* x0s, const int* nsplits,
-                                  const int64_t* part_strides, const m2m_step_head* head, int B, hipStream_t st) {
+                                  const int64_t* part_strides, const m2m_step_head* head, int B, hipStream_t st,
+                                  void* const* p16s = nullptr) {
     constexpr int RB = 16;
     EmbedFwdGroupArgs a;
     memset(&a, 0, sizeof(a));
@@ -117,6 +119,7 @@
         const int N = (es[i]->H / es[i]->ph) * (es[i]->W / es[i]->pw);
         a.em[k] = *es[i]; a.in[k] = ins[i]; a.x0[k] = x0s[i]; a.N[k] = N; a.M[k] = (long)B * N;
         a.fast[k] = embed_fwd_fast_ok(es[i], ins[i]);
+        a.p16[k] = p16s ? (char*)p16s[i] : nullptr;
         a.nsplit[k] = nsplits ? nsplits[i] : 1;
         a.part_stride[k] = part_strides ? (long)part_strides[i] : 0;
         if (a.nsplit[k] < 1 || a.nsplit[k] > 4 || (a.nsplit[k] > 1 && a.part_stride[k] < a.M[k] * (long)D)) {
@@ -213,8 +216,38 @@
     return pays ? 2 : 1;
 }
 
+extern "C" int64_t m2m_embed_p16_bytes(const m2m_embed* e, const float* input, int B) {
+    if (!e || !input || B < 1 || e->ph < 1 || e->pw < 1 || !m2m_embed_p16_on() || !embed_fwd_fast_ok(e, input) || e->K % 8) return 0;
+    const int64_t N = (int64_t)(e->H / e->ph) * (e->W / e->pw);
+    return (int64_t)B * N * ((e->K + 7) & ~7) * 2;
+}
+
+static int embeds_forward_impl(const m2m_embed* const* embeds, const float* const* inputs, float* const* x0s, const int* nsplits,
+                               const int64_t* part_strides, int nembeds, int B, const m2m_step_head* head, void* const* p16s,
+                               void* stream);
 extern "C" int m2m_embeds_forward(const m2m_embed* const* embeds, const float* const* inputs, float* const* x0s, const int* nsplits,
                                   const int64_t* part_strides, int nembeds, int B, const m2m_step_head* head, void* stream) {
+    return embeds_forward_impl(embeds, inputs, x0s, nsplits, part_strides, nembeds, B, head, nullptr, stream);
+}
+extern "C" int m2m_embeds_forward_p16(const m2m_embed* const* embeds, const float* const* inputs, float* const* x0s, const int* nsplits,
+                                      const int64_t* part_strides, int nembeds, int B, const m2m_step_head* head,
+                                      void* const* p16s, const int64_t* p16_bytes, void* stream) {
+    if (p16s) {
+        if (!embeds || !inputs || !p16_bytes || nembeds != 2) { m2m_set_error("embeds_forward_p16: exactly two embeddings", __FILE__, __LINE__); return -1; }
+        for (int i = 0; i < nembeds; ++i) {
+            if (!p16s[i]) continue;
+            const int64_t need = m2m_embed_p16_bytes(embeds[i], inputs[i], B);
+            if (need == 0 || p16_bytes[i] < need || ((uintptr_t)p16s[i] & 15)) {
+                m2m_set_error("embeds_forward_p16: a 16-byte aligned workspace of m2m_embed_p16_bytes() bytes, for embeddings that function accepts", __FILE__, __LINE__);
+                return -1;
+            }
+        }
+    }
+    return embeds_forward_impl(embeds, inputs, x0s, nsplits, part_strides, nembeds, B, head, p16s, stream);
+}
+static int embeds_forward_impl(const m2m_embed* const* embeds, const float* const* inputs, float* const* x0s, const int* nsplits,
+                               const int64_t* part_strides, int nembeds, int B, const m2m_step_head* head, void* const* p16s,
+                               void* stream) {
     if (!embeds || !inputs || !x0s || nembeds != 2) { m2m_set_error("embeds_forward: exactly two embeddings", __FILE__, __LINE__); return -1; }
     for (int i = 0; i < nembeds; ++i) {
         if (int rc = m2m_check_embed(embeds[i], B)) return rc;
@@ -225,7 +258,7 @@
     }
     hipStream_t st = reinterpret_cast<hipStream_t>(stream);
     const m2m_embed* e = embeds[0];
-#define M2M_EFG_CASE(PP, DD) if (e->prec == PP && e->D == DD) return launch_embed_fwd_group<PP, DD>(embeds, inputs, x0s, nsplits, part_strides, head, B, st);
+#define M2M_EFG_CASE(PP, DD) if (e->prec == PP && e->D == DD) return launch_embed_fwd_group<PP, DD>(embeds, inputs, x0s, nsplits, part_strides, head, B, st, p16s);
     M2M_EFG_CASE(PREC_BF16, 32) M2M_EFG_CASE(PREC_BF16, 64) M2M_EFG_CASE(PREC_BF16, 128) M2M_EFG_CASE(PREC_BF16, 256)
     M2M_EFG_CASE(PREC_F32, 32) M2M_EFG_CASE(PREC_F32, 64) M2M_EFG_CASE(PREC_F32, 128) M2M_EFG_CASE(PREC_F32, 256)
 #undef M2M_EFG_CASE
diff --git a/m2_mixer_amd/csrc/embed_fwd.h b/m2_mixer_amd/csrc/embed_fwd.h
--- a/m2_mixer_amd/csrc/embed_fwd.h
+++ b/m2_mixer_amd/csrc/embed_fwd.h
@@ -115,7 +115,8 @@
 #endif
 template <int D>
 static __device__ __forceinline__ void embed_fwd_fast_body(const m2m_embed& em, const float* __restrict__ in, long M, int N,
-                                                           float* __restrict__ x0, int wg, int split, int nsplit, char* smem) {
+                                                           float* __restrict__ x0, int wg, int split, int nsplit, char* smem,
+                                                           char* __restrict__ p16 = nullptr) {
     typedef Prec<PREC_BF16> Pr;
     constexpr int KSB = EMB_FKS / 32, DT = D / 16, DPW = (DT + NWAVES - 1) / NWAVES, IMG_B = 16 * EMB_FKS * 2;
     static_assert(KSB == NWAVES, "one k-block of the stage per wave");
@@ -125,6 +126,7 @@
     const long m0 = (long)wg * 16;
     const long rb = patch_rowbase(pg, m0 + il, M);
     const int nKB = em.Kp / 32;
+    char* const p16_row = p16 ? p16 + ((m0 + il) * (long)((em.K + 7) & ~7) + wave * 32 + 8 * g) * 2 : nullptr;
     const int nst_all = (em.Kp + EMB_FKS - 1) / EMB_FKS;
     const int per = (nst_all + nsplit - 1) / nsplit;
     const int st_begin = split * per, nst = min(nst_all, st_begin + per);
@@ -154,6 +156,7 @@
         f.u[0] = pack_bf2(p.p0[0], p.p0[1]); f.u[1] = pack_bf2(p.p0[2], p.p0[3]);
         f.u[2] = pack_bf2(p.p1[0], p.p1[1]); f.u[3] = pack_bf2(p.p1[2], p.p1[3]);
         if (!valid) f.u = u32x4_t{0u, 0u, 0u, 0u};
+        else if (p16_row) __builtin_nontemporal_store(f.u, reinterpret_cast<u32x4_t*>(p16_row + (long)st * (EMB_FKS * 2)));
         char* cur = img + ((st - st_begin) & 1) * IMG_B;
         *reinterpret_cast<u32x4_t*>(cur + tid * 16) = f.u;
         __syncthreads();
diff --git a/m2_mixer_amd/csrc/embed_wgrad.h b/m2_mixer_amd/csrc/embed_wgrad.h
--- a/m2_mixer_amd/csrc/embed_wgrad.h
+++ b/m2_mixer_amd/csrc/embed_wgrad.h
@@ -138,6 +138,39 @@
 template <int D, int NT> static constexpr size_t embed_wgrad_fast_red_bytes() { return (size_t)(NT / 64) * (EFK / 16) * (D / 16) * 64 * 16; }
 bool m2m_split_eligible(const m2m_tower* t, int B, int training);
 template <int D, int NT>
+static __device__ __forceinline__ void embed_wgrad_bias_walk(const m2m_embed& em, const char* __restrict__ dx0_chn, int npairs, char* smem) {
+    typedef Prec<PREC_BF16> Pr;
+    constexpr int DT = D / 16, NW = NT / 64;
+    const int tid = threadIdx.x, lane = tid & 63, g = lane >> 4, il = lane & 15;
+    const int wave = __builtin_amdgcn_readfirstlane(tid >> 6);
+    f32x4_t* red = reinterpret_cast<f32x4_t*>(smem);
+    Frag ones;
+    ones.u = u32x4_t{0x3F803F80u, 0x3F803F80u, 0x3F803F80u, 0x3F803F80u};
+    f32x4_t accb[DT];
+#pragma unroll
+    for (int dt = 0; dt < DT; ++dt) accb[dt] = f32x4_t{0.f, 0.f, 0.f, 0.f};
+    for (int p = wave; p < npairs; p += NW) {
+        Frag a[DT];
+#pragma unroll
+        for (int dt = 0; dt < DT; ++dt) a[dt] = ld_frag_global(dx0_chn, (long)p * DT + dt, lane);
+#pragma unroll
+        for (int dt = 0; dt < DT; ++dt) Pr::mma(accb[dt], a[dt], ones);
+    }
+    __syncthreads();
+#pragma unroll
+    for (int dt = 0; dt < DT; ++dt) red[(wave * DT + dt) * 64 + lane] = accb[dt];
+    __syncthreads();
+    for (int dt = wave; dt < DT; dt += NW) {
+        f32x4_t sb = red[dt * 64 + lane];
+#pragma unroll
+        for (int w = 1; w < NW; ++w) sb = sb + red[(w * DT + dt) * 64 + lane];
+        if (il == 0) {
+#pragma unroll
+            for (int r = 0; r < 4; ++r) em.g_b[16 * dt + 4 * g + r] += sb[r];
+        }
+    }
+}
+template <int D, int NT>
 static __device__ __forceinline__ void embed_wgrad_fast_body(const m2m_embed& em, const float* __restrict__ in,
                                                              const char* __restrict__ dx0_chn, long M, int N, int npairs, int rpt,
                                                              int chunk, bool vec2, char* smem) {
@@ -242,35 +275,134 @@
             }
         }
     }
-    if (chunk == 0) {
-        Frag ones;
-        ones.u = u32x4_t{0x3F803F80u, 0x3F803F80u, 0x3F803F80u, 0x3F803F80u};
-        f32x4_t accb[DT];
-#pragma unroll
-        for (int dt = 0; dt < DT; ++dt) accb[dt] = f32x4_t{0.f, 0.f, 0.f, 0.f};
-        for (int p = wave; p < npairs; p += NW) {
-            Frag a[DT];
-#pragma unroll
-            for (int dt = 0; dt < DT; ++dt) a[dt] = ld_frag_global(dx0_chn, (long)p * DT + dt, lane);
-#pragma unroll
-            for (int dt = 0; dt < DT; ++dt) Pr::mma(accb[dt], a[dt], ones);
-        }
+    if (chunk == 0) embed_wgrad_bias_walk<D, NT>(em, dx0_chn, npairs, smem);
+}
+template <int D, int NT> static constexpr size_t embed_wgrad_fast_lds() { return embed_wgrad_fast_red_bytes<D, NT>() + 128 * sizeof(int); }
+
+#ifndef EFK16
+#define EFK16 64
+#endif
+#ifndef EFK16_DEPTH
+#define EFK16_DEPTH 4
+#endif
+static inline int m2m_embed_p16_on() {
+    static const int on = [] { const char* v = getenv("M2M_EMBED_P16"); return v ? atoi(v) : 1; }();
+    return on;
+}
+template <int D, int NT, int CW> static constexpr size_t embed_wgrad_p16_lds() {
+    constexpr size_t stage = (size_t)(NT / 64) * 2 * 32 * CW * 2, red = (size_t)(NT / 64) * 2 * (D / 16) * 64 * 16;
+    return stage > red ? stage : red;
+}
+template <int D, int NT, int CW>
+static __device__ __forceinline__ void embed_wgrad_p16_body(const m2m_embed& em, const char* __restrict__ p16,
+                                                            const char* __restrict__ dx0_chn, long M, int npairs, int rpt, int chunk,
+                                                            char* smem) {
+    typedef Prec<PREC_BF16> Pr;
+    typedef short s16x4 __attribute__((ext_vector_type(4)));
+    typedef unsigned int u32x2 __attribute__((ext_vector_type(2)));
+    typedef __attribute__((address_space(3))) s16x4* lds_s16x4_p;
+    constexpr int DT = D / 16, NW = NT / 64, NB = CW / 16;
+    constexpr int CPR = CW / 8, NLD = 32 * CPR / 64, ROW_B = CW * 2, STAGE_B = 32 * ROW_B;
+    static_assert(CW == 32 || CW == 64, "32 or 64 pixel columns per workgroup");
+    const int tid = threadIdx.x, lane = tid & 63, g = lane >> 4, il = lane & 15;
+    const int wave = __builtin_amdgcn_readfirstlane(tid >> 6);
+    const int k0 = chunk * CW;
+    const long pitch = (long)((em.K + 7) & ~7) * 2;
+    auto swz = [](int row) { return CPR == 4 ? (row >> 2) & 3 : (row >> 1) & 7; };
+    constexpr int RPI = 64 / CPR;
+    const int q = lane % CPR, sbase = lane / CPR;
+    const bool colok = k0 + 8 * q < em.K;
+    const char* const src = p16 + (colok ? (long)(k0 + 8 * q) * 2 : 0);
+    char* stage = smem + wave * 2 * STAGE_B;
+    const int rrow = 4 * g + (il >> 2);
+    int rd_off[NB];
+#pragma unroll
+    for (int jb = 0; jb < NB; ++jb) rd_off[jb] = rrow * ROW_B + 16 * ((2 * jb + ((il >> 1) & 1)) ^ swz(rrow)) + 8 * (il & 1);
+
+    f32x4_t acc[NB][DT];
+#pragma unroll
+    for (int jb = 0; jb < NB; ++jb)
+#pragma unroll
+        for (int dt = 0; dt < DT; ++dt) acc[jb][dt] = f32x4_t{0.f, 0.f, 0.f, 0.f};
+
+    struct Tile { Frag a[DT]; u32x4_t v[NLD]; unsigned int okbits; };
+    auto load = [&](Tile& t, int p) {
+#pragma unroll
+        for (int dt = 0; dt < DT; ++dt) t.a[dt] = ld_frag_global(dx0_chn, (long)p * DT + dt, lane);
+        t.okbits = 0u;
+#pragma unroll
+        for (int i = 0; i < NLD; ++i) {
+            const int r = sbase + ((RPI * i) & 15);
+            const long row = (long)(2 * p + (RPI * i) / 16) * rpt + r;
+            const bool ok = r < rpt && row < M && colok;
+            t.v[i] = __builtin_nontemporal_load(reinterpret_cast<const u32x4_t*>(src + (ok ? row : 0) * pitch));
+            t.okbits |= (ok ? 1u : 0u) << i;
+        }
+    };
+    auto mac = [&](const Tile& t, char* st) {
+#pragma unroll
+        for (int i = 0; i < NLD; ++i)
+        {
+            const int srow = sbase + RPI * i;
+            *reinterpret_cast<u32x4_t*>(st + srow * ROW_B + 16 * (q ^ swz(srow))) = ((t.okbits >> i) & 1u) ? t.v[i] : u32x4_t{0u, 0u, 0u, 0u};
+        }
+#pragma unroll
+        for (int jb = 0; jb < NB; ++jb) {
+            const s16x4 lo = __builtin_amdgcn_ds_read_tr16_b64_v4i16((lds_s16x4_p)(st + rd_off[jb]));
+            const s16x4 hi = __builtin_amdgcn_ds_read_tr16_b64_v4i16((lds_s16x4_p)(st + rd_off[jb] + 16 * ROW_B));
+            const u32x2 l2 = __builtin_bit_cast(u32x2, lo), h2 = __builtin_bit_cast(u32x2, hi);
+            Frag b;
+            b.u = u32x4_t{l2[0], l2[1], h2[0], h2[1]};
+#pragma unroll
+            for (int dt = 0; dt < DT; ++dt) Pr::mma(acc[jb][dt], t.a[dt], b);
+        }
+    };
+    constexpr int DEPTH = CW == 32 ? EFK16_DEPTH : 2;
+    static_assert(DEPTH % 2 == 0, "the ring alternates between the two LDS stages");
+    Tile ring[DEPTH];
+    const int nmine = npairs > wave ? (npairs - wave + NW - 1) / NW : 0;
+    auto pair_at = [&](int i) { return wave + NW * min(i, nmine - 1); };
+    if (nmine > 0) {
+#pragma unroll
+        for (int d = 0; d + 1 < DEPTH; ++d) load(ring[d], pair_at(d));
+        for (int i = 0; i < nmine; i += DEPTH) {
+#pragma unroll
+            for (int d = 0; d < DEPTH; ++d) {
+                load(ring[(d + DEPTH - 1) % DEPTH], pair_at(i + d + DEPTH - 1));
+                __builtin_amdgcn_sched_barrier(0);
+                if (i + d >= nmine) ring[d].okbits = 0u;
+                mac(ring[d], stage + (d & 1) * STAGE_B);
+                __builtin_amdgcn_sched_barrier(0);
+            }
+        }
+    }
+    f32x4_t* red = reinterpret_cast<f32x4_t*>(smem);
+    const bool store = (em.wgrad_flags & M2M_WGRAD_OVERWRITE) != 0;
+#pragma unroll
+    for (int h = 0; h < NB / 2; ++h) {
         __syncthreads();
 #pragma unroll
-        for (int dt = 0; dt < DT; ++dt) red[(wave * DT + dt) * 64 + lane] = accb[dt];
+        for (int jb = 0; jb < 2; ++jb)
+#pragma unroll
+            for (int dt = 0; dt < DT; ++dt) red[((wave * 2 + jb) * DT + dt) * 64 + lane] = acc[2 * h + jb][dt];
         __syncthreads();
-        for (int dt = wave; dt < DT; dt += NW) {
-            f32x4_t sb = red[dt * 64 + lane];
-#pragma unroll
-            for (int w = 1; w < NW; ++w) sb = sb + red[(w * DT + dt) * 64 + lane];
-            if (il == 0) {
-#pragma unroll
-                for (int r = 0; r < 4; ++r) em.g_b[16 * dt + 4 * g + r] += sb[r];
+        for (int q = wave; q < 2 * DT; q += NW) {
+            const int jb = q / DT, dt = q % DT;
+            f32x4_t s = red[q * 64 + lane];
+#pragma unroll
+            for (int w = 1; w < NW; ++w) s = s + red[(w * 2 * DT + q) * 64 + lane];
+            const int k = k0 + 16 * (2 * h + jb) + il;
+            if (k < em.K) {
+#pragma unroll
+                for (int r = 0; r < 4; ++r) {
+                    float* qd = em.g_w + (long)(16 * dt + 4 * g + r) * em.K + k;
+                    *qd = store ? s[r] : *qd + s[r];
+                }
             }
         }
     }
-}
-template <int D, int NT> static constexpr size_t embed_wgrad_fast_lds() { return embed_wgrad_fast_red_bytes<D, NT>() + 128 * sizeof(int); }
+    if (chunk == 0) embed_wgrad_bias_walk<D, NT>(em, dx0_chn, npairs, smem);
+}
 
 #define EMB_GROUP 2
 struct EmbedWgradGroupArgs {
@@ -281,7 +413,15 @@
     int N[EMB_GROUP], tpg[EMB_GROUP], nchunks[EMB_GROUP], groups[EMB_GROUP];
     const char* dx0_chn[EMB_GROUP];
     int npairs[EMB_GROUP], rpt[EMB_GROUP], vec2[EMB_GROUP], fast;
+    const char* p16[EMB_GROUP];
+    int p16_chunks[EMB_GROUP], n_p16;
 };
+template <int D, int NT>
+static __device__ __forceinline__ void embed_wgrad_p16_group_body(const EmbedWgradGroupArgs& a, int id, char* smem) {
+    const int e = id < a.p16_chunks[0] ? 0 : 1;
+    if (e) id -= a.p16_chunks[0];
+    embed_wgrad_p16_body<D, NT, EFK16>(a.em[e], a.p16[e], a.dx0_chn[e], a.M[e], a.npairs[e], a.rpt[e], id, smem);
+}
 template <int P, int D, int NT>
 static __device__ __forceinline__ void embed_wgrad_group_body(const EmbedWgradGroupArgs& a, int id, char* smem) {
     const int n0 = a.nchunks[0] * a.groups[0];
@@ -318,7 +458,7 @@
 
 
 static inline int embed_wgrad_group_args_fast(EmbedWgradGroupArgs& a, const m2m_embed* const* es, const float* const* ins,
-                                              const m2m_tower* const* tw, int B) {
+                                              const m2m_tower* const* tw, int B, const void* const* p16s = nullptr) {
     memset(&a, 0, sizeof(a));
     int total = 0;
     for (int i = 0; i < EMB_GROUP; ++i) {
@@ -334,7 +474,11 @@
         a.nchunks[i] = (e->K + EFK - 1) / EFK; a.groups[i] = 1; a.tpg[i] = 0;
         static const int vec2_on = [] { const char* v = getenv("M2M_EMBED_VEC2"); return v ? atoi(v) : 1; }();
         a.vec2[i] = (vec2_on && e->pw % 2 == 0 && e->W % 2 == 0 && ((long)e->H * e->W) % 2 == 0 && e->K % 2 == 0 && ((uintptr_t)ins[i] & 7) == 0) ? 1 : 0;
-        total += a.nchunks[i];
+        if (p16s && p16s[i] && m2m_embed_p16_on() && e->K % 8 == 0) {
+            a.p16[i] = (const char*)p16s[i]; a.p16_chunks[i] = (e->K + EFK16 - 1) / EFK16; a.n_p16 += a.p16_chunks[i];
+            a.nchunks[i] = 0; a.groups[i] = 0;
+        }
+        total += a.nchunks[i] + a.p16_chunks[i];
     }
     a.fast = 1;
     return total;
diff --git a/m2_mixer_amd/csrc/tower_wgrad.hip b/m2_mixer_amd/csrc/tower_wgrad.hip
--- a/m2_mixer_amd/csrc/tower_wgrad.hip
+++ b/m2_mixer_amd/csrc/tower_wgrad.hip
@@ -401,6 +401,8 @@
     int dma;
     int n_embed_first, n_embed_pad;
     int n_reduce, reduce_sets;
+    int p16_before_reduce;
+    int n_p16_first, n_p16_last;
     unsigned int seed, step_host;
     const unsigned int* step_dev;
     unsigned int* bump_counter;
@@ -416,14 +418,26 @@
     int id = blockIdx.x;
     if (a.bump_counter && blockIdx.x == 0 && threadIdx.x == 0) *a.bump_counter += 1u;
 #ifndef M2M_WG_PROBE_TOWERS_ONLY
-    if (a.n_reduce && id >= (int)gridDim.x - a.n_reduce) {
-        const int rid = id - ((int)gridDim.x - a.n_reduce);
+    const int tail_begin = (int)gridDim.x - a.n_reduce - a.n_p16_last;
+    if (id >= tail_begin) {
+        const int tid_ = id - tail_begin;
+        const bool is_p16 = a.p16_before_reduce ? tid_ < a.n_p16_last : tid_ >= a.n_reduce;
+        if (is_p16) {
+            if constexpr (P == PREC_BF16 && D <= 128)
+                embed_wgrad_p16_group_body<D, WgradKernelGeom<P, D, RCDM>::THREADS>(ea, a.p16_before_reduce ? tid_ : tid_ - a.n_reduce, smem);
+            return;
+        }
+        const int rid = a.p16_before_reduce ? tid_ - a.n_p16_last : tid_;
         const int bx = rid % SPR_NBX, L = (rid / SPR_NBX) % a.reduce_sets, z = rid / (SPR_NBX * a.reduce_sets);
         split_small_grads_body<WgradKernelGeom<P, D, RCDM>::THREADS>(ra.t[z], bx, L, reinterpret_cast<float*>(smem));
         return;
     }
     if (id < a.n_embed_pad) {
         if (id < a.n_embed_first) embed_wgrad_group_body<P, D, WgradKernelGeom<P, D, RCDM>::THREADS>(ea, id, smem);
+        else if (id < a.n_embed_first + a.n_p16_first) {
+            if constexpr (P == PREC_BF16 && D <= 128)
+                embed_wgrad_p16_group_body<D, WgradKernelGeom<P, D, RCDM>::THREADS>(ea, id - a.n_embed_first, smem);
+        }
         return;
     }
     id -= a.n_embed_pad;
@@ -553,7 +567,8 @@
 static int launch_wgrad_group(const m2m_tower* const* host, const m2m_tower* const* dev, int n, const m2m_embed* const* embeds,
                               const float* const* inputs, const float* const* d_x0s, const m2m_tower* const* embed_towers,
                               int nembeds, int B, unsigned int seed, unsigned int step, const unsigned int* step_dev, hipStream_t st,
-                              const SplitReduceTower* heads_reduce = nullptr, unsigned int* bump_counter = nullptr) {
+                              const SplitReduceTower* heads_reduce = nullptr, unsigned int* bump_counter = nullptr,
+                              const void* const* p16s = nullptr) {
     typedef WgradKernelGeom<P, D, RCDM> KG;
     WgradGroupArgs a;
     memset(&a, 0, sizeof(a));
@@ -595,12 +610,18 @@
     a.dma = wgrad_use_dma();
     EmbedWgradGroupArgs ea;
     memset(&ea, 0, sizeof(ea));
-    int n_embed_wgs = 0;
+    int n_embed_wgs = 0, n_p16 = 0;
     size_t lds_e = 0;
     bool embeds_separately = false;
+    static const int merged = wgrad_env("M2M_EMBED_MERGED", 1);
+    if (!merged || D > 128) p16s = nullptr;
     if (nembeds) {
-        n_embed_wgs = (P == PREC_BF16 && nembeds == EMB_GROUP) ? embed_wgrad_group_args_fast(ea, embeds, inputs, embed_towers, B) : 0;
-        if (n_embed_wgs) lds_e = embed_wgrad_fast_lds<D, KG::THREADS>();
+        n_embed_wgs = (P == PREC_BF16 && nembeds == EMB_GROUP) ? embed_wgrad_group_args_fast(ea, embeds, inputs, embed_towers, B, p16s) : 0;
+        if (n_embed_wgs) {
+            n_p16 = ea.n_p16; n_embed_wgs -= n_p16;
+            if (n_embed_wgs) lds_e = embed_wgrad_fast_lds<D, KG::THREADS>();
+            if constexpr (D <= 128) { if (n_p16 && embed_wgrad_p16_lds<D, KG::THREADS, EFK16>() > lds_e) lds_e = embed_wgrad_p16_lds<D, KG::THREADS, EFK16>(); }
+        }
         else if (KG::THREADS == 256) { static const int ewgs = wgrad_env("M2M_EMBED_WGS", D >= 256 ? 128 : 512);    n_embed_wgs = embed_wgrad_group_args(ea, embeds, inputs, d_x0s, B, ewgs, nembeds); lds_e = embed_wgrad_lds<D, P>(); }
         else embeds_separately = true;
     }
@@ -609,7 +630,6 @@
         else if (int rc = m2m_embeds_wgrad(embeds, inputs, d_x0s, nembeds, B, (void*)st)) return rc;
     }
     if constexpr (P == PREC_BF16) {
-        static const int merged = wgrad_env("M2M_EMBED_MERGED", 1);
         if (n_embed_wgs && ea.fast && !merged && KG::THREADS != 256) {
             const size_t le = embed_wgrad_fast_lds<D, 256>();
             auto ek = embed_wgrad_fast_group_kernel<D>;
@@ -630,6 +650,10 @@
     }
     static const int embed_first = wgrad_env("M2M_EMBED_FIRST", 1);
     if (ea.fast && n_embed_wgs && embed_first) { a.n_embed_first = n_embed_wgs; a.n_embed_pad = (n_embed_wgs + 7) & ~7; n_embed_wgs = 0; }
+    static const int p16_place = wgrad_env("M2M_EMBED_P16_PLACE", 1);
+    if (n_p16 && p16_place == 2) { a.n_p16_first = n_p16; a.n_embed_pad = (a.n_embed_first + n_p16 + 7) & ~7; n_p16 = 0; }
+    a.n_p16_last = n_p16;
+    a.p16_before_reduce = p16_place == 1;
     SplitReduceArgs ra;
     memset(&ra, 0, sizeof(ra));
     for (int i = 0; i < n; ++i) {
@@ -653,7 +677,7 @@
     }
     for (int i = 0; i < ra.ntow; ++i) a.reduce_sets = ra.t[i].nlaunch > a.reduce_sets ? ra.t[i].nlaunch : a.reduce_sets;
     a.n_reduce = SPR_NBX * a.reduce_sets * ra.ntow;
-    hipLaunchKernelGGL(kern, dim3((unsigned)(a.n_embed_pad + a.n_tower_wgs + n_embed_wgs + a.n_reduce)), dim3(KG::THREADS), lds, st, a, ea, ra);
+    hipLaunchKernelGGL(kern, dim3((unsigned)(a.n_embed_pad + a.n_tower_wgs + n_embed_wgs + a.n_reduce + n_p16)), dim3(KG::THREADS), lds, st, a, ea, ra);
     M2M_CHECK_HIP(hipGetLastError());
     return 0;
 }
@@ -698,7 +722,8 @@
                              const m2m_embed* const* embeds, const float* const* inputs, const float* const* d_x0s,
                              const m2m_tower* const* embed_towers, int nembeds,
                              int B, uint32_t seed, uint32_t step, const uint32_t* step_dev,
-                             const m2m_head* heads, int nheads, int K, void* stream, uint32_t* bump_counter = nullptr) {
+                             const m2m_head* heads, int nheads, int K, void* stream, uint32_t* bump_counter = nullptr,
+                             const void* const* p16s = nullptr) {
     SplitReduceTower hr;
     const SplitReduceTower* heads_reduce = nullptr;
     if (heads && nheads > 0) {
@@ -754,7 +779,7 @@
             return launch_wgrad_group<PREC_BF16, 128, DM_HALF>(towers, dev_towers, ntowers, embeds, inputs, d_x0s, embed_towers, nembeds, B, seed, step, step_dev, st, heads_reduce);
         return launch_wgrad_group<PREC_BF16, 128, DM_NONE>(towers, dev_towers, ntowers, embeds, inputs, d_x0s, embed_towers, nembeds, B, seed, step, step_dev, st, heads_reduce);
     }
-#define M2M_WGG_CASE(PP, DD) if (t->prec == PP && t->D == DD) return launch_wgrad_group<PP, DD, -1>(towers, dev_towers, ntowers, embeds, inputs, d_x0s, embed_towers, nembeds, B, seed, step, step_dev, st, heads_reduce, bump_counter);
+#define M2M_WGG_CASE(PP, DD) if (t->prec == PP && t->D == DD) return launch_wgrad_group<PP, DD, -1>(towers, dev_towers, ntowers, embeds, inputs, d_x0s, embed_towers, nembeds, B, seed, step, step_dev, st, heads_reduce, bump_counter, p16s);
     M2M_WGG_CASE(PREC_BF16, 32) M2M_WGG_CASE(PREC_BF16, 64) M2M_WGG_CASE(PREC_BF16, 128) M2M_WGG_CASE(PREC_BF16, 256)
     M2M_WGG_CASE(PREC_F32, 32) M2M_WGG_CASE(PREC_F32, 64) M2M_WGG_CASE(PREC_F32, 128) M2M_WGG_CASE(PREC_F32, 256)
 #undef M2M_WGG_CASE
@@ -782,6 +807,21 @@
                                      int B, uint32_t seed, uint32_t step, const uint32_t* step_dev,
                                      const m2m_head* heads, int nheads, int K, uint32_t* bump_counter, void* stream) {
     return towers_wgrad_impl(towers, dev_towers, ntowers, embeds, inputs, d_x0s, embed_towers, nembeds, B, seed, step, step_dev, heads, nheads, K, stream, bump_counter);
+}
+
+extern "C" int m2m_towers_wgrad_p16(const m2m_tower* const* towers, const m2m_tower* const* dev_towers, int ntowers,
+                                    const m2m_embed* const* embeds, const float* const* inputs, const float* const* d_x0s,
+                                    const m2m_tower* const* embed_towers, int nembeds,
+                                    int B, uint32_t seed, uint32_t step, const uint32_t* step_dev,
+                                    const m2m_head* heads, int nheads, int K, uint32_t* bump_counter,
+                                    const void* const* p16s, void* stream) {
+    if (p16s && nembeds != EMB_GROUP) { m2m_set_error("towers_wgrad_p16: the patch copies belong to a launch with two embeddings", __FILE__, __LINE__); return -1; }
+    if (p16s) {
+        for (int i = 0; i < nembeds; ++i)
+            if ((uintptr_t)p16s[i] & 15) { m2m_set_error("towers_wgrad_p16: the patch copy must be 16-byte aligned", __FILE__, __LINE__); return -1; }
+    }
+    return towers_wgrad_impl(towers, dev_towers, ntowers, embeds, inputs, d_x0s, embed_towers, nembeds, B, seed, step, step_dev, heads, nheads, K, stream,
+                             bump_counter, p16s);
 }
 
 extern "C" int m2m_embeds_wgrad_form(const m2m_embed* const* embeds, const m2m_tower* const* embed_towers, int nembeds, int B) {
diff --git a/m2_mixer_amd/engine.py b/m2_mixer_amd/engine.py
--- a/m2_mixer_amd/engine.py
+++ b/m2_mixer_amd/engine.py
@@ -737,6 +737,21 @@
                             and towers_forward_embeds_ok([self.t_a, self.t_b], [self.e_a, self.e_b], B)
                             and self.t_a.wgrad_form(B) == 0 and self.t_fus.wgrad_form(B) == 0)
         self._pending_bump = False
+        self._alloc_p16()
+
+    def _alloc_p16(self):
+        self._p16_bufs, self._p16_live = [None, None], None
+        if not self._embed_towers or any(t.wgrad_form(self.B) != 0 for t in (self.t_a, self.t_b, self.t_fus)):
+            return
+        for i, e in enumerate((self.e_a, self.e_b)):
+            need = e.p16_bytes(None, self.B)
+            if need:
+                self._p16_bufs[i] = torch.empty(need, dtype=torch.uint8, device=self.device)
+
+    def _p16_workspaces(self, xa, xb):
+        out = [buf if buf is not None and e.p16_bytes(x, self.B) else None
+               for buf, e, x in zip(self._p16_bufs, (self.e_a, self.e_b), (xa, xb))]
+        return out if any(t is not None for t in out) else None
 
     def _build_fusion(self):
         B, D, dev = self.B, self.D, self.device
@@ -824,6 +839,7 @@
         so = 0
         pa, pb, pf = (None, None, None) if self._heads_pool else (self.pool_a, self.pool_b, self.pool_fus)
         self._pending_bump = False
+        self._p16_live = None
         if self._embed_fold and training and prologue:
             so, self._pending_bump = 1, True
             towers_forward([self.t_a, self.t_b],
@@ -834,7 +850,8 @@
             sa, sb = self.x0_splits
             if can_group_embeds(self.e_a, self.e_b):
                 head = (self.adam_state, self.drop_step, self.losses) if prologue else None
-                embeds_forward([self.e_a, self.e_b], [xa, xb], [self._x0_a, self._x0_b], B, [sa, sb], head)
+                self._p16_live = self._p16_workspaces(xa, xb) if training and with_grad else None
+                embeds_forward([self.e_a, self.e_b], [xa, xb], [self._x0_a, self._x0_b], B, [sa, sb], head, p16s=self._p16_live)
             else:
                 if prologue:
                     self._prologue()
@@ -915,7 +932,7 @@
         if can_group_embeds(self.e_a, self.e_b) and self.e_a.prec == self.t_a.prec and self.e_a.D == self.t_a.D:
             towers_wgrad(wg_towers, B, [self.e_a, self.e_b], [xa, xb], [self.dx0_a, self.dx0_b],
                          seed=self.seed, step=so, step_dev=sd, embed_towers=self._embed_towers, heads=self._wgrad_heads, K=self.K,
-                         bump=bump)
+                         bump=bump, p16s=self._p16_live)
         else:
             if bump is not None:
                 raise RuntimeError("the embedding fold needs the merged weight-gradient launch (it advances the dropout counter)")
diff --git a/m2_mixer_amd/runtime.py b/m2_mixer_amd/runtime.py
--- a/m2_mixer_amd/runtime.py
+++ b/m2_mixer_amd/runtime.py
@@ -405,7 +405,8 @@
 def towers_wgrad(towers: Sequence[TowerRuntime], B: int, embeds: Sequence["EmbedRuntime"] = (),
                  inputs: Sequence[torch.Tensor] = (), d_x0s: Sequence[torch.Tensor] = (), seed: int = 0, step: int = 0,
                  step_dev: Optional[torch.Tensor] = None, embed_towers: Sequence[TowerRuntime] = (),
-                 heads: Optional[Sequence[dict]] = None, K: int = 0, bump: Optional[torch.Tensor] = None):
+                 heads: Optional[Sequence[dict]] = None, K: int = 0, bump: Optional[torch.Tensor] = None,
+                 p16s: Optional[Sequence[Optional[torch.Tensor]]] = None):
     n, ne = len(towers), len(embeds)
     host = (C.POINTER(L.Tower) * n)(*[C.pointer(t.desc) for t in towers])
     dev = (C.c_void_p * n)(*[t.device_desc() for t in towers])
@@ -413,6 +414,12 @@
     ip = (C.c_void_p * max(ne, 1))(*[t.data_ptr() for t in inputs])
     dp = (C.c_void_p * max(ne, 1))(*[t.data_ptr() for t in d_x0s])
     et = (C.POINTER(L.Tower) * max(ne, 1))(*[C.pointer(t.desc) for t in embed_towers]) if len(embed_towers) == ne and ne else None
+    if p16s is not None and any(t is not None for t in p16s):
+        pp = (C.c_void_p * ne)(*[L.ptr(t) for t in p16s])
+        L.check(L.lib().m2m_towers_wgrad_p16(host, dev, n, ep, ip, dp, et, ne, B, seed & 0xFFFFFFFF, step & 0xFFFFFFFF,
+                                             L.ptr(step_dev), _head_array(heads) if heads else None, len(heads) if heads else 0, K,
+                                             L.ptr(bump), pp, L.stream_ptr()), "towers_wgrad_p16")
+        return
     if bump is not None:
         L.check(L.lib().m2m_towers_wgrad_tail(host, dev, n, ep, ip, dp, et, ne, B, seed & 0xFFFFFFFF, step & 0xFFFFFFFF,
                                               L.ptr(step_dev), _head_array(heads) if heads else None, len(heads) if heads else 0, K,
@@ -522,6 +529,9 @@
     def fwd_splits(self) -> int:
         return int(L.lib().m2m_embed_fwd_splits(C.byref(self.desc)))
 
+    def p16_bytes(self, inp: Optional[torch.Tensor], B: int) -> int:
+        return int(L.lib().m2m_embed_p16_bytes(C.byref(self.desc), 16 if inp is None else inp.data_ptr(), B))
+
     def forward(self, inp: torch.Tensor, B: int, x0: torch.Tensor, step_head: Optional[tuple] = None):
         head = None
         if step_head is not None:
@@ -540,7 +550,8 @@
 
 
 def embeds_forward(embeds: Sequence[EmbedRuntime], inputs: Sequence[torch.Tensor], x0s: Sequence[torch.Tensor], B: int,
-                   nsplits: Optional[Sequence[int]] = None, step_head: Optional[tuple] = None):
+                   nsplits: Optional[Sequence[int]] = None, step_head: Optional[tuple] = None,
+                   p16s: Optional[Sequence[Optional[torch.Tensor]]] = None):
     n = len(embeds)
     ep = (C.POINTER(L.Embed) * n)(*[C.pointer(e.desc) for e in embeds])
     ip = (C.c_void_p * n)(*[t.data_ptr() for t in inputs])
@@ -551,6 +562,11 @@
     if step_head is not None:
         adam_state, drop_counter, losses = step_head
         head = C.byref(L.StepHead(adam_state.data_ptr(), drop_counter.data_ptr(), losses.data_ptr(), losses.numel()))
+    if p16s is not None and any(t is not None for t in p16s):
+        pp = (C.c_void_p * n)(*[L.ptr(t) for t in p16s])
+        pb = (C.c_int64 * n)(*[0 if t is None else t.numel() * t.element_size() for t in p16s])
+        L.check(L.lib().m2m_embeds_forward_p16(ep, ip, xp, ns, ps, n, B, head, pp, pb, L.stream_ptr()), "embeds_forward_p16")
+        return
     L.check(L.lib().m2m_embeds_forward(ep, ip, xp, ns, ps, n, B, head, L.stream_ptr()), "embeds_forward")
 
 
```

After: 1.054 million. About the same (-0.3%).
